# DCDmllm/AnyEdit

Measured on AMD Instinct MI355X. Metric: edited-images/sec @512x512, 50 DDIM steps, higher is better.
Workload: dtype bf16; 1 GPU; configs[1]: AnySD (SD-1.5 UNet in=8 + task embedding/expert adapters) 512x512 bf16, 50 DDIM steps, batch=4/GPU, 3-branch CFG (UNet batch 12); images_per_gpu=4, ddim_steps=50, cfg_branches=3, hip_graph=True, parallelism=dp1 (image-sharded, no data-path collective)

## Files before the change

anyedit_amd/_lib.py:

```python
import ctypes
import os

import torch

_HERE = os.path.dirname(os.path.abspath(__file__))
LIB_PATH = os.environ.get("AE_LIB_PATH") or os.path.join(_HERE, "libanyedit_hip.so")

c_void_p, c_int, c_long, c_float = ctypes.c_void_p, ctypes.c_int, ctypes.c_long, ctypes.c_float

SIGNATURES = {
    "ae_version": [],
    "ae_last_error": [],
    "ae_device_arch": [ctypes.c_char_p, c_int],
    "ae_device_info": [ctypes.POINTER(c_int), ctypes.POINTER(c_long), ctypes.POINTER(c_int)],
    "ae_gemm_bf16": [c_void_p, c_long, c_void_p, c_long, c_int, c_void_p, c_long, c_void_p, c_long, c_int, c_int, c_int,
                     c_void_p, c_void_p, c_long, c_void_p, c_long, c_int, c_int, c_int, c_void_p, c_void_p],
    "ae_conv3x3_workspace_floats": [c_int, c_int, c_int, c_int, c_int, c_int, c_int],
    "ae_conv3x3_bf16": [c_void_p, c_void_p, c_void_p, c_void_p, c_long, c_void_p, c_void_p, c_int, c_int, c_int, c_int, c_int,
                        c_int, c_int, c_int, c_void_p, c_void_p, c_int, c_void_p],
    "ae_conv3x3_up2_bf16": [c_void_p, c_void_p, c_void_p, c_void_p, c_int, c_int, c_int, c_int, c_int, c_void_p, c_void_p],
    "ae_gemm_plan": [c_int] * 8 + [ctypes.POINTER(c_int)],
    "ae_conv3x3_plan": [c_int] * 11 + [ctypes.POINTER(c_int)],
    "ae_conv3x3_up2_plan": [c_int] * 6 + [ctypes.POINTER(c_int)],
    "ae_groupnorm_rows_per_chunk": [c_int, c_int],
    "ae_groupnorm_workspace_floats": [c_int, c_int, c_int, c_int],
    "ae_groupnorm_nhwc_bf16": [c_void_p, c_void_p, c_int, c_void_p, c_void_p, c_void_p, c_int, c_int, c_int, c_int, c_float,
                               c_int, c_void_p, c_void_p, c_void_p, c_void_p, c_void_p, c_void_p],
    "ae_layernorm_bf16": [c_void_p, c_void_p, c_void_p, c_void_p, c_int, c_int, c_float, c_void_p],
    "ae_attn_fwd_bf16": [c_void_p, c_void_p, c_void_p, c_void_p, c_int, c_int, c_int, c_int, c_int,
                         c_long, c_long, c_long, c_long, c_long, c_long, c_long, c_long, c_long, c_long, c_long, c_long,
                         c_float, c_void_p, c_void_p, c_int, c_int, c_void_p, c_void_p, c_int,
                         c_void_p, c_void_p, c_int, c_long, c_long, c_long, c_long, c_long, c_long, c_void_p, c_void_p, c_void_p,
                         c_void_p],
    "ae_attn_bwd_bf16": [c_void_p] * 10 + [c_int] * 5 + [c_long] * 21 + [c_float, c_void_p, c_int, c_void_p, c_void_p],
    "ae_attn_bwd_workspace_floats": [c_int] * 5,
    "ae_groupnorm_bwd_workspace_floats": [c_int, c_int, c_int, c_int],
    "ae_groupnorm_bwd_nhwc_bf16": [c_void_p, c_void_p, c_int, c_void_p, c_void_p, c_void_p, c_void_p, c_void_p, c_int, c_int, c_int,
                                   c_int, c_float, c_int, c_void_p, c_void_p, c_void_p, c_int, c_void_p],
    "ae_layernorm_bwd_bf16": [c_void_p, c_void_p, c_void_p, c_void_p, c_void_p, c_int, c_int, c_float, c_int, c_void_p],
    "ae_layernorm_param_grad_f32": [c_void_p, c_void_p, c_void_p, c_void_p, c_void_p, c_int, c_int, c_void_p],
    "ae_add_bf16": [c_void_p, c_void_p, c_void_p, c_long, c_void_p],
    "ae_axpy_bf16": [c_void_p, c_void_p, c_float, c_void_p, c_long, c_void_p],
    "ae_geglu_fwd_bf16": [c_void_p, c_void_p, c_long, c_int, c_void_p],
    "ae_geglu_bwd_bf16": [c_void_p, c_void_p, c_void_p, c_long, c_int, c_void_p],
    "ae_sumpool2x2_bf16": [c_void_p, c_void_p, c_int, c_int, c_int, c_int, c_void_p],
    "ae_colsum_bf16_f32": [c_void_p, c_void_p, c_int, c_int, c_long, c_void_p],
    "ae_mse_grad_f32": [c_void_p, c_void_p, c_void_p, c_long, c_float, c_void_p],
    "ae_adamw_f32": [c_void_p, c_void_p, c_void_p, c_void_p, c_long, c_float, c_float, c_float, c_float, c_float, c_int, c_float,
                     c_void_p],
    "ae_rowsum_f32": [c_void_p, c_void_p, c_int, c_long, c_void_p],
    "ae_scatter_add_rows_f32": [c_void_p, c_void_p, c_void_p, c_int, c_int, c_int, c_void_p],
    "ae_attn_fp8_workspace_bytes": [c_int, c_int, c_int, c_int, c_int],
    "ae_attn_fwd_fp8": [c_void_p, c_void_p, c_void_p, c_void_p, c_int, c_int, c_int, c_int, c_int] + [c_long] * 12 +
                       [c_float, c_void_p, c_void_p, c_int, c_int, c_void_p, c_long, c_void_p],
    "ae_ln_gemm_supported": [c_int, c_int, c_int, c_int],
    "ae_ln_gemm_bf16": [c_void_p, c_long, c_void_p, c_long, c_void_p, c_long, c_int, c_int, c_int, c_void_p, c_void_p, c_long, c_void_p, c_void_p,
                        c_float, c_int, c_void_p, c_void_p],
    "ae_gemm_ln_plan": [c_int, c_int, c_int, c_int, c_int],
    "ae_ff_fused_supported": [c_int, c_int, c_int],
    "ae_ff_fused_bf16": [c_void_p, c_long, c_void_p, c_void_p, c_float, c_void_p, c_long, c_void_p, c_void_p, c_void_p, c_void_p, c_long,
                         c_void_p, c_long, c_void_p, c_void_p, c_long, c_void_p, c_void_p, c_long, c_int, c_int, c_int, c_void_p],
    "ae_gemm_ln_bf16": [c_void_p, c_long, c_void_p, c_long, c_void_p, c_long, c_int, c_int, c_int, c_void_p, c_void_p, c_long, c_int, c_void_p,
                        c_void_p, c_int, c_void_p, c_float, c_void_p],
    "ae_task_gate_bwd": [c_void_p, c_void_p, c_void_p, c_void_p, c_int, c_int, c_int, c_void_p, c_void_p],
    "ae_task_gate_wgrad": [c_void_p, c_void_p, c_void_p, c_void_p, c_void_p, c_int, c_int, c_int, c_int, c_void_p, c_void_p, c_void_p],
    "ae_expert_kv_fwd": [c_void_p, c_void_p, c_void_p, c_void_p, c_int, c_int, c_int, c_int, c_int, c_void_p],
    "ae_expert_kv_dgrad_slices": [c_int],
    "ae_expert_kv_dgrad": [c_void_p, c_void_p, c_void_p, c_void_p, c_int, c_int, c_int, c_int, c_int, c_void_p, c_void_p],
    "ae_expert_kv_wgrad": [c_void_p, c_void_p, c_void_p, c_void_p, c_int, c_int, c_int, c_int, c_int, c_void_p],
    "ae_transpose_last2": [c_void_p, c_void_p, c_int, c_int, c_int, c_int, c_int, c_int, c_void_p],
    "ae_concat_channels_bf16": [c_void_p, c_int, c_void_p, c_int, c_void_p, c_long, c_void_p],
    "ae_im2col3x3_c8_bf16": [c_void_p, c_void_p, c_int, c_int, c_int, c_void_p],
    "ae_split_channels_bf16": [c_void_p, c_int, c_int, c_void_p, c_void_p, c_long, c_int, c_int, c_void_p],
    "ae_timestep_embedding": [c_void_p, c_void_p, c_void_p, c_void_p, c_int, c_int, c_float, c_void_p],
    "ae_ddim_step_f32": [c_void_p, c_void_p, c_void_p, c_void_p, c_void_p, c_void_p, c_long, c_int, c_float, c_float, c_float,
                         c_float, c_float, c_float, c_float, c_float, c_void_p],
    "ae_ddim_encode_step_f32": [c_void_p, c_void_p, c_void_p, c_long, c_int, c_float, c_float, c_float, c_void_p],
    "ae_plms_combine_f32": [c_void_p, c_void_p, c_void_p, c_void_p, c_void_p, c_long, c_int, c_void_p],
    "ae_mask_blend_f32": [c_void_p, c_void_p, c_void_p, c_void_p, c_void_p, c_int, c_int, c_int, c_float, c_float, c_int, c_void_p],
    "ae_q_sample_f32": [c_void_p, c_void_p, c_void_p, c_void_p, c_void_p, c_int, c_long, c_void_p],
    "ae_silu_to_bf16": [c_void_p, c_int, c_void_p, c_long, c_void_p],
    "ae_add_bcast_bf16": [c_void_p, c_void_p, c_void_p, c_long, c_long, c_void_p],
    "ae_resample2x_rows_bf16": [c_void_p, c_void_p, c_int, c_int, c_int, c_int, c_int, c_void_p],
    "ae_scale_shift_rows_bf16": [c_void_p, c_void_p, c_long, c_void_p, c_int, c_long, c_int, c_int, c_void_p],
    "ae_window_partition_bf16": [c_void_p, c_void_p, c_int, c_int, c_int, c_int, c_int, c_int, c_void_p],
    "ae_layernorm_window_supported": [c_int],
    "ae_layernorm_window_bf16": [c_void_p, c_void_p, c_void_p, c_void_p, c_void_p, c_void_p, c_int, c_int, c_int, c_int, c_int, c_int, c_float,
                                 c_void_p],
    "ae_sam_relpos_terms": [c_void_p, c_long, c_long, c_long, c_void_p, c_void_p, c_void_p, c_void_p, c_int, c_int, c_int, c_int,
                            c_int, c_int, c_int, c_void_p],
    "ae_softmax_rows_f32_bf16": [c_void_p, c_long, c_void_p, c_long, c_int, c_int, c_float, c_void_p],
    "ae_gaussian_moments_f32": [c_void_p, c_void_p, c_void_p, c_void_p, c_void_p, c_void_p, c_int, c_long, c_void_p],
    "ae_ms_deform_attn_fwd_f32": [c_void_p] * 6 + [c_int] * 7 + [c_void_p],
    "ae_ms_deform_attn_bwd_f32": [c_void_p] * 9 + [c_int] * 7 + [c_void_p],
    "ae_linear_f32": [c_void_p, c_long, c_void_p, c_long, c_void_p, c_void_p, c_long, c_int, c_int, c_int, c_void_p],
    "ae_dpm_multistep_f32": [c_void_p] * 5 + [c_long, c_int, c_float, c_int, c_int, c_float, c_float, c_int, c_float, c_float, c_float,
                             c_float, c_void_p],
    "ae_layernorm_act_bf16": [c_void_p, c_void_p, c_void_p, c_void_p, c_long, c_int, c_float, c_int, c_void_p],
    "ae_sam_pe_encode_f32": [c_void_p, c_void_p, c_void_p, c_void_p, c_void_p, c_int, c_int, c_float, c_float, c_float, c_void_p],
    "ae_sam_mask_downscale_bf16": [c_void_p] * 10 + [c_int, c_int, c_int, c_float, c_void_p],
    "ae_sam_mask_product_f32": [c_void_p, c_void_p, c_void_p, c_int, c_int, c_int, c_int, c_int, c_void_p],
    "ae_sam_postprocess_masks": [c_void_p, c_void_p, c_void_p] + [c_int] * 8 + [c_float, c_int, c_void_p],
    "ae_nms_sorted_f32": [c_void_p, c_void_p, c_int, c_float, c_void_p],
    "ae_sam_preprocess_f32": [c_void_p, c_int, c_void_p, c_int, c_int, c_int, c_int, c_int, c_void_p, c_void_p, c_void_p],
    "ae_patchify_f32_bf16": [c_void_p, c_void_p, c_int, c_int, c_int, c_int, c_int, c_void_p],
    "ae_mse_f32": [c_void_p, c_void_p, c_void_p, c_void_p, c_long, c_void_p],
    "ae_lincomb4_f32": [c_void_p, c_void_p, c_float, c_void_p, c_float, c_void_p, c_float, c_void_p, c_float, c_long, c_void_p],
    "ae_dpm_adaptive_err_f32": [c_void_p, c_void_p, c_void_p, c_float, c_float, c_int, c_long, c_void_p, c_void_p],
    "ae_task_gate": [c_void_p, c_void_p, c_void_p, c_void_p, c_int, c_int, c_int, c_int, c_void_p, c_void_p, c_void_p, c_void_p],
    "ae_attn_causal_short_bf16": [c_void_p, c_void_p, c_void_p, c_void_p, c_int, c_int, c_int, c_int] + [c_long] * 12 + [c_float, c_void_p],
    "ae_clip_embed_bf16": [c_void_p, c_int, c_void_p, c_void_p, c_void_p, c_int, c_int, c_int, c_int, c_int, c_void_p],
    "ae_bias_act_f32_bf16": [c_void_p, c_long, c_void_p, c_void_p, c_long, c_long, c_int, c_int, c_void_p],
    "ae_clip_pool_eos_bf16": [c_void_p, c_int, c_void_p, c_void_p, c_int, c_int, c_int, c_long, c_void_p],
    "ae_clip_patch_rows_bf16": [c_void_p, c_int, c_void_p, c_int, c_int, c_int, c_int, c_int, c_int, c_float, c_void_p, c_void_p, c_void_p],
    "ae_clip_vision_embed_ln_bf16": [c_void_p, c_long, c_void_p, c_void_p, c_void_p, c_void_p, c_void_p, c_int, c_int, c_int, c_float, c_void_p],
    "ae_clip_vision_pool_ln_bf16": [c_void_p, c_long, c_void_p, c_void_p, c_void_p, c_int, c_int, c_float, c_void_p],
    "ae_dino_embed_bf16": [c_void_p, c_long, c_void_p, c_void_p, c_void_p, c_void_p, c_int, c_int, c_int, c_void_p],
    "ae_swiglu_f32_bf16": [c_void_p, c_long, c_void_p, c_void_p, c_long, c_long, c_int, c_void_p],
    "ae_swin_window_attn_bf16": [c_void_p, c_long, c_void_p, c_void_p, c_void_p, c_long, c_int, c_int, c_int, c_int, c_int, c_int, c_int, c_float, c_void_p],
    "ae_swin_merge_ln_bf16": [c_void_p, c_void_p, c_void_p, c_void_p, c_int, c_int, c_int, c_int, c_float, c_void_p],
    "ae_scale_residual_f32_bf16": [c_void_p, c_long, c_void_p, c_void_p, c_void_p, c_long, c_void_p, c_long, c_long, c_int, c_void_p],
    "ae_biattn_split_rows": [c_int],
    "ae_biattn_workspace_bytes": [c_int, c_int, c_int, c_int, c_int],
    "ae_biattn_bf16": [c_void_p, c_long] * 4 + [c_void_p, c_void_p] + [c_void_p, c_long] * 2 + [c_int] * 5 + [c_float, c_void_p, c_long, c_void_p],
    "ae_attn_masked_short_bf16": [c_void_p] * 5 + [c_int] * 4 + [c_long] * 12 + [c_float, c_void_p],
    "ae_contrastive_bf16": [c_void_p, c_long, c_void_p, c_void_p, c_void_p, c_long, c_void_p] + [c_int] * 5 + [c_void_p],
    "ae_topk_rows_max_n": [],
    "ae_topk_rows_f32": [c_void_p, c_long, c_void_p, c_int, c_int, c_int, c_void_p],
    "ae_gdino_proposals_f32": [c_void_p, ctypes.POINTER(c_int), ctypes.POINTER(c_int), c_int, c_void_p, c_void_p, c_int, c_int, c_void_p],
    "ae_gdino_query_sine": [c_void_p, c_void_p, c_void_p, c_void_p, c_long, c_int, c_int, c_int, c_void_p],
    "ae_gdino_box_refine_f32": [c_void_p, c_long, c_void_p, c_void_p, c_void_p, c_void_p, c_void_p, c_long, c_int, c_void_p],
    "ae_gdino_text_spans": [c_void_p, c_int, c_int, c_int, c_int] + [c_long] * 8 + [c_void_p, c_void_p, c_void_p, c_void_p],
    "ae_bert_embed_ln_bf16": [c_void_p, c_void_p, c_void_p] + [c_void_p] * 6 + [c_int] * 6 + [c_float, c_void_p],
    "ae_attn_span_short_bf16": [c_void_p] * 5 + [c_int] * 4 + [c_long] * 12 + [c_float, c_void_p],
    "ae_gdino_level_geometry": [c_void_p, c_int, c_int, c_int, ctypes.POINTER(c_int), ctypes.POINTER(c_int), c_int, c_float, c_float, c_void_p, c_void_p, c_void_p,
                                c_void_p, c_int, c_void_p],
    "ae_gdino_neck_groupnorm_workspace_floats": [c_int, c_int],
    "ae_gdino_neck_groupnorm": [c_void_p, c_long, c_void_p, c_void_p, c_float, c_void_p, c_long, c_long, c_int, c_int, c_void_p, c_void_p],
    "ae_gdino_ground": [c_void_p, c_void_p, c_float, c_float, c_void_p, c_void_p, c_void_p, c_void_p, c_void_p, c_int, c_int, c_int, c_void_p],
    "ae_hed_stem_bf16": [c_void_p, c_int, c_long, c_long, c_long, c_long, c_void_p, c_void_p, c_void_p, c_void_p, c_int, c_int, c_int, c_int, c_void_p],
    "ae_relu_bf16": [c_void_p, c_long, c_void_p],
    "ae_hed_tail_bf16": [c_void_p, c_void_p, c_void_p, c_void_p, c_void_p, c_int, c_int, c_int, c_int, c_void_p],
    "ae_hed_fuse": [c_void_p] * 7 + [c_int] * 4 + [c_void_p],
    "ae_dpt_reassemble_bf16": [c_void_p, c_long, c_void_p, c_void_p, c_int, c_int, c_int, c_int, c_int, c_void_p],
    "ae_dpt_resize_bf16": [c_void_p] * 4 + [c_int] * 6 + [c_void_p],
    "ae_dpt_relu_bf16": [c_void_p, c_void_p, c_long, c_void_p],
    "ae_dpt_tail_bf16": [c_void_p] * 4 + [c_int] * 4 + [c_void_p],
    "ae_depth_resize_minmax_f32": [c_void_p] * 3 + [c_int] * 5 + [c_void_p],
    "ae_depth_colorize_u8": [c_void_p] * 4 + [c_int] * 3 + [c_void_p],
    "ae_dwconv_rows_bf16": [c_void_p] * 5 + [c_int] * 5 + [c_void_p],
    "ae_patch2_rows_bf16": [c_void_p, c_void_p, c_int, c_int, c_int, c_int, c_void_p],
    "ae_layernorm_rows_nchw": [c_void_p, c_void_p, c_void_p, c_float, c_void_p, c_void_p, c_int, c_int, c_int, c_int, c_void_p],
    "ae_ppm_pool_rows_bf16": [c_void_p, c_void_p, c_int, c_int, c_int, c_int, c_void_p, c_int, c_void_p],
    "ae_resize_concat_rows_bf16": [c_void_p] * 8 + [c_int, c_void_p, c_long, c_void_p, c_long, c_int, c_int, c_int, c_void_p],
    "ae_seg_argmax_u8": [c_void_p, c_long, c_int, c_void_p, c_void_p, c_void_p] + [c_int] * 7 + [c_void_p],
    "ae_attn_mutual_bf16": [c_void_p] * 4 + [c_int] * 4 + [c_long] * 12 + [c_float, ctypes.POINTER(c_int), c_void_p, c_void_p, c_void_p, c_void_p],
    "ae_attn_token_map_bf16": [c_void_p] * 3 + [c_int] * 5 + [c_long] * 6 + [c_float, ctypes.POINTER(ctypes.c_ulonglong), c_int, c_void_p],
    "ae_masactrl_classes": [c_void_p, c_long, c_int, c_int, c_float, c_int, ctypes.POINTER(c_int), ctypes.POINTER(c_int), c_void_p, c_void_p, c_void_p],
}
_RESTYPES = {"ae_last_error": ctypes.c_char_p, "ae_groupnorm_workspace_floats": c_long, "ae_conv3x3_workspace_floats": c_long,
             "ae_groupnorm_bwd_workspace_floats": c_long, "ae_attn_fp8_workspace_bytes": c_long, "ae_attn_bwd_workspace_floats": c_long,
             "ae_biattn_workspace_bytes": c_long, "ae_gdino_neck_groupnorm_workspace_floats": c_long}


class AnyEditHipError(RuntimeError):
    pass


def _load():
    if not os.path.exists(LIB_PATH):
        raise ImportError(
            f"{LIB_PATH} is missing: the HIP extension is REQUIRED (no CPU/eager fallback exists). "
            "Build it with `python -c 'import __graft_entry__ as g; g.build()'` or `python anyedit_amd/build.py`.")
    lib = ctypes.CDLL(LIB_PATH)
    for name, argtypes in SIGNATURES.items():
        fn = getattr(lib, name)
        fn.argtypes = argtypes
        fn.restype = _RESTYPES.get(name, c_int)
    return lib


lib = _load()


def check(rc, what=""):
    if rc != 0:
        msg = lib.ae_last_error()
        raise AnyEditHipError(f"{what} failed (rc={rc}): {msg.decode() if msg else ''}")


def device_arch():
    buf = ctypes.create_string_buffer(128)
    check(lib.ae_device_arch(buf, 128), "ae_device_arch")
    return buf.value.decode()
```

anyedit_amd/csrc/gemm_conv.hip:

```cpp
#include "common.hpp"
#include <stdlib.h>
#include <string.h>
#include <type_traits>

namespace {

#ifndef AE_CONV_SPEC
#define AE_CONV_SPEC 1
#endif
#ifndef AE_XE_OCC
#define AE_XE_OCC 4
#endif
#ifndef AE_PP_LAB
#define AE_PP_LAB 0
#endif
#ifndef AE_PP_PRIO
#define AE_PP_PRIO 1
#endif
#ifndef AE_PP_DMA_FIRST
#define AE_PP_DMA_FIRST 0
#endif
constexpr int BK = 64;

enum { A_DENSE = 0, A_CONV3 = 1 };
enum { EPI_NONE = 0, EPI_GELU = 1, EPI_GEGLU = 2, EPI_SILU = 3, EPI_RELU = 4 };

struct GemmArgs {
    const bf16_t* A;
    const bf16_t* A2;
    const bf16_t* W;
    void* C;
    const float* bias;
    const bf16_t* res;
    const float* addvec;
    int M, N, K, Ksplit;
    long lda, lda2, ldw, ldc, ldr, ldav;
    int epi, out_f32, rows_per_batch;
    int H, Wd, Cin, CinPad, Ho, Wo, stride, ups;
    unsigned a_bytes, a2_bytes, w_bytes;
    int splitk;
    float* partial;
    float* colstats;
    int kmajor;
    int m_fast;
    int xe;
    float* rowstats;
    const float* ln_stats;
    const float* ln_colsum;
    int ln_parts;
    float ln_eps;
    int sub2;
};

__device__ __forceinline__ void lds_dma16(__amdgpu_buffer_rsrc_t rs, bf16_t* lds_dst, int voffset, int soffset = 0) {
#if defined(__HIP_DEVICE_COMPILE__)
    __builtin_amdgcn_raw_ptr_buffer_load_lds(rs, (__attribute__((address_space(3))) void*)lds_dst, 16, voffset, soffset, 0, 0);
#endif
}

#ifdef AE_GEMM_LAB
__device__ unsigned long long g_gemm_dbg[32];
#define GL_T(i) do { const unsigned long long t_ = __builtin_readcyclecounter(); if (lab_me) g_gemm_dbg[lab_base + (i)] += t_ - tlast; tlast = t_; } while (0)
#elif defined(AE_GEMM_TRACE)
constexpr int TR_K0 = 18, TR_T = 6;
__device__ unsigned long long g_pp_trace[8 * TR_T * 16];
#define GL_T(i) do { __builtin_amdgcn_sched_barrier(0); tr_t[(i)] = __builtin_readcyclecounter(); __builtin_amdgcn_sched_barrier(0); } while (0)
#else
#define GL_T(i)
#endif

constexpr int epilogue_passes(int FM, int bytes_per_frag_row, int lds_bytes) {
    for (int ps = 1; ps <= FM; ++ps)
        if (FM % ps == 0 && (FM / ps) * bytes_per_frag_row <= lds_bytes) return ps;
    return FM;
}

template <int BM, int BN, int AMODE, int WAVES_M = 2, int WAVES_N = 2, bool GLDS = false, int WAVES_K = 1, int STAGES = 2, bool CS = false, int LAB = 0, int WA = 0, int XE = 0>
__global__ __launch_bounds__(64 * WAVES_M * WAVES_N * WAVES_K, (XE == 2 && BM == 128 && BN == 128 && STAGES == 2) ? AE_XE_OCC : 0) void gemm_kernel(const GemmArgs p) {
    static_assert(XE == 0 || (AMODE == A_DENSE && WAVES_K == 1 && !CS && GLDS), "row statistics / LayerNorm fold: dense LDS-DMA instantiations, one K group, no column statistics");
    static_assert(XE != 1 || BN / WAVES_N == 64, "row statistics are emitted per 64-column slice = one wave tile's width");
    static_assert(STAGES == 2 || (GLDS && WAVES_K == 1), "the deep LDS ring exists only for the LDS-DMA loader");
    static_assert(!WA || (GLDS && STAGES == 2 && WAVES_K == 1), "operand-ahead is a variant of the two-stage LDS-DMA pipeline");
    static_assert(WA == 0 || WA == 1 || WA == 3 || WA == 4, "WA: 0 none, 1 weights two tiles ahead (three W stages), 3 ping-pong (two wave groups one barrier apart), 4 ping-pong over an activation slab per (channel chunk, ky)");
    static_assert(WA < 3 || 64 * WAVES_M * WAVES_N * WAVES_K == 512, "the ping-pong loops pair wave w with wave w + 4 (one SIMD's two waves)");
    static_assert(WA != 4 || (AMODE == A_CONV3 && GLDS && BM % 16 == 0), "the slab loop is a 3x3-convolution loop");
    static_assert(WAVES_K == 1, "one K group per block (the two-group form is removed: DESIGN.md, \"Built, measured, removed\")");
    constexpr int NT = 64 * WAVES_M * WAVES_N * WAVES_K;
    constexpr int WM = BM / WAVES_M, WN = BN / WAVES_N;
    constexpr int FM = WM / 16, FN = WN / 16;
    constexpr int A_CH = BM * 8 / NT, B_CH = BN * 8 / NT;
    static_assert((BM * 8) % NT == 0 && (BN * 8) % NT == 0, "tile / thread-count combination not supported");
    extern __shared__ __attribute__((aligned(16))) unsigned char smem_raw[];
    bf16_t* const smem = reinterpret_cast<bf16_t*>(smem_raw);
    bf16_t* sA = smem;
    bf16_t* sB = smem + (WA >= 3 ? 3 : STAGES) * BM * BK;

#ifndef AE_WAVE_SGPR
#define AE_WAVE_SGPR 1
#endif
    const int tid = threadIdx.x, lane = tid & 63, wave = AE_WAVE_SGPR ? __builtin_amdgcn_readfirstlane(tid >> 6) : tid >> 6;
#ifdef AE_GEMM_TRACE
    const bool tr_blk = blockIdx.x == gridDim.x / 2 && WA == 3;
    unsigned long long* const tr_lds = reinterpret_cast<unsigned long long*>(smem_raw + 152 * 1024);
    int tr_kt = -1;
    unsigned long long tr_t[16];
#pragma unroll
    for (int q = 0; q < 16; ++q) tr_t[q] = 0;
#endif
#ifdef AE_GEMM_LAB
    unsigned long long tlast = __builtin_readcyclecounter();
    const bool lab_me = blockIdx.x == gridDim.x / 2 && lane == 0 && (wave == 0 || wave == 4);
    const int lab_base = wave == 0 ? 0 : 16;
#endif
    const int wk = wave / (WAVES_M * WAVES_N), wmn = wave % (WAVES_M * WAVES_N);
    const int wm = wmn / WAVES_N, wn = wmn % WAVES_N;
    const int l15 = lane & 15, lg = lane >> 4;
    const int ntn = (p.N + BN - 1) / BN, ntm = (p.M + BM - 1) / BM;
    const int ntiles = ntm * ntn;
    const int split = blockIdx.x / ntiles;
    const int py = (AMODE == A_CONV3 && p.sub2) ? split >> 1 : 0, px = (AMODE == A_CONV3 && p.sub2) ? split & 1 : 0;
    const int tile = xcd_remap(blockIdx.x % ntiles, ntiles);
    const int m0 = (p.m_fast ? tile % ntm : tile / ntn) * BM, n0 = (p.m_fast ? tile / ntm : tile % ntn) * BN;

    long a_base[A_CH];
    int a_iy[A_CH], a_ix[A_CH];
#pragma unroll
    for (int i = 0; i < A_CH; ++i) {
        const int row = (tid + i * NT) >> 3;
        const int m = m0 + row;
        const int mc = min(m, p.M - 1);
        if (AMODE == A_DENSE) {
            a_base[i] = (long)mc;
            a_iy[i] = a_ix[i] = 0;
        } else {
            const int hw = p.Ho * p.Wo;
            const int b = mc / hw, rem = mc - b * hw;
            const int oy = rem / p.Wo, ox = rem - oy * p.Wo;
            a_base[i] = (long)b * p.H * p.Wd;
            a_iy[i] = (m < p.M) ? oy * p.stride - 1 : -100000;
            a_ix[i] = ox * p.stride - 1;
        }
    }
    long b_base[B_CH];
#pragma unroll
    for (int i = 0; i < B_CH; ++i) {
        const int row = (tid + i * NT) >> 3;
        b_base[i] = (long)min(n0 + row, p.N - 1) * p.ldw;
    }

    const __amdgpu_buffer_rsrc_t rsA = __builtin_amdgcn_make_buffer_rsrc(const_cast<bf16_t*>(p.A), 0, (int)p.a_bytes, 0x00020000);
    const __amdgpu_buffer_rsrc_t rsA2 = __builtin_amdgcn_make_buffer_rsrc(const_cast<bf16_t*>(p.A2 ? p.A2 : p.A), 0, (int)(p.A2 ? p.a2_bytes : 0u), 0x00020000);
    const __amdgpu_buffer_rsrc_t rsW = __builtin_amdgcn_make_buffer_rsrc(const_cast<bf16_t*>(p.W) + ((AMODE == A_CONV3 && p.sub2) ? (long)split * p.N * p.ldw : 0L), 0, (int)p.w_bytes, 0x00020000);
    constexpr int OOB = (int)0x80000000;
    int fa_off[A_CH], fa2_off[A_CH], fb_off[B_CH];
    unsigned fa_mask[A_CH];
#pragma unroll
    for (int i = 0; i < A_CH; ++i) {
        const int id = tid + i * NT, row = id >> 3;
        const int c = GLDS ? ((id & 7) ^ (row & 7)) : (id & 7);
        const int m = m0 + row;
        fa_mask[i] = 0u;
        if (AMODE == A_DENSE) {
            fa_off[i] = (m < p.M) ? (int)((long)m * p.lda * 2) + c * 16 : OOB;
            fa2_off[i] = (m < p.M) ? (int)((long)m * p.lda2 * 2) + c * 16 : OOB;
        } else {
            fa2_off[i] = OOB;
            const int hw = p.Ho * p.Wo;
            const int mc = min(m, p.M - 1);
            const int b = mc / hw, rem = mc - b * hw;
            const int oy = rem / p.Wo, ox = rem - oy * p.Wo;
            const int iy0 = oy * p.stride - 1, ix0 = ox * p.stride - 1;
            fa_off[i] = (int)(((long)(b * p.H + iy0) * p.Wd + ix0) * p.Cin + c * 8) * 2;
            const int Hv = p.ups ? 2 * p.H : p.H, Wv = p.ups ? 2 * p.Wd : p.Wd;
            if (m < p.M) {
#pragma unroll
                for (int t9 = 0; t9 < 9; ++t9) {
                    const int iy = iy0 + t9 / 3, ix = ix0 + t9 % 3;
                    if ((unsigned)iy < (unsigned)Hv && (unsigned)ix < (unsigned)Wv && (p.ups != 2 || ((iy | ix) & 1) == 0)) fa_mask[i] |= 1u << t9;
                }
            }

        }
    }
#pragma unroll
    for (int i = 0; i < B_CH; ++i) {
        const int id = tid + i * NT, row = id >> 3;
        const int c = GLDS ? ((id & 7) ^ (row & 7)) : (id & 7);
        fb_off[i] = (n0 + row < p.N) ? (int)((long)(n0 + row) * p.ldw * 2) + c * 16 : OOB;
    }
    const bool conv_fast = (AMODE == A_CONV3) && p.Cin == p.CinPad;

    u32x4 ra[A_CH], rb[B_CH];
    const u32x4 zero4 = {0u, 0u, 0u, 0u};
    const int KT_all = (p.K + BK - 1) / BK;
    const int kt_per = (KT_all + p.splitk - 1) / p.splitk;
    const int kt_begin = (AMODE == A_CONV3 && p.sub2) ? 0 : split * kt_per;
    const int KT = max(min(KT_all - kt_begin, kt_per), 0);
    const int klast = p.K - 8;
    const int conv_per = AMODE == A_CONV3 ? p.CinPad / BK : 1;
    const unsigned conv_per_magic = (AE_CONV_SPEC && conv_per > 1) ? 0xFFFFFFFFu / (unsigned)conv_per + 1u : 0u;
    const unsigned pp_magic = (WA == 3 && conv_per > 1) ? 0xFFFFFFFFu / (unsigned)conv_per + 1u : 0u;
    int ld_tap = (kt_begin * BK) / (AMODE == A_CONV3 ? p.CinPad : 1 << 30), ld_ci = (AMODE == A_CONV3) ? (kt_begin * BK) % p.CinPad : 0;
    if (AMODE == A_CONV3 && p.kmajor) { ld_tap = kt_begin % 9; ld_ci = (kt_begin / 9) * BK; }

    auto load_tile = [&](int kt) __attribute__((always_inline)) {
        const int k0 = (kt_begin + kt) * BK;
        const bool full_k = k0 + BK <= p.K;
        if (AMODE == A_DENSE && full_k && (k0 + BK <= p.Ksplit || k0 >= p.Ksplit)) {
            if (k0 < p.Ksplit) {
#pragma unroll
                for (int i = 0; i < A_CH; ++i) ra[i] = __builtin_amdgcn_raw_buffer_load_b128(rsA, fa_off[i] + k0 * 2, 0, 0);
            } else {
#pragma unroll
                for (int i = 0; i < A_CH; ++i) ra[i] = __builtin_amdgcn_raw_buffer_load_b128(rsA2, fa2_off[i] + (k0 - p.Ksplit) * 2, 0, 0);
            }
#pragma unroll
            for (int i = 0; i < B_CH; ++i) rb[i] = __builtin_amdgcn_raw_buffer_load_b128(rsW, fb_off[i] + k0 * 2, 0, 0);
            return;
        }
        if (conv_fast) {
            const int ky = ld_tap / 3, kx = ld_tap - ky * 3;
            const int tap_off = ((ky * p.Wd + kx) * p.Cin + ld_ci) * 2;
#pragma unroll
            for (int i = 0; i < A_CH; ++i) {
                int src = fa_off[i] + tap_off;
                if (p.ups) {
                    const int cc = GLDS ? (((tid + i * NT) & 7) ^ (((tid + i * NT) >> 3) & 7)) : ((tid + i * NT) & 7);
                    src = (int)((a_base[i] + (long)(max(a_iy[i] + ky, 0) >> 1) * p.Wd + (max(a_ix[i] + kx, 0) >> 1)) * p.Cin + cc * 8 + ld_ci) * 2;
                }
                const int off = ((fa_mask[i] >> ld_tap) & 1u) ? src : OOB;
                ra[i] = __builtin_amdgcn_raw_buffer_load_b128(rsA, off, 0, 0);
            }
            ld_ci += BK;
            if (ld_ci >= p.CinPad) { ld_ci = 0; ++ld_tap; }
#pragma unroll
            for (int i = 0; i < B_CH; ++i) rb[i] = __builtin_amdgcn_raw_buffer_load_b128(rsW, fb_off[i] + k0 * 2, 0, 0);
            return;
        }
        if (AMODE == A_DENSE) {
#pragma unroll
            for (int i = 0; i < A_CH; ++i) {
                const int c = (tid + i * NT) & 7;
                const int k = min(k0 + c * 8, klast);
                const bf16_t* src = (k >= p.Ksplit) ? p.A2 + a_base[i] * p.lda2 + (k - p.Ksplit) : p.A + a_base[i] * p.lda + k;
                ra[i] = *reinterpret_cast<const u32x4*>(src);
            }
        } else {
            const int ky = ld_tap / 3, kx = ld_tap - ky * 3;
            const int Hv = p.ups ? 2 * p.H : p.H, Wv = p.ups ? 2 * p.Wd : p.Wd;
#pragma unroll
            for (int i = 0; i < A_CH; ++i) {
                const int c = (tid + i * NT) & 7;
                const int iy = a_iy[i] + ky, ix = a_ix[i] + kx;
                const int ci = ld_ci + c * 8;
                const bool ok = (unsigned)iy < (unsigned)Hv && (unsigned)ix < (unsigned)Wv && ci < p.Cin && (p.ups != 2 || ((iy | ix) & 1) == 0);
                const int cy = min(max(iy, 0), Hv - 1), cx = min(max(ix, 0), Wv - 1);
                const int sy = p.ups ? (cy >> 1) : cy, sx = p.ups ? (cx >> 1) : cx;
                const u32x4 v = *reinterpret_cast<const u32x4*>(p.A + (a_base[i] + (long)sy * p.Wd + sx) * p.Cin + min(ci, p.Cin - 8));
                ra[i] = ok ? v : zero4;
            }
            ld_ci += BK;
            if (ld_ci >= p.CinPad) { ld_ci = 0; ++ld_tap; }
        }
#pragma unroll
        for (int i = 0; i < B_CH; ++i) {
            const int k = k0 + ((tid + i * NT) & 7) * 8;
            const u32x4 v = *reinterpret_cast<const u32x4*>(p.W + b_base[i] + min(k, klast));
            rb[i] = (k < p.K) ? v : zero4;
        }
    };

    auto store_tile = [&](int buf) __attribute__((always_inline)) {
#pragma unroll
        for (int i = 0; i < A_CH; ++i) {
            const int id = tid + i * NT, row = id >> 3, c = id & 7;
            *reinterpret_cast<u32x4*>(sA + buf * BM * BK + row * BK + ((c ^ (row & 7)) << 3)) = ra[i];
        }
#pragma unroll
        for (int i = 0; i < B_CH; ++i) {
            const int id = tid + i * NT, row = id >> 3, c = id & 7;
            *reinterpret_cast<u32x4*>(sB + buf * BN * BK + row * BK + ((c ^ (row & 7)) << 3)) = rb[i];
        }
    };

    f32x4 acc[FM][FN];
#pragma unroll
    for (int i = 0; i < FM; ++i)
#pragma unroll
        for (int j = 0; j < FN; ++j) acc[i][j] = (f32x4){0.f, 0.f, 0.f, 0.f};

    float ln_r[XE == 2 ? FM : 1], ln_t[XE == 2 ? FM : 1];
    constexpr int LNP = 5;
    constexpr bool SC_LDS = XE == 2 && WA == 3;
    static_assert(!SC_LDS || (BN % 4 == 0 && (3 * BM + 2 * BN) * BK * 2 + 2 * BN * 4 <= 160 * 1024), "s / c of the block must fit behind the ping-pong ring");
    float* const sc_lds = reinterpret_cast<float*>(smem_raw + (3 * BM + 2 * BN) * BK * 2);
    f32x2 raw[XE == 2 ? FM : 1][LNP];
    f32x4 szp[(XE == 2 && !SC_LDS) ? FN : 1], bzp[(XE == 2 && !SC_LDS) ? FN : 1], scv[2];
    if constexpr (XE == 2) {
#pragma unroll
        for (int i = 0; i < FM; ++i) {
            const int m = min(m0 + wm * WM + i * 16 + l15, p.M - 1);
            const f32x2* sp = reinterpret_cast<const f32x2*>(p.ln_stats) + (long)m * p.ln_parts;
#pragma unroll
            for (int u = 0; u < LNP; ++u) raw[i][u] = sp[min(lg + 4 * u, p.ln_parts - 1)];
        }
        if constexpr (SC_LDS) {
            const int n = min(n0 + 4 * min(tid, BN / 4 - 1), p.N - 4);
            scv[0] = *reinterpret_cast<const f32x4*>(p.ln_colsum + n);
            scv[1] = *reinterpret_cast<const f32x4*>(p.bias + n);
        } else {
#pragma unroll
            for (int j = 0; j < FN; ++j) {
                const int nc = p.epi == EPI_GEGLU ? min(n0 + wn * WN + (j & ~1) * 16 + lg * 4, p.N - 20) + (j & 1) * 16 : min(n0 + wn * WN + j * 16 + lg * 4, p.N - 4);
                szp[j] = *reinterpret_cast<const f32x4*>(p.ln_colsum + nc);
                bzp[j] = *reinterpret_cast<const f32x4*>(p.bias + nc);
            }
        }
    }
    auto xe_mid = [&]() __attribute__((always_inline)) {
        if constexpr (XE == 2) {
            const float inv_k = 1.0f / (float)p.K;
#pragma unroll
            for (int i = 0; i < FM; ++i) {
                float s = 0.f, q = 0.f;
#pragma unroll
                for (int u = 0; u < LNP; ++u) {
                    const bool in = lg + 4 * u < p.ln_parts;
                    s += in ? raw[i][u][0] : 0.f;
                    q += in ? raw[i][u][1] : 0.f;
                }
                s += __shfl_xor(s, 16, 64); q += __shfl_xor(q, 16, 64);
                s += __shfl_xor(s, 32, 64); q += __shfl_xor(q, 32, 64);
                const float mu = s * inv_k;
                const float r = rsqrtf(fmaxf(q * inv_k - mu * mu, 0.f) + p.ln_eps);
                ln_r[i] = r;
                ln_t[i] = -r * mu;
            }
            if constexpr (SC_LDS) {
                if (tid < BN / 4) {
                    const float hc = (p.epi == EPI_GEGLU && ((4 * tid) & 16) == 0) ? 0.5f : 1.0f;
                    reinterpret_cast<f32x4*>(sc_lds)[tid] = scv[0];
                    reinterpret_cast<f32x4*>(sc_lds + BN)[tid] = (f32x4){scv[1][0] * hc, scv[1][1] * hc, scv[1][2] * hc, scv[1][3] * hc};
                }
            }
        }
    };

    auto compute_tile = [&](int cur, int curB = -1) __attribute__((always_inline)) {
        if (LAB == 2) return;
        const bf16_t* cA = sA + cur * BM * BK + (wm * WM) * BK;
        const bf16_t* cB = sB + (curB < 0 ? cur : curB) * BN * BK + (wn * WN) * BK;
#pragma unroll
        for (int kk = 0; kk < 2; ++kk) {
            bf16x8_t af[FM], bfr[FN];
            const int ch = kk * 4 + lg;
#pragma unroll
            for (int i = 0; i < FM; ++i) {
                const int row = i * 16 + l15;
                if (LAB == 3) af[i] = as_bf16x8((u32x4){(uint32_t)(i + cur), 0x3f803f80u, (uint32_t)lane, 0u});
                else af[i] = as_bf16x8(*reinterpret_cast<const u32x4*>(cA + row * BK + ((ch ^ (row & 7)) << 3)));
            }
#pragma unroll
            for (int j = 0; j < FN; ++j) {
                const int row = j * 16 + l15;
                if (LAB == 3) bfr[j] = as_bf16x8((u32x4){(uint32_t)(j + kk), 0x3f803f80u, (uint32_t)lane, 0u});
                else bfr[j] = as_bf16x8(*reinterpret_cast<const u32x4*>(cB + row * BK + ((ch ^ (row & 7)) << 3)));
            }
#pragma unroll
            for (int i = 0; i < FM; ++i)
#pragma unroll
                for (int j = 0; j < FN; ++j)
                    acc[i][j] = __builtin_amdgcn_mfma_f32_16x16x32_bf16(bfr[j], af[i], acc[i][j], 0, 0, 0);
        }
    };

    if (!GLDS) {
        load_tile(0);
        store_tile(0);
        __syncthreads();
        for (int kt = 0; kt < KT; ++kt) {
            const int cur = kt & 1;
            if (kt + 1 < KT) load_tile(kt + 1);
            compute_tile(cur);
            if (kt + 1 < KT) store_tile(cur ^ 1);
            __syncthreads();
        }
    } else {
        int fa_cur[A_CH];
        auto dma_a = [&](int kt, int buf) __attribute__((always_inline)) {
            const int k0 = (kt_begin + kt) * BK;
            if (AMODE == A_DENSE) {
                const bool second = k0 >= p.Ksplit;
                if (AE_CONV_SPEC) {
                    if (!second) {
#pragma unroll
                        for (int i = 0; i < A_CH; ++i) lds_dma16(rsA, sA + buf * BM * BK + (wave + (NT / 64) * i) * 8 * BK, fa_off[i], k0 * 2);
                    } else {
#pragma unroll
                        for (int i = 0; i < A_CH; ++i) lds_dma16(rsA2, sA + buf * BM * BK + (wave + (NT / 64) * i) * 8 * BK, fa2_off[i], (k0 - p.Ksplit) * 2);
                    }
                } else {
#pragma unroll
                for (int i = 0; i < A_CH; ++i) {
                    bf16_t* dst = sA + buf * BM * BK + (wave + (NT / 64) * i) * 8 * BK;
                    if (!second) lds_dma16(rsA, dst, fa_off[i], k0 * 2);
                    else lds_dma16(rsA2, dst, fa2_off[i], (k0 - p.Ksplit) * 2);
                }
                }
            } else {
                int cur_tap = ld_tap, cur_ci = ld_ci;
                constexpr bool STATELESS = true;
                if (STATELESS) {
                    const int lin = kt_begin + kt;
                    if (p.kmajor) { cur_tap = lin % 9; cur_ci = (lin / 9) * BK; }
                    else if (AE_CONV_SPEC) {
                        cur_tap = conv_per == 1 ? lin : (int)__umulhi((unsigned)lin, conv_per_magic);
                        cur_ci = (lin - cur_tap * conv_per) * BK;
                    } else { const int per = p.CinPad / BK; cur_tap = lin / per; cur_ci = (lin - cur_tap * per) * BK; }
                }
                const int ky = p.sub2 ? py + (cur_tap >> 1) : cur_tap / 3, kx = p.sub2 ? px + (cur_tap & 1) : cur_tap - ky * 3;
                const int mbit = p.sub2 ? ky * 3 + kx : cur_tap;
                if (cur_ci == 0 || kt == 0 || p.kmajor) {
#pragma unroll
                    for (int i = 0; i < A_CH; ++i) {
                        int src = fa_off[i] + ((ky * p.Wd + kx) * p.Cin) * 2;
                        if (p.ups) {
                            const int cc = ((tid + i * NT) & 7) ^ (((tid + i * NT) >> 3) & 7);
                            src = (int)((a_base[i] + (long)(max(a_iy[i] + ky, 0) >> 1) * p.Wd + (max(a_ix[i] + kx, 0) >> 1)) * p.Cin + cc * 8) * 2;
                        }
                        fa_cur[i] = ((fa_mask[i] >> mbit) & 1u) ? src : OOB;
                    }
                }
                const int tap_off = cur_ci * 2;
                if (!(LAB == 4 && (kt % 9) >= 2)) {
#pragma unroll
                for (int i = 0; i < A_CH; ++i) {
                    bf16_t* dst = sA + buf * BM * BK + (wave + (NT / 64) * i) * 8 * BK;
                    lds_dma16(rsA, dst, fa_cur[i], tap_off);
                }
                }
                if (STATELESS) {
                } else if (p.kmajor) {
                    if (++ld_tap == 9) { ld_tap = 0; ld_ci += BK; }
                } else {
                    ld_ci += BK;
                    if (ld_ci >= p.CinPad) { ld_ci = 0; ++ld_tap; }
                }
            }
        };
        auto dma_w = [&](int kt, int buf) __attribute__((always_inline)) {
            const int k0 = (kt_begin + kt) * BK;
#pragma unroll
            for (int i = 0; i < B_CH; ++i) {
                bf16_t* dst = sB + buf * BN * BK + (wave + (NT / 64) * i) * 8 * BK;
                lds_dma16(rsW, dst, fb_off[i], k0 * 2);
            }
        };
        auto dma_tile = [&](int kt, int buf) __attribute__((always_inline)) { dma_a(kt, buf); dma_w(kt, buf); };
        if constexpr (WA == 4) {
            static_assert(BK * 2 == 128, "slab rows are 128 bytes");
            constexpr int SLAB_P = (BM + BM / 16 + 1 + 7) / 8;
            constexpr int S_CH = (SLAB_P + NT / 64 - 1) / (NT / 64);
            constexpr int A_ST = SLAB_P * 1024, W_ST = BN * BK * 2;
            const int lds0 = (int)(uintptr_t)((__attribute__((address_space(3))) char*)smem_raw);
            const int ldsW = lds0 + 2 * A_ST + wave * 1024;
            const int grp = wave >> 2;
            const int W1 = p.Wd + 1, nrow = BM / p.Wd;
            const int y0 = (m0 / p.Wd) % p.H;
            int sl_off[S_CH], sl_dst[S_CH];
            unsigned sl_ok[S_CH];
#pragma unroll
            for (int j = 0; j < S_CH; ++j) {
                int q = wave + (NT / 64) * j;
                if (q >= SLAB_P) q -= NT / 64;
                const int srow = 8 * q + (lane >> 3);
                const int jr = srow / W1, pos = srow - jr * W1;
                const int m = m0 + jr * p.Wd + pos - 1;
                int y = y0 + jr;
                y -= (y >= p.H) ? p.H : 0;
                unsigned ok = 0u;
                if (pos > 0 && jr < nrow && m < p.M) {
#pragma unroll
                    for (int ky = 0; ky < 3; ++ky)
                        if ((unsigned)(y + ky - 1) < (unsigned)p.H) ok |= 1u << ky;
                }
                sl_ok[j] = ok;
                sl_off[j] = m * p.Cin * 2 + (((lane & 7) ^ (lane >> 3)) << 4);
                sl_dst[j] = lds0 + q * 1024;
            }
            const int ky_step = p.Wd * p.Cin * 2;
            const int cbase = kt_begin / 9;
            auto pp_slab = [&](int c, int ky, int st) __attribute__((always_inline)) {
                int off[S_CH];
#pragma unroll
                for (int j = 0; j < S_CH; ++j) off[j] = ((sl_ok[j] >> ky) & 1u) ? sl_off[j] + (ky - 1) * ky_step : OOB;
#pragma unroll
                for (int j = 0; j < S_CH; ++j) asm volatile("" : "+v"(off[j]));
#pragma unroll
                for (int j = 0; j < S_CH; ++j) ae_dma16(rsA, sl_dst[j] + st * A_ST, off[j], (cbase + c) * (BK * 2));
            };
            auto pp_w = [&](int kt, int st) __attribute__((always_inline)) {
                const int k0 = (kt_begin + kt) * BK;
#pragma unroll
                for (int i = 0; i < B_CH; ++i) ae_dma16(rsW, ldsW + st * W_ST + i * (NT / 64) * 1024, fb_off[i], k0 * 2);
            };
            int a_rd[FM][3][2];
#pragma unroll
            for (int i = 0; i < FM; ++i) {
                const int r0 = wm * WM + i * 16;
                const int base = r0 + r0 / p.Wd + l15;
#pragma unroll
                for (int kx = 0; kx < 3; ++kx)
#pragma unroll
                    for (int kk = 0; kk < 2; ++kk) a_rd[i][kx][kk] = (base + kx) * 128 + (((kk * 4 + lg) ^ ((base + kx) & 7)) << 4);
            }
            int w_rd[2];
#pragma unroll
            for (int kk = 0; kk < 2; ++kk) w_rd[kk] = 2 * A_ST + (wn * WN + l15) * 128 + (((kk * 4 + lg) ^ (l15 & 7)) << 4);
            bf16x8_t af[FM], bfr[FN];
            auto pp_read = [&](int kk, int kx, int sa, int sw) __attribute__((always_inline)) {
#pragma unroll
                for (int i = 0; i < FM; ++i) af[i] = as_bf16x8(*reinterpret_cast<const u32x4*>(smem_raw + sa * A_ST + a_rd[i][kx][kk]));
#pragma unroll
                for (int j = 0; j < FN; ++j) bfr[j] = as_bf16x8(*reinterpret_cast<const u32x4*>(smem_raw + sw * W_ST + w_rd[kk] + j * 16 * 128));
            };
            auto pp_mfma = [&]() __attribute__((always_inline)) {
                __builtin_amdgcn_sched_barrier(0);
                if (AE_PP_PRIO) __builtin_amdgcn_s_setprio(1);
#pragma unroll
                for (int i = 0; i < FM; ++i)
#pragma unroll
                    for (int j = 0; j < FN; ++j) acc[i][j] = __builtin_amdgcn_mfma_f32_16x16x32_bf16(bfr[j], af[i], acc[i][j], 0, 0, 0);
                if (AE_PP_PRIO) __builtin_amdgcn_s_setprio(0);
                __builtin_amdgcn_sched_barrier(0);
                __builtin_amdgcn_s_barrier();
                __builtin_amdgcn_sched_barrier(0);
            };
            if (KT > 0) { pp_w(0, 0); pp_slab(0, 0, 0); }
            asm volatile("s_waitcnt vmcnt(0)" ::: "memory");
            __builtin_amdgcn_s_barrier();
            if (grp) __builtin_amdgcn_s_barrier();
            __builtin_amdgcn_sched_barrier(0);
            for (int kt0 = 0; kt0 < KT; kt0 += 18) {
                const int c0 = kt0 / 9;
#pragma unroll
                for (int u = 0; u < 18; ++u) {
                    const int kt = kt0 + u;
                    if (kt >= KT) break;
                    const int tap = u % 9, ky = tap / 3, kx = tap % 3;
                    const int sa = ((u / 9) + ky) & 1, sw = u & 1;
                    pp_read(0, kx, sa, sw);
                    if (kt + 1 < KT) pp_w(kt + 1, sw ^ 1);
                    asm volatile("s_waitcnt lgkmcnt(0)" ::: "memory");
                    __builtin_amdgcn_sched_barrier(0);
                    __builtin_amdgcn_s_barrier();
                    pp_mfma();
                    pp_read(1, kx, sa, sw);
                    const bool slab_next = kx == 0 && kt + 3 < KT;
                    if (slab_next) pp_slab(ky == 2 ? c0 + u / 9 + 1 : c0 + u / 9, ky == 2 ? 0 : ky + 1, sa ^ 1);
                    asm volatile("s_waitcnt lgkmcnt(0)" ::: "memory");
                    if (slab_next) asm volatile("s_waitcnt vmcnt(%0)" ::"n"(S_CH) : "memory");
                    else asm volatile("s_waitcnt vmcnt(0)" ::: "memory");
                    __builtin_amdgcn_sched_barrier(0);
                    __builtin_amdgcn_s_barrier();
                    pp_mfma();
                }
            }
            if (!grp) __builtin_amdgcn_s_barrier();
            __builtin_amdgcn_sched_barrier(0);
        } else if constexpr (WA == 3) {
            const int lds0 = (int)(uintptr_t)((__attribute__((address_space(3))) char*)smem_raw);
            constexpr int A_ST = BM * BK * 2, W_ST = BN * BK * 2;
            const int ldsA = lds0 + wave * 1024, ldsW = lds0 + 3 * A_ST + wave * 1024;
            const int grp = wave >> 2;
            auto pp_w = [&](int kt, int st) __attribute__((always_inline)) {
                const int k0 = (kt_begin + kt) * BK;
#pragma unroll
                for (int i = 0; i < B_CH; ++i) ae_dma16(rsW, ldsW + st * W_ST + i * (NT / 64) * 1024, fb_off[i], k0 * 2);
            };
            int cs_tap = 0, cs_kx = 0, cs_base = 0, cs_ci = 0;
            const int cs_cin2 = p.Cin * 2, cs_row2 = (p.Wd - 3) * p.Cin * 2;
            auto cs_set = [&](int kt) __attribute__((always_inline)) {
                const int lin = kt_begin + kt;
                if (p.kmajor) { cs_tap = lin % 9; cs_ci = (lin / 9) * BK; }
                else { cs_tap = conv_per == 1 ? lin : (int)__umulhi((unsigned)lin, pp_magic); cs_ci = (lin - cs_tap * conv_per) * BK; }
                int ky = cs_tap / 3;
                cs_kx = cs_tap - ky * 3;
                if (p.sub2) { ky = py + (cs_tap >> 1); cs_kx = px + (cs_tap & 1); cs_tap = ky * 3 + cs_kx; }
                cs_base = ((ky * p.Wd + cs_kx) * p.Cin) * 2;
            };
            auto cs_next = [&]() __attribute__((always_inline)) {
                bool tap_step = true;
                if (!p.kmajor) { cs_ci += BK; tap_step = cs_ci >= p.CinPad; cs_ci = tap_step ? 0 : cs_ci; }
                if (tap_step) {
                    if (p.sub2) {
                        if (cs_kx == px) { ++cs_tap; ++cs_kx; cs_base += cs_cin2; }
                        else { cs_tap += 2; cs_kx = px; cs_base += cs_row2 + 2 * cs_cin2; }
                    } else {
                    ++cs_tap; ++cs_kx; cs_base += cs_cin2;
                    if (cs_kx == 3) { cs_kx = 0; cs_base += cs_row2; }
                    if (cs_tap == 9) { cs_tap = 0; cs_base = 0; cs_ci += BK; }
                    }
                }
            };
            auto pp_a = [&](int kt, int st) __attribute__((always_inline)) {
                if constexpr (AMODE == A_DENSE) {
                    const int k0 = (kt_begin + kt) * BK;
                    if (k0 < p.Ksplit) {
#pragma unroll
                        for (int i = 0; i < A_CH; ++i) ae_dma16(rsA, ldsA + st * A_ST + i * (NT / 64) * 1024, fa_off[i], k0 * 2);
                    } else {
#pragma unroll
                        for (int i = 0; i < A_CH; ++i) ae_dma16(rsA2, ldsA + st * A_ST + i * (NT / 64) * 1024, fa2_off[i], (k0 - p.Ksplit) * 2);
                    }
                } else {
                    int off[A_CH];
#pragma unroll
                    for (int i = 0; i < A_CH; ++i) off[i] = ((fa_mask[i] >> cs_tap) & 1u) ? fa_off[i] + cs_base : OOB;
#pragma unroll
                    for (int i = 0; i < A_CH; ++i) asm volatile("" : "+v"(off[i]));
#pragma unroll
                    for (int i = 0; i < A_CH; ++i) ae_dma16(rsA, ldsA + st * A_ST + i * (NT / 64) * 1024, off[i], cs_ci * 2);
                    cs_next();
                }
            };
            bf16x8_t af[FM], bfr[FN];
            auto pp_read = [&](int kk, int sa, int sw) __attribute__((always_inline)) {
                const bf16_t* cA = sA + sa * BM * BK + (wm * WM) * BK;
                const bf16_t* cB = sB + sw * BN * BK + (wn * WN) * BK;
                const int ch = kk * 4 + lg;
#pragma unroll
                for (int i = 0; i < FM; ++i) {
                    const int row = i * 16 + l15;
                    if (AE_PP_LAB == 2 || AE_PP_LAB == 3) af[i] = as_bf16x8((u32x4){(uint32_t)(i + sa), 0x3f803f80u, (uint32_t)lane, 0u});
                    else af[i] = as_bf16x8(*reinterpret_cast<const u32x4*>(cA + row * BK + ((ch ^ (row & 7)) << 3)));
                }
#pragma unroll
                for (int j = 0; j < FN; ++j) {
                    const int row = j * 16 + l15;
                    if (AE_PP_LAB == 2 || AE_PP_LAB == 3) bfr[j] = as_bf16x8((u32x4){(uint32_t)(j + kk), 0x3f803f80u, (uint32_t)lane, 0u});
                    else bfr[j] = as_bf16x8(*reinterpret_cast<const u32x4*>(cB + row * BK + ((ch ^ (row & 7)) << 3)));
                }
            };
            auto pp_mfma = [&](int lab_m, int lab_b) __attribute__((always_inline)) {
                __builtin_amdgcn_sched_barrier(0);
                if (AE_PP_PRIO) __builtin_amdgcn_s_setprio(1);
                if (AE_PP_LAB != 2) {
#pragma unroll
                for (int i = 0; i < FM; ++i)
#pragma unroll
                    for (int j = 0; j < FN; ++j) acc[i][j] = __builtin_amdgcn_mfma_f32_16x16x32_bf16(bfr[j], af[i], acc[i][j], 0, 0, 0);
                }
                if (AE_PP_PRIO) __builtin_amdgcn_s_setprio(0);
                __builtin_amdgcn_sched_barrier(0);
                GL_T(lab_m);
                __builtin_amdgcn_s_barrier();
                __builtin_amdgcn_sched_barrier(0);
                GL_T(lab_b);
            };
            if constexpr (AMODE == A_CONV3) cs_set(0);
            pp_w(0, 0); pp_a(0, 0);
            if (KT > 1) { pp_a(1, 1); asm volatile("s_waitcnt vmcnt(%0)" ::"n"(A_CH) : "memory"); }
            else asm volatile("s_waitcnt vmcnt(0)" ::: "memory");
            xe_mid();
            __builtin_amdgcn_s_barrier();
            if (grp) __builtin_amdgcn_s_barrier();
            __builtin_amdgcn_sched_barrier(0);
            GL_T(0);
            for (int kt0 = 0; kt0 < KT; kt0 += 6) {
#pragma unroll
                for (int u = 0; u < 6; ++u) {
                    const int kt = kt0 + u;
                    if (kt >= KT) break;
                    const int sa = u % 3, sw = u & 1;
#ifdef AE_GEMM_TRACE
                    tr_kt = kt;
                    GL_T(0);
#endif
                    if (AE_PP_DMA_FIRST && AE_PP_LAB != 1 && kt + 1 < KT) pp_w(kt + 1, sw ^ 1);
                    pp_read(0, sa, sw);
                    if (!AE_PP_DMA_FIRST && AE_PP_LAB != 1 && kt + 1 < KT) pp_w(kt + 1, sw ^ 1);
                    asm volatile("s_waitcnt lgkmcnt(0)" ::: "memory");
                    __builtin_amdgcn_sched_barrier(0);
                    GL_T(1);
                    __builtin_amdgcn_s_barrier();
                    GL_T(2);
                    pp_mfma(3, 8);
                    if (AE_PP_DMA_FIRST && AE_PP_LAB != 1 && kt + 2 < KT) pp_a(kt + 2, (u + 2) % 3);
                    pp_read(1, sa, sw);
                    if (!AE_PP_DMA_FIRST && AE_PP_LAB != 1 && kt + 2 < KT) pp_a(kt + 2, (u + 2) % 3);
                    asm volatile("s_waitcnt lgkmcnt(0)" ::: "memory");
                    GL_T(9);
                    if (kt + 2 < KT) asm volatile("s_waitcnt vmcnt(%0)" ::"n"(A_CH) : "memory");
                    else asm volatile("s_waitcnt vmcnt(0)" ::: "memory");
                    __builtin_amdgcn_sched_barrier(0);
                    GL_T(10);
                    __builtin_amdgcn_s_barrier();
                    GL_T(11);
                    pp_mfma(12, 13);
#ifdef AE_GEMM_TRACE
                    if (tr_blk && kt >= TR_K0 && kt < TR_K0 + TR_T && lane == 0) {
#pragma unroll
                        for (int q = 0; q < 16; ++q) tr_lds[(wave * TR_T + (kt - TR_K0)) * 16 + q] = tr_t[q];
                    }
#endif
#ifdef AE_GEMM_LAB
                    if (lab_me) g_gemm_dbg[lab_base + 5] += 1;
#endif
                }
            }
            if (!grp) __builtin_amdgcn_s_barrier();
            __builtin_amdgcn_sched_barrier(0);
#ifdef AE_GEMM_TRACE
            tr_kt = -1;
            if (tr_blk) {
                asm volatile("s_waitcnt lgkmcnt(0)" ::: "memory");
                __builtin_amdgcn_s_barrier();
                for (int q = tid; q < 8 * TR_T * 16; q += NT) g_pp_trace[q] = tr_lds[q];
            }
#endif
        } else if constexpr (WA != 0) {
            constexpr int FAR = B_CH;
            dma_a(0, 0); dma_w(0, 0); if (KT > 1) dma_w(1, 1);
            if (KT > 1) asm volatile("s_waitcnt vmcnt(%0)" ::"n"(FAR) : "memory");
            else asm volatile("s_waitcnt vmcnt(0)" ::: "memory");
            xe_mid();
            __builtin_amdgcn_s_barrier();
            for (int kt0 = 0; kt0 < KT; kt0 += 6) {
#pragma unroll
                for (int u = 0; u < 6; ++u) {
                    const int kt = kt0 + u;
                    if (kt >= KT) break;
                    const int near_cur = u & 1, far_cur = u % 3, far_next = (u + 2) % 3;
                    if (kt + 1 < KT) dma_a(kt + 1, near_cur ^ 1);
                    if (kt + 2 < KT) dma_w(kt + 2, far_next);
                    compute_tile(near_cur, far_cur);
                    if (kt + 2 < KT) asm volatile("s_waitcnt vmcnt(%0)" ::"n"(FAR) : "memory");
                    else asm volatile("s_waitcnt vmcnt(0)" ::: "memory");
                    asm volatile("s_waitcnt lgkmcnt(0)" ::: "memory");
                    __builtin_amdgcn_s_barrier();
                    asm volatile("" ::: "memory");
                }
            }
        } else if constexpr (STAGES == 2) {
            dma_tile(0, 0);
            __syncthreads();
            GL_T(0);
            for (int kt = 0; kt < KT; ++kt) {
                const int cur = kt & 1;
                if (LAB != 1 && kt + 1 < KT) dma_tile(kt + 1, cur ^ 1);
                GL_T(1);
                compute_tile(cur);
                GL_T(2);
                __syncthreads();
                GL_T(3);
#ifdef AE_GEMM_LAB
                if (lab_me) g_gemm_dbg[lab_base + 5] += 1;
#endif
            }
        } else {
            constexpr int PIECES = A_CH + B_CH;
            constexpr int AHEAD = STAGES - 1;
#pragma unroll
            for (int t = 0; t < AHEAD; ++t)
                if (t < KT) dma_tile(t, t);
            xe_mid();
            int cur = 0, nxt = AHEAD % STAGES;
// ... 387 lines not shown
        }
        if (p.res) { o[0] += bf16lo(rr.x); o[1] += bf16hi(rr.x); o[2] += bf16lo(rr.y); o[3] += bf16hi(rr.y); }
        if (p.out_f32) *reinterpret_cast<f32x4*>(reinterpret_cast<float*>(p.C) + (long)m * p.ldc + n) = (f32x4){o[0], o[1], o[2], o[3]};
        else *reinterpret_cast<u32x2*>(reinterpret_cast<bf16_t*>(p.C) + (long)m * p.ldc + n) = (u32x2){pack_bf16x2(o[0], o[1]), pack_bf16x2(o[2], o[3])};
    }
}

__global__ __launch_bounds__(256) void colstats_kernel(const bf16_t* x, long ld, int M, int N, float* out) {
    __shared__ float red[8][2][256];
    const int cc = threadIdx.x & 31, rr = threadIdx.x >> 5;
    const int n = blockIdx.y * 256 + cc * 8;
    const int r0 = blockIdx.x * 32;
    float s[8], q[8];
#pragma unroll
    for (int e = 0; e < 8; ++e) s[e] = q[e] = 0.f;
    if (n < N) {
        u32x4 v[4];
#pragma unroll
        for (int j = 0; j < 4; ++j) v[j] = *reinterpret_cast<const u32x4*>(x + (long)min(r0 + rr + 8 * j, M - 1) * ld + n);
#pragma unroll
        for (int j = 0; j < 4; ++j) {
            const float keep = (r0 + rr + 8 * j < M) ? 1.f : 0.f;
            const uint32_t w[4] = {v[j].x, v[j].y, v[j].z, v[j].w};
#pragma unroll
            for (int e = 0; e < 4; ++e) {
                const float a = bf16lo(w[e]) * keep, c = bf16hi(w[e]) * keep;
                s[2 * e] += a; q[2 * e] += a * a;
                s[2 * e + 1] += c; q[2 * e + 1] += c * c;
            }
        }
    }
#pragma unroll
    for (int e = 0; e < 8; ++e) { red[rr][0][cc * 8 + e] = s[e]; red[rr][1][cc * 8 + e] = q[e]; }
    __syncthreads();
    const int col = threadIdx.x;
    if (blockIdx.y * 256 + col < N) {
        float a = 0.f, c = 0.f;
#pragma unroll
        for (int r = 0; r < 8; ++r) { a += red[r][0][col]; c += red[r][1][col]; }
        *reinterpret_cast<f32x2*>(out + ((long)blockIdx.x * N + blockIdx.y * 256 + col) * 2) = (f32x2){a, c};
    }
}

int pick_tile(int M, int N) {
    const int cand[3][2] = {{128, 128}, {128, 64}, {64, 64}};
    if (N % 160 == 0 && N % 128 != 0 && (long)((M + 127) / 128) * (N / 160) >= 256) return 3;
    for (int c = 0; c < 3; ++c) {
        const long tm = (M + cand[c][0] - 1) / cand[c][0], tn = (N + cand[c][1] - 1) / cand[c][1];
        const double waste = (double)(tn * cand[c][1]) / (double)N;
        if (tm * tn >= 256 && waste <= 1.10) return c;
    }
    return 2;
}

struct Plan { int tile, splitk; };
Plan make_plan(int M, int N, int K, bool can_split) {
    const int t = pick_tile(M, N);
    const int kt = (K + BK - 1) / BK;
    static const int force_s = getenv("AE_GEMM_SPLITK") ? atoi(getenv("AE_GEMM_SPLITK")) : 0;
    static const int t320_split = getenv("AE_CONV_T320_SPLITK") ? atoi(getenv("AE_CONV_T320_SPLITK")) : 3;
    if (t320_split && can_split && N % 320 == 0 && M % 192 == 0 && force_s <= 0) {
        const long t192 = (long)(M / 192) * (N / 320);
        if (t192 >= 32 && t192 <= (t320_split == 2 ? 64 : (t320_split == 3 && kt < 180 ? 64 : 128))) {
            int s = (int)(256 / t192);
            if (s > 8) s = 8;
            while (s > 1 && kt / s < 16) --s;
            if (s >= 2) return {4, s};
        }
    }
    if (!can_split || kt < 32 || t == 0 || t == 3) return {t, 1};
    const long t128 = (long)((M + 127) / 128) * ((N + 127) / 128);
    const double waste128 = (double)(((N + 127) / 128) * 128) / (double)N;
    if (waste128 <= 1.10 && t128 < 256) {
        int s = force_s > 0 ? force_s : (int)((480 + t128 - 1) / t128);
        static const int smax = getenv("AE_CONV_SPLIT_MAX") ? atoi(getenv("AE_CONV_SPLIT_MAX")) : 8;
        if (s > smax) s = smax;
        if (s > kt / 8) s = kt / 8;
        if (s >= 2) return {0, s};
    }
    return {t, 1};
}

template <typename Kern>
int launch_kernel(Kern kern, unsigned grid, int threads, size_t lds, hipStream_t stream, const GemmArgs& a, const char* what) {
    if (lds > 64 * 1024) {
        static const void* done[32];
        static int ndone = 0;
        const void* fn = reinterpret_cast<const void*>(kern);
        bool seen = false;
        for (int i = 0; i < ndone; ++i) seen |= done[i] == fn;
        if (!seen) {
            if (hipFuncSetAttribute(fn, hipFuncAttributeMaxDynamicSharedMemorySize, (int)lds) != hipSuccess) {
                ae_set_error("hipFuncSetAttribute(MaxDynamicSharedMemorySize=%zu) failed", lds);
                return AE_ERR_LAUNCH;
            }
            if (ndone < 32) done[ndone++] = fn;
        }
    }
    hipLaunchKernelGGL(kern, dim3(grid), dim3(threads), lds, stream, a);
    return ae_check_launch(what);
}

struct PlanReport {
    int BM, BN, AMODE, WAVES_M, WAVES_N, GLDS, WAVES_K, STAGES, CS, LAB, WA, XE;
    int grid, threads, lds, splitk;
    int reduce, colstats;
    int rowpanel;
};
#define AE_PLAN_INTS 19
static_assert(sizeof(PlanReport) == AE_PLAN_INTS * sizeof(int), "PlanReport is the int array of anyedit_hip.h");

void* const kQueryPtr = reinterpret_cast<void*>(uintptr_t(256));
float* const kQueryF32 = reinterpret_cast<float*>(uintptr_t(256));
int plan_out(int rc, const PlanReport& r, int* plan) {
    if (!rc) memcpy(plan, &r, sizeof r);
    return rc;
}

struct LaunchCtx { const GemmArgs& a; hipStream_t stream; const char* what; PlanReport* report; };

template <int BM, int BN, int AMODE, int WAVES_M = 2, int WAVES_N = 2, bool GLDS = false, int WAVES_K = 1, int STAGES = 2, bool CS = false, int LAB = 0, int WA = 0, int XE = 0>
int run_tile(const LaunchCtx& c, long grid, size_t lds) {
    constexpr int threads = 64 * WAVES_M * WAVES_N * WAVES_K;
    if (c.report) {
        *c.report = PlanReport{BM, BN, AMODE, WAVES_M, WAVES_N, GLDS, WAVES_K, STAGES, CS, LAB, WA, XE, (int)grid, threads, (int)lds, c.a.splitk, 0, 0, 0};
        return 0;
    }
    return launch_kernel(gemm_kernel<BM, BN, AMODE, WAVES_M, WAVES_N, GLDS, WAVES_K, STAGES, CS, LAB, WA, XE>, (unsigned)grid, threads, lds, c.stream, c.a, c.what);
}

template <int BM, int BN, int AMODE, int WAVES_M, int WAVES_N>
int run_plain(const LaunchCtx& c, bool glds, long grid) {
    const size_t lds = (size_t)2 * (BM + BN) * BK * sizeof(bf16_t);
    return glds ? run_tile<BM, BN, AMODE, WAVES_M, WAVES_N, true>(c, grid, lds) : run_tile<BM, BN, AMODE, WAVES_M, WAVES_N, false>(c, grid, lds);
}

template <int AMODE>
int launch(const GemmArgs& a_in, hipStream_t stream, PlanReport* report = nullptr, int split_tile = 0) {
    GemmArgs a = a_in;
    static const int mfast_env = getenv("AE_GEMM_MFAST") ? atoi(getenv("AE_GEMM_MFAST")) : -1;
    a.m_fast = mfast_env >= 0 ? mfast_env : (AMODE == A_CONV3 ? (9L * a.N >= 8L * a.M) : ((long)a.N >= 3L * a.M)) ? 1 : 0;
    const int cand[4][2] = {{128, 128}, {128, 64}, {64, 64}, {128, 160}};
    static const int t160 = getenv("AE_GEMM_T160") ? atoi(getenv("AE_GEMM_T160")) : 1;
    int pick = a.splitk > 1 ? 0 : pick_tile(a.M, a.N);
    static const int force_tile = getenv("AE_GEMM_TILE") ? atoi(getenv("AE_GEMM_TILE")) : -1;
    if (force_tile >= 0 && force_tile <= 2 && a.splitk <= 1) pick = force_tile;
    if (pick == 3 && (!t160 || AMODE == A_DENSE || a.epi == EPI_GEGLU || a.splitk > 1)) pick = 1;
    const int kt_block = ((a.K + BK - 1) / BK + a.splitk - 1) / a.splitk;
    const bool conv = AMODE == A_CONV3;
    const char* what = conv ? "ae_conv3x3_bf16" : "ae_gemm_bf16";
    const LaunchCtx lc{a, stream, what, report};
    static const int glds_env = getenv("AE_GEMM_GLDS") ? atoi(getenv("AE_GEMM_GLDS")) : 1;
    const bool glds = glds_env && (conv ? (a.Cin == a.CinPad) : (a.K % BK == 0 && (!a.A2 || a.Ksplit % BK == 0)));
    if (conv && a.kmajor && !glds) { ae_set_error("%s: the chunk-major K order exists only in the LDS-DMA loader (AE_GEMM_GLDS=0 is set)", what); return AE_ERR_UNSUPPORTED; }
    auto lds_of = [](int bm, int bn, int st) { return (size_t)st * (bm + bn) * BK * sizeof(bf16_t); };
    auto lds_wa = [](int bm, int bn) { return (size_t)(2 * bm + 3 * bn) * BK * sizeof(bf16_t); };
#ifdef AE_GEMM_TRACE
    auto lds_aa = [](int bm, int bn) { return (size_t)(3 * bm + 2 * bn) * BK * sizeof(bf16_t) + 8192; };
#else
    auto lds_aa = [](int bm, int bn) { return (size_t)(3 * bm + 2 * bn) * BK * sizeof(bf16_t); };
#endif
    int rc = 0;

    static const int t320 = getenv("AE_GEMM_T320") ? atoi(getenv("AE_GEMM_T320")) : 11;
    bool done = false;
    bool xe_done = false;
    const bool cs_epi_ok = a.colstats && a.epi != EPI_GEGLU && !a.out_f32 && a.splitk <= 1 && a.N % 8 == 0 && a.ldc % 8 == 0 &&
                           (!a.res || (a.ldr % 8 == 0 && (reinterpret_cast<uintptr_t>(a.res) & 15) == 0));
    bool cs_done = false;
#ifdef AE_GEMM_ABLATE
    static const int lab_abl = getenv("AE_GEMM_ABL") ? atoi(getenv("AE_GEMM_ABL")) : 0;
#endif
    const bool slab_ok = conv && a.kmajor && a.stride == 1 && !a.ups && a.Cin == a.CinPad && a.H == a.Ho && a.Wd == a.Wo && a.Wd % 16 == 0 && 192 % a.Wd == 0 &&
                         192 / a.Wd <= a.H + 1 &&
                         (a.splitk <= 1 || kt_block % 9 == 0);
    const size_t lds_slab = (size_t)2 * ((192 + 192 / 16 + 1 + 7) / 8) * 1024 + (size_t)2 * 320 * BK * sizeof(bf16_t);
    if (conv && a.splitk > 1 && glds && split_tile == 4) {
        const long t = (long)(a.M / 192) * (a.N / 320) * a.splitk;
        if constexpr (AMODE == A_CONV3) {
            if (slab_ok) rc = run_tile<192, 320, A_CONV3, 2, 4, true, 1, 2, false, 0, 4>(lc, t, lds_slab);
            else if (!a.ups) rc = run_tile<192, 320, A_CONV3, 2, 4, true, 1, 2, false, 0, 3>(lc, t, lds_aa(192, 320));
            else rc = run_tile<192, 320, A_CONV3, 2, 4, true>(lc, t, lds_of(192, 320, 2));
        }
        done = true;
    }
    if (!done && t320 && glds && a.splitk <= 1 && a.N % 320 == 0 && ((conv && (t320 & 1)) || (!conv && a.epi == EPI_GEGLU && a.K >= 640 && (t320 & 2)) || (!conv && a.epi == EPI_GEGLU && a.K < 640 && a.K >= 320 && (t320 & 4)) ||
                                                                     (!conv && a.epi != EPI_GEGLU && a.K >= 640 && (t320 & 8)))) {
        const long t = (long)((a.M + 191) / 192) * (a.N / 320);
        const double fill = (double)t / (double)(((t + 255) / 256) * 256) * ((double)a.M / (double)(((a.M + 191) / 192) * 192));
        static const int t320_xe = getenv("AE_GEMM_T320_XE") ? atoi(getenv("AE_GEMM_T320_XE")) : 1;
        const long t128x = (long)((a.M + 127) / 128) * ((a.N + 127) / 128);
        const bool xe_tail = t320_xe && !conv && a.xe == 2 && a.epi != EPI_GEGLU && fill >= 0.74 && fill < 0.85 &&
                             (double)t128x / (double)(((t128x + 511) / 512) * 512) <= 0.72;
        if (fill >= 0.85 || xe_tail) {
            if constexpr (AMODE == A_DENSE) {
                if (xe_tail || (a.epi == EPI_GEGLU && a.xe == 2)) { rc = run_tile<192, 320, A_DENSE, 4, 2, true, 1, 2, false, 0, 3, 2>(lc, t, lds_aa(192, 320) + 2 * 320 * sizeof(float)); xe_done = true; }
                else if (a.epi == EPI_GEGLU) rc = run_tile<192, 320, A_DENSE, 4, 2, true, 1, 2, false, 0, 3>(lc, t, lds_aa(192, 320));
                else rc = run_tile<192, 320, A_DENSE, 2, 4, true, 1, 2, false, 0, 3>(lc, t, lds_aa(192, 320));
            } else {
#ifdef AE_GEMM_ABLATE
                if (lab_abl == 1) rc = run_tile<192, 320, A_CONV3, 2, 4, true, 1, 2, false, 1>(lc, t, lds_of(192, 320, 2));
                else if (lab_abl == 2) rc = run_tile<192, 320, A_CONV3, 2, 4, true, 1, 2, false, 2>(lc, t, lds_of(192, 320, 2));
                else if (lab_abl == 3) rc = run_tile<192, 320, A_CONV3, 2, 4, true, 1, 2, false, 3>(lc, t, lds_of(192, 320, 2));
                else if (lab_abl == 4) rc = run_tile<192, 320, A_CONV3, 2, 4, true, 1, 2, false, 4>(lc, t, lds_of(192, 320, 2));
                else if (lab_abl == 20) rc = run_tile<192, 320, A_CONV3, 2, 4, false>(lc, t, lds_of(192, 320, 2));
                else
#endif
                if (!a.ups) {
                    if (slab_ok && cs_epi_ok) { rc = run_tile<192, 320, A_CONV3, 2, 4, true, 1, 2, true, 0, 4>(lc, t, lds_slab); cs_done = true; }
                    else if (slab_ok) rc = run_tile<192, 320, A_CONV3, 2, 4, true, 1, 2, false, 0, 4>(lc, t, lds_slab);
                    else if (cs_epi_ok) { rc = run_tile<192, 320, A_CONV3, 2, 4, true, 1, 2, true, 0, 3>(lc, t, lds_aa(192, 320)); cs_done = true; }
                    else rc = run_tile<192, 320, A_CONV3, 2, 4, true, 1, 2, false, 0, 3>(lc, t, lds_aa(192, 320));
                } else if (cs_epi_ok) {
                    rc = run_tile<192, 320, A_CONV3, 2, 4, true, 1, 2, true>(lc, t, lds_of(192, 320, 2));
                    cs_done = true;
                }
                else rc = run_tile<192, 320, A_CONV3, 2, 4, true>(lc, t, lds_of(192, 320, 2));
            }
            done = true;
        }
    }
    static const int deep_pref = getenv("AE_GEMM_DEEP") ? atoi(getenv("AE_GEMM_DEEP")) : 1;
    if constexpr (AMODE == A_DENSE) {
        if (!done && deep_pref && glds && a.splitk <= 1 && a.epi != EPI_GEGLU && a.N % 128 == 0 && a.K >= 1280) {
            const long t128 = (long)((a.M + 127) / 128) * (a.N / 128);
            const long t192 = (long)((a.M + 191) / 192) * (a.N / 128);
            if (t128 >= 128 && t128 <= 256) {
                if (a.xe == 1) rc = run_tile<128, 128, A_DENSE, 4, 2, true, 1, 3, false, 0, 0, 1>(lc, t128, lds_of(128, 128, 3));
                else if (a.xe) rc = run_tile<128, 128, A_DENSE, 4, 2, true, 1, 3, false, 0, 0, 2>(lc, t128, lds_of(128, 128, 3));
                else rc = run_tile<128, 128, A_DENSE, 4, 2, true, 1, 3>(lc, t128, lds_of(128, 128, 3));
                xe_done = a.xe != 0;
                done = true;
            } else if (t128 > 256 && t192 >= 128 && t192 <= 256 && a.K >= 2560) {
                rc = run_tile<192, 128, A_DENSE, 4, 2, true, 1, 3>(lc, t192, lds_of(192, 128, 3));
                done = true;
            }
        }
    }
    if (!done) {
        const int BM = cand[pick][0], BN = cand[pick][1];
        const unsigned grid = (unsigned)((long)((a.M + BM - 1) / BM) * ((a.N + BN - 1) / BN) * a.splitk);
        static const int deep64_max = getenv("AE_GEMM_DEEP64_MAX") ? atoi(getenv("AE_GEMM_DEEP64_MAX")) : 768;
        if (pick == 3) {
            if constexpr (AMODE == A_CONV3) rc = run_plain<128, 160, AMODE, 2, 2>(lc, glds, grid);
        }
#ifdef AE_GEMM_ABLATE
        else if (pick == 0 && glds && lab_abl == 1) rc = run_tile<128, 128, AMODE, 4, 2, true, 1, 2, false, 1>(lc, grid, lds_of(128, 128, 2));
        else if (pick == 0 && glds && lab_abl == 2) rc = run_tile<128, 128, AMODE, 4, 2, true, 1, 2, false, 2>(lc, grid, lds_of(128, 128, 2));
        else if (pick == 0 && glds && lab_abl == 3) rc = run_tile<128, 128, AMODE, 4, 2, true, 1, 2, false, 3>(lc, grid, lds_of(128, 128, 2));
        else if (pick == 0 && glds && lab_abl == 4) rc = run_tile<128, 128, AMODE, 4, 2, true, 1, 2, false, 4>(lc, grid, lds_of(128, 128, 2));
#endif
        else if (pick == 0 && cs_epi_ok && glds) {
            rc = run_tile<128, 128, AMODE, 4, 2, true, 1, 2, true, 0, 1>(lc, grid, lds_wa(128, 128));
            cs_done = true;
        } else if (pick == 0 && glds && (conv || kt_block >= 3)) {
            if constexpr (AMODE == A_DENSE) {
                if (a.xe == 1) rc = run_tile<128, 128, A_DENSE, 4, 2, true, 1, 2, false, 0, 1, 1>(lc, grid, lds_wa(128, 128));
                else if (a.xe) rc = run_tile<128, 128, A_DENSE, 4, 2, true, 1, 2, false, 0, 1, 2>(lc, grid, lds_wa(128, 128));
                xe_done = a.xe != 0;
            }
            if (!a.xe) rc = run_tile<128, 128, AMODE, 4, 2, true, 1, 2, false, 0, 1>(lc, grid, lds_wa(128, 128));
        }
        else if (pick == 0) {
            if constexpr (AMODE == A_DENSE) rc = run_plain<128, 128, AMODE, 4, 2>(lc, glds, grid);
            else rc = run_tile<128, 128, A_CONV3, 4, 2, false>(lc, grid, lds_of(128, 128, 2));
        } else if (pick == 1) {
            if constexpr (AMODE == A_DENSE) rc = run_plain<128, 64, AMODE, 4, 2>(lc, glds, grid);
            else rc = run_plain<128, 64, AMODE, 2, 2>(lc, glds, grid);
        } else if (deep_pref && glds && !conv && a.splitk <= 1 && grid <= (unsigned)deep64_max && a.K >= 1280) {
            if constexpr (AMODE == A_DENSE) rc = run_tile<64, 64, A_DENSE, 2, 2, true, 1, 3>(lc, grid, lds_of(64, 64, 3));
        } else rc = run_plain<64, 64, AMODE, 2, 2>(lc, glds, grid);
    }
    if (rc) return rc;
    if (a.xe && !xe_done) {
        ae_set_error("%s: no %s instantiation for M=%d N=%d K=%d epilogue %d (ae_gemm_ln_plan says which shapes are covered)", what,
                     a.xe == 1 ? "row-statistics" : "LayerNorm-fold", a.M, a.N, a.K, a.epi);
        return AE_ERR_UNSUPPORTED;
    }
    if (report) {
        report->reduce = a.splitk > 1;
        report->colstats = a.colstats && !cs_done;
        return 0;
    }
    if (a.splitk > 1) {
        long nb = ((long)a.M * a.N / 4 + 255) / 256;
        if (nb > 2048) nb = 2048;
        hipLaunchKernelGGL(splitk_reduce_kernel, dim3((unsigned)nb), dim3(256), 0, stream, a);
        rc = ae_check_launch("ae_conv3x3_bf16(split-K reduce)");
        if (rc) return rc;
    }
    if (a.colstats && !cs_done) return ae_launch_colstats(reinterpret_cast<const bf16_t*>(a.C), a.ldc, a.M, a.epi == EPI_GEGLU ? a.N / 2 : a.N, a.colstats, stream);
    return rc;
}

bool aligned16(const void* p) { return (reinterpret_cast<uintptr_t>(p) & 15) == 0; }

}

int ae_launch_colstats(const bf16_t* x, long ld, int M, int N, float* out, hipStream_t stream) {
    hipLaunchKernelGGL(colstats_kernel, dim3((unsigned)((M + 31) / 32), (unsigned)((N + 255) / 256)), dim3(256), 0, stream, x, ld, M, N, out);
    return ae_check_launch("column statistics");
}

namespace {
struct LnExtras {
    float* rowstats_out = nullptr;
// ... 15 lines not shown
    AE_REQUIRE(epilogue >= EPI_NONE && epilogue <= EPI_RELU, "ae_gemm_bf16: bad epilogue %d", epilogue);
    if (A2) {
        AE_REQUIRE(Ksplit > 0 && Ksplit < K && Ksplit % 8 == 0 && lda2 % 8 == 0 && aligned16(A2),
                   "ae_gemm_bf16: bad two-source split (Ksplit=%d, K=%d)", Ksplit, K);
    }
    if (epilogue == EPI_GEGLU) {
        AE_REQUIRE(N % 32 == 0 && !residual && !addvec && !out_f32, "ae_gemm_bf16: GEGLU needs N %% 32 == 0, bf16 out, no residual");
    }
    if (residual) AE_REQUIRE(ldr % 4 == 0 && (reinterpret_cast<uintptr_t>(residual) & 7) == 0, "ae_gemm_bf16: residual alignment");
    if (addvec) AE_REQUIRE(rows_per_batch > 0, "ae_gemm_bf16: rows_per_batch must be > 0 with addvec");
    a = GemmArgs{};
    a.A = (const bf16_t*)A; a.A2 = (const bf16_t*)A2; a.W = (const bf16_t*)W; a.C = C;
    a.bias = bias; a.res = (const bf16_t*)residual; a.addvec = addvec;
    a.M = M; a.N = N; a.K = K; a.Ksplit = A2 ? Ksplit : K;
    a.lda = lda; a.lda2 = lda2; a.ldw = ldw; a.ldc = ldc; a.ldr = ldr; a.ldav = addvec_ld > 0 ? addvec_ld : N;
    a.epi = epilogue; a.out_f32 = out_f32; a.rows_per_batch = rows_per_batch > 0 ? rows_per_batch : 1;
    a.splitk = 1; a.partial = nullptr; a.colstats = colstats;
    a.a_bytes = (unsigned)((((long)M - 1) * lda + (A2 ? Ksplit : K)) * 2);
    a.a2_bytes = A2 ? (unsigned)((((long)M - 1) * lda2 + (K - Ksplit)) * 2) : 0u;
    a.w_bytes = (unsigned)((((long)N - 1) * ldw + K) * 2);
    AE_REQUIRE(((long)M * lda * 2) < (1L << 31) && ((long)N * ldw * 2) < (1L << 31) && (!A2 || ((long)M * lda2 * 2) < (1L << 31)),
               "ae_gemm_bf16: operands must be smaller than 2 GiB");
    if (x.rowstats_out || x.ln_stats) {
        const int n_out = epilogue == EPI_GEGLU ? N / 2 : N;
        AE_REQUIRE(N % 64 == 0 && n_out % 8 == 0 && ldc % 8 == 0 && (!residual || (ldr % 8 == 0 && aligned16(residual))),
                   "ae_gemm_ln_bf16: N %% 64 == 0 and 16-byte aligned output / residual rows");
        if (x.rowstats_out) {
            AE_REQUIRE(epilogue != EPI_GEGLU && (reinterpret_cast<uintptr_t>(x.rowstats_out) & 7) == 0, "ae_gemm_ln_bf16: row statistics: no GEGLU, 8-byte aligned buffer");
            a.xe = 1; a.rowstats = x.rowstats_out;
        } else {
            AE_REQUIRE(x.ln_colsum && bias && x.ln_parts > 0 && x.ln_parts <= 20 && x.ln_eps >= 0.f, "ae_gemm_ln_bf16: LayerNorm fold needs s (ln_colsum), c (bias), 1..20 statistics slices per row (K <= 1280)");
            AE_REQUIRE(x.ln_parts * 64 == K, "ae_gemm_ln_bf16: the statistics must cover the row: ln_parts * 64 = %d, K = %d (the kernel divides the summed slices by K)", x.ln_parts * 64, K);
            AE_REQUIRE(aligned16(x.ln_colsum) && aligned16(bias) && (reinterpret_cast<uintptr_t>(x.ln_stats) & 7) == 0, "ae_gemm_ln_bf16: s / c must be 16-byte aligned, the statistics 8-byte aligned");
            a.xe = 2; a.ln_stats = x.ln_stats; a.ln_colsum = x.ln_colsum; a.ln_parts = x.ln_parts; a.ln_eps = x.ln_eps;
        }
    }
    return 0;
}

int gemm_entry(const void* A, long lda, const void* A2, long lda2, int Ksplit, const void* W, long ldw,
               void* C, long ldc, int M, int N, int K, const float* bias, const void* residual, long ldr,
               const float* addvec, long addvec_ld, int rows_per_batch, int epilogue, int out_f32, float* colstats, const LnExtras& x, void* stream) {
    GemmArgs a;
    int rc = gemm_args(a, A, lda, A2, lda2, Ksplit, W, ldw, C, ldc, M, N, K, bias, residual, ldr, addvec, addvec_ld, rows_per_batch, epilogue, out_f32, colstats, x);
    if (rc) return rc;
    if (a.xe) {
        PlanReport r;
        rc = launch<A_DENSE>(a, nullptr, &r);
        if (rc) return rc;
    }
    return launch<A_DENSE>(a, (hipStream_t)stream);
}
}

extern "C" int ae_gemm_bf16(const void* A, long lda, const void* A2, long lda2, int Ksplit, const void* W, long ldw,
                            void* C, long ldc, int M, int N, int K, const float* bias, const void* residual, long ldr,
                            const float* addvec, long addvec_ld, int rows_per_batch, int epilogue, int out_f32, float* colstats, void* stream) {
    return gemm_entry(A, lda, A2, lda2, Ksplit, W, ldw, C, ldc, M, N, K, bias, residual, ldr, addvec, addvec_ld, rows_per_batch, epilogue, out_f32, colstats, LnExtras{}, stream);
}

extern "C" int ae_gemm_ln_bf16(const void* A, long lda, const void* W, long ldw, void* C, long ldc, int M, int N, int K, const float* bias,
                               const void* residual, long ldr, int epilogue, float* rowstats_out, const float* ln_stats, int ln_parts,
                               const float* ln_colsum, float ln_eps, void* stream) {
    AE_REQUIRE((rowstats_out != nullptr) != (ln_stats != nullptr), "ae_gemm_ln_bf16: exactly one of rowstats_out (emit) and ln_stats (consume) must be given");
    AE_REQUIRE(A && W && C && M > 0 && N > 0 && K > 0, "ae_gemm_ln_bf16: null pointer or empty shape");
    {
        const int rc = ae_rowpanel_fold_launch(A, lda, W, ldw, C, ldc, M, N, K, bias, residual, ldr, epilogue, rowstats_out, ln_stats, ln_parts, ln_colsum, ln_eps, stream);
        if (rc != AE_ERR_UNSUPPORTED) return rc;
    }
    LnExtras x;
    x.rowstats_out = rowstats_out; x.ln_stats = ln_stats; x.ln_colsum = ln_colsum; x.ln_parts = ln_parts; x.ln_eps = ln_eps;
    return gemm_entry(A, lda, nullptr, 0, 0, W, ldw, C, ldc, M, N, K, bias, residual, ldr, nullptr, 0, 0, epilogue, 0, nullptr, x, stream);
}

extern "C" int ae_gemm_plan(int M, int N, int K, int epilogue, int Ksplit, int out_f32, int colstats, int ln_mode, int* plan) {
    AE_REQUIRE(plan && ln_mode >= 0 && ln_mode <= 2, "ae_gemm_plan: null plan or LN mode %d outside 0..2", ln_mode);
    AE_REQUIRE(M > 0 && N > 0 && K > 0 && K % 8 == 0 && epilogue >= EPI_NONE && epilogue <= EPI_RELU, "ae_gemm_plan: bad shape or epilogue");
    PlanReport r{};
    r.rowpanel = ln_mode ? ae_rowpanel_fold_covers(M, N, K, epilogue, ln_mode) : 0;
    if (r.rowpanel) return plan_out(0, r, plan);
    AE_REQUIRE(ln_mode != 1 || N <= 1280, "ae_gemm_plan: the consumer of row statistics sums up to 20 slices per row (N = %d)", N);
    void* const p = kQueryPtr;
    float* const f = kQueryF32;
    LnExtras x;
    if (ln_mode == 1) x.rowstats_out = f;
    if (ln_mode == 2) { x.ln_stats = f; x.ln_colsum = f; x.ln_parts = K / 64; }
    GemmArgs a;
    const int rc = gemm_args(a, p, K, Ksplit > 0 ? p : nullptr, K, Ksplit, p, K, p, epilogue == EPI_GEGLU ? N / 2 : N, M, N, K, ln_mode == 2 ? f : nullptr, nullptr, 0,
                             nullptr, 0, 0, epilogue, out_f32, colstats ? f : nullptr, x);
    return plan_out(rc ? rc : launch<A_DENSE>(a, nullptr, &r), r, plan);
}

extern "C" int ae_gemm_ln_plan(int M, int N, int K, int epilogue, int mode) {
    int plan[AE_PLAN_INTS];
    return (mode == 1 || mode == 2) && ae_gemm_plan(M, N, K, epilogue, 0, 0, 0, mode, plan) == 0 ? 1 : 0;
}

namespace {
int launch_sub2(GemmArgs a, hipStream_t stream, PlanReport* report = nullptr) {
    const LaunchCtx lc{a, stream, "ae_conv3x3_up2_bf16", report};
    a.m_fast = (9L * a.N >= 8L * a.M) ? 1 : 0;
    const bool cs = a.colstats != nullptr;
    int rc;
    const long t192 = (a.M % 192 == 0 && a.N % 320 == 0) ? (long)(a.M / 192) * (a.N / 320) * 4 : 0;
    if (t192 > 0 && (double)t192 / (double)(((t192 + 255) / 256) * 256) >= 0.85) {
        const size_t lds = (size_t)(3 * 192 + 2 * 320) * BK * sizeof(bf16_t);
        if (cs) rc = run_tile<192, 320, A_CONV3, 2, 4, true, 1, 2, true, 0, 3>(lc, t192, lds);
        else rc = run_tile<192, 320, A_CONV3, 2, 4, true, 1, 2, false, 0, 3>(lc, t192, lds);
    } else {
        const unsigned grid = (unsigned)((long)((a.M + 127) / 128) * ((a.N + 127) / 128) * 4);
        const size_t lds = (size_t)(2 * 128 + 3 * 128) * BK * sizeof(bf16_t);
        if (cs) rc = run_tile<128, 128, A_CONV3, 4, 2, true, 1, 2, true, 0, 1>(lc, grid, lds);
        else rc = run_tile<128, 128, A_CONV3, 4, 2, true, 1, 2, false, 0, 1>(lc, grid, lds);
    }
    return rc;
}
}

namespace {
int up2_args(GemmArgs& a, const void* x, const void* w4, const float* bias, void* y, int B, int H, int W, int Cin, int Cout, float* colstats) {
    AE_REQUIRE(x && w4 && y, "ae_conv3x3_up2_bf16: null pointer");
    AE_REQUIRE(B > 0 && H > 0 && W > 0, "ae_conv3x3_up2_bf16: bad shape B=%d H=%d W=%d", B, H, W);
    AE_REQUIRE(Cin % 64 == 0 && Cout % 8 == 0, "ae_conv3x3_up2_bf16: Cin %% 64 == 0 (whole K tiles per tap) and Cout %% 8 == 0 (row-contiguous stores), got %d -> %d", Cin, Cout);
    AE_REQUIRE(aligned16(x) && aligned16(w4) && aligned16(y), "ae_conv3x3_up2_bf16: pointers must be 16-byte aligned");
    if (colstats) AE_REQUIRE((H * W) % 32 == 0 && (reinterpret_cast<uintptr_t>(colstats) & 15) == 0, "ae_conv3x3_up2_bf16: column statistics are kept per 32-row slab of a sample and parity: H * W = %d must be a multiple of 32", H * W);
    AE_REQUIRE((long)B * H * W * Cin * 2 < (1L << 31) && (long)Cout * 4 * Cin * 2 < (1L << 31) && (long)B * 4 * H * W < (1L << 31), "ae_conv3x3_up2_bf16: operands must be smaller than 2 GiB");
    a = GemmArgs{};
    a.A = (const bf16_t*)x; a.A2 = nullptr; a.W = (const bf16_t*)w4; a.C = y;
    a.bias = bias; a.res = nullptr; a.addvec = nullptr;
    a.M = B * H * W; a.N = Cout; a.K = 4 * Cin; a.Ksplit = a.K;
    a.lda = 0; a.lda2 = 0; a.ldw = 4L * Cin; a.ldc = Cout; a.ldr = Cout; a.ldav = Cout;
    a.epi = EPI_NONE; a.out_f32 = 0; a.rows_per_batch = H * W;
    a.H = H; a.Wd = W; a.Cin = Cin; a.CinPad = Cin; a.Ho = H; a.Wo = W; a.stride = 1; a.ups = 0;
    a.a_bytes = (unsigned)((long)B * H * W * Cin * 2); a.a2_bytes = 0u; a.w_bytes = (unsigned)((long)Cout * 4 * Cin * 2);
    a.splitk = 1; a.partial = nullptr; a.colstats = colstats; a.kmajor = 0; a.sub2 = 1;
    return 0;
}
}

extern "C" int ae_conv3x3_up2_bf16(const void* x, const void* w4, const float* bias, void* y, int B, int H, int W, int Cin, int Cout, float* colstats, void* stream) {
    GemmArgs a;
    const int rc = up2_args(a, x, w4, bias, y, B, H, W, Cin, Cout, colstats);
    return rc ? rc : launch_sub2(a, (hipStream_t)stream);
}

extern "C" int ae_conv3x3_up2_plan(int B, int H, int W, int Cin, int Cout, int colstats, int* plan) {
    AE_REQUIRE(plan, "ae_conv3x3_up2_plan: null plan");
    GemmArgs a;
    PlanReport r{};
    const int rc = up2_args(a, kQueryPtr, kQueryPtr, nullptr, kQueryPtr, B, H, W, Cin, Cout, colstats ? kQueryF32 : nullptr);
    return plan_out(rc ? rc : launch_sub2(a, nullptr, &r), r, plan);
}

extern "C" long ae_conv3x3_workspace_floats(int B, int H, int W, int Cin, int Cout, int stride, int upsample2x) {
    const int Hv = upsample2x ? 2 * H : H, Wv = upsample2x ? 2 * W : W;
    const int Ho = (Hv + 2 - 3) / stride + 1, Wo = (Wv + 2 - 3) / stride + 1;
    const int CinPad = (Cin + BK - 1) / BK * BK;
    const long M = (long)B * Ho * Wo;
    const int s = make_plan((int)M, Cout, 9 * CinPad, true).splitk;
    return s > 1 ? (long)s * M * Cout : 0;
}

namespace {
int conv_args(GemmArgs& a, int& split_tile, const void* x, const void* w, const float* bias, const float* addvec, long addvec_ld,
              const void* residual, void* y, int B, int H, int W, int Cin, int Cout, int stride, int upsample2x,
              int out_f32, float* workspace, float* colstats, int k_order) {
    AE_REQUIRE(x && w && y, "ae_conv3x3_bf16: null pointer");
    AE_REQUIRE(k_order == 0 || k_order == 1, "ae_conv3x3_bf16: k_order must be 0 (tap, channel) or 1 (64-channel chunk, tap, channel)");
    AE_REQUIRE(k_order == 0 || (Cin % 64 == 0 && !upsample2x), "ae_conv3x3_bf16: the chunk-major K order needs Cin %% 64 == 0 and no upsampling (Cin=%d)", Cin);
    if (colstats) AE_REQUIRE(!out_f32 && Cout % 8 == 0 && (reinterpret_cast<uintptr_t>(colstats) & 15) == 0, "ae_conv3x3_bf16: column statistics need a bf16 output with Cout %% 8 == 0");
    AE_REQUIRE(B > 0 && H > 0 && W > 0, "ae_conv3x3_bf16: bad shape B=%d H=%d W=%d", B, H, W);
    AE_REQUIRE(Cin % 8 == 0, "ae_conv3x3_bf16: Cin=%d must be a multiple of 8", Cin);
    AE_REQUIRE(Cout % 4 == 0, "ae_conv3x3_bf16: Cout=%d must be a multiple of 4", Cout);
    AE_REQUIRE(stride == 1 || stride == 2, "ae_conv3x3_bf16: stride must be 1 or 2");
    AE_REQUIRE(upsample2x >= 0 && upsample2x <= 2, "ae_conv3x3_bf16: upsample2x must be 0, 1 (nearest) or 2 (zero-insert)");
    AE_REQUIRE(!(upsample2x && stride != 1), "ae_conv3x3_bf16: upsample2x requires stride 1");
    AE_REQUIRE(aligned16(x) && aligned16(w) && aligned16(y), "ae_conv3x3_bf16: pointers must be 16-byte aligned");
    const int Hv = upsample2x ? 2 * H : H, Wv = upsample2x ? 2 * W : W;
    const int Ho = (Hv + 2 - 3) / stride + 1, Wo = (Wv + 2 - 3) / stride + 1;
    a = GemmArgs{};
    a.A = (const bf16_t*)x; a.A2 = nullptr; a.W = (const bf16_t*)w; a.C = y;
    a.bias = bias; a.res = (const bf16_t*)residual; a.addvec = addvec;
    const int CinPad = (Cin + BK - 1) / BK * BK;
    a.M = B * Ho * Wo; a.N = Cout; a.K = 9 * CinPad; a.Ksplit = a.K;
    a.lda = 0; a.lda2 = 0; a.ldw = 9L * CinPad; a.ldc = Cout; a.ldr = Cout; a.ldav = addvec_ld > 0 ? addvec_ld : Cout;
    a.epi = EPI_NONE; a.out_f32 = out_f32; a.rows_per_batch = Ho * Wo;
    a.H = H; a.Wd = W; a.Cin = Cin; a.CinPad = CinPad; a.Ho = Ho; a.Wo = Wo; a.stride = stride; a.ups = upsample2x;
    a.a_bytes = (unsigned)((long)B * H * W * Cin * 2); a.a2_bytes = 0u; a.w_bytes = (unsigned)((long)Cout * 9 * CinPad * 2);
    AE_REQUIRE((long)B * H * W * Cin * 2 < (1L << 31) && (long)Cout * 9 * CinPad * 2 < (1L << 31), "ae_conv3x3_bf16: operands must be smaller than 2 GiB");
    const Plan plan = workspace ? make_plan(a.M, a.N, a.K, true) : Plan{0, 1};
    a.splitk = plan.splitk;
    split_tile = plan.tile;
    a.partial = workspace;
    a.colstats = colstats;
    a.kmajor = k_order;
    return 0;
}
}

extern "C" int ae_conv3x3_bf16(const void* x, const void* w, const float* bias, const float* addvec, long addvec_ld,
                               const void* residual, void* y, int B, int H, int W, int Cin, int Cout, int stride, int upsample2x,
                               int out_f32, float* workspace, float* colstats, int k_order, void* stream) {
    GemmArgs a;
    int split_tile;
    const int rc = conv_args(a, split_tile, x, w, bias, addvec, addvec_ld, residual, y, B, H, W, Cin, Cout, stride, upsample2x, out_f32, workspace, colstats, k_order);
    return rc ? rc : launch<A_CONV3>(a, (hipStream_t)stream, nullptr, split_tile);
}

extern "C" int ae_conv3x3_plan(int B, int H, int W, int Cin, int Cout, int stride, int upsample2x, int out_f32, int workspace, int colstats, int k_order, int* plan) {
    AE_REQUIRE(plan, "ae_conv3x3_plan: null plan");
    GemmArgs a;
    int split_tile;
    PlanReport r{};
    const int rc = conv_args(a, split_tile, kQueryPtr, kQueryPtr, nullptr, nullptr, 0, nullptr, kQueryPtr, B, H, W, Cin, Cout, stride, upsample2x, out_f32,
                             workspace ? kQueryF32 : nullptr, colstats ? kQueryF32 : nullptr, k_order);
    return plan_out(rc ? rc : launch<A_CONV3>(a, nullptr, &r, split_tile), r, plan);
}
```

anyedit_amd/ldm/modules/diffusionmodules/openaimodel.py:

```python
from abc import abstractmethod
import math

import torch
import torch.nn as nn

from anyedit_amd import ops
from anyedit_amd.ldm.util import exists
from anyedit_amd.ldm.modules.attention import SpatialTransformer
from anyedit_amd.ldm.modules.diffusionmodules.util import avg_pool_nd, conv_nd, linear, normalization, zero_module

BF16 = torch.bfloat16


class TimestepBlock(nn.Module):

    @abstractmethod
    def forward(self, x, emb):
        """Apply the module to `x` given `emb` timestep embeddings."""


class Feat:
    __slots__ = ("t", "B", "H", "W", "t2", "st", "st2")

    def __init__(self, t, B, H, W, t2=None, st=None, st2=None):
# ... 25 lines not shown
            if isinstance(layer, TimestepBlock):
                f = layer.rows(f, emb_silu)
            elif isinstance(layer, SpatialTransformer):
                x_st = f.st if f.t2 is None else None
                x = f.materialize()
                st = _stats_for(f.B, f.H, f.W, x.shape[1], x.device)
                f = Feat(layer.rows(x, f.B, f.H, f.W, context_rows=context_rows, kv_cache=kv_cache, colstats=x_st, out_colstats=st),
                         f.B, f.H, f.W, st=st)
            elif isinstance(layer, AttentionBlock):
                x_st = f.st if f.t2 is None else None
                f = Feat(layer.rows(f.materialize(), f.B, f.H * f.W, colstats=x_st), f.B, f.H, f.W)
            else:
                f = layer.rows(f)
        return f

    def forward(self, x, emb, context=None):
        for layer in self:
            if isinstance(layer, TimestepBlock):
                x = layer(x, emb)
            elif isinstance(layer, SpatialTransformer):
                x = layer(x, context)
            else:
                x = layer(x)
        return x


class Upsample(nn.Module):

    def __init__(self, channels, use_conv, dims=2, out_channels=None, padding=1):
        super().__init__()
        self.channels = channels
        self.out_channels = out_channels or channels
        self.use_conv = use_conv
        self.dims = dims
        if dims != 2:
            raise NotImplementedError("Upsample: only dims=2 (the 1-D / 3-D forms of openaimodel.py:108-112 have no caller in AnyEdit)")
        if use_conv:
            self.conv = conv_nd(dims, self.channels, self.out_channels, 3, padding=padding)

    def rows(self, f):
        if not self.use_conv:
            y, Ho, Wo = ops.resample2x_rows(f.materialize(), f.B, f.H, f.W)
            return Feat(y, f.B, Ho, Wo)
        Ho, Wo = self.conv.out_hw(f.H, f.W, upsample2x=True)
        st = _stats_for(f.B, Ho, Wo, self.out_channels, f.t.device)
        y, Ho, Wo = self.conv.rows(f.materialize(), f.B, f.H, f.W, upsample2x=True, colstats=st)
        return Feat(y, f.B, Ho, Wo, st=st)

    def forward(self, x):
        assert x.shape[1] == self.channels
        B, C, H, W = x.shape
        f = self.rows(Feat(ops.nchw_to_rows(x), B, H, W))
        return ops.rows_to_nchw(f.t, B, f.H, f.W, out_dtype=x.dtype)


class Downsample(nn.Module):

    def __init__(self, channels, use_conv, dims=2, out_channels=None, padding=1):
        super().__init__()
        self.channels = channels
        self.out_channels = out_channels or channels
        self.use_conv = use_conv
        self.dims = dims
        if dims != 2:
            raise NotImplementedError("Downsample: only dims=2 (the 1-D / 3-D forms of openaimodel.py:146 have no caller in AnyEdit)")
        if use_conv:
            self.op = conv_nd(dims, self.channels, self.out_channels, 3, stride=2, padding=padding)
        else:
            assert self.channels == self.out_channels
            self.op = avg_pool_nd(dims, kernel_size=2, stride=2)

    def rows(self, f):
        if not self.use_conv:
            y, Ho, Wo = self.op.rows(f.materialize(), f.B, f.H, f.W)
            return Feat(y, f.B, Ho, Wo)
        Ho, Wo = self.op.out_hw(f.H, f.W)
        st = _stats_for(f.B, Ho, Wo, self.out_channels, f.t.device)
        y, Ho, Wo = self.op.rows(f.materialize(), f.B, f.H, f.W, colstats=st)
        return Feat(y, f.B, Ho, Wo, st=st)

    def forward(self, x):
        assert x.shape[1] == self.channels
        B, C, H, W = x.shape
        f = self.rows(Feat(ops.nchw_to_rows(x), B, H, W))
        return ops.rows_to_nchw(f.t, B, f.H, f.W, out_dtype=x.dtype)


class ResBlock(TimestepBlock):

    def __init__(self, channels, emb_channels, dropout, out_channels=None, use_conv=False, use_scale_shift_norm=False,
                 dims=2, use_checkpoint=False, up=False, down=False):
        super().__init__()
        self.channels = channels
        self.emb_channels = emb_channels
        self.dropout = dropout
        self.out_channels = out_channels or channels
        self.use_conv = use_conv
        self.use_checkpoint = use_checkpoint
        self.use_scale_shift_norm = use_scale_shift_norm
        self.in_layers = nn.Sequential(normalization(channels), nn.SiLU(), conv_nd(dims, channels, self.out_channels, 3, padding=1))
        self.updown = up or down
        self.up, self.down = bool(up), bool(down) and not up
        if up:
            self.h_upd, self.x_upd = Upsample(channels, False, dims), Upsample(channels, False, dims)
        elif down:
            self.h_upd, self.x_upd = Downsample(channels, False, dims), Downsample(channels, False, dims)
        else:
            self.h_upd = self.x_upd = nn.Identity()
        self.emb_layers = nn.Sequential(nn.SiLU(), linear(emb_channels, 2 * self.out_channels if use_scale_shift_norm else self.out_channels))
        self.out_layers = nn.Sequential(normalization(self.out_channels), nn.SiLU(), nn.Dropout(p=dropout),
                                        zero_module(conv_nd(dims, self.out_channels, self.out_channels, 3, padding=1)))
        if self.out_channels == channels:
            self.skip_connection = nn.Identity()
        elif use_conv:
            self.skip_connection = conv_nd(dims, channels, self.out_channels, 3, padding=1)
        else:
            self.skip_connection = conv_nd(dims, channels, self.out_channels, 1)

    def rows(self, f, emb_silu):
        tape = ops._TAPE
        if self.use_checkpoint and tape is not None and tape.active:
            return Feat(tape.checkpoint(lambda: self._rows(f, emb_silu).t), f.B, f.H, f.W)
        return self._rows(f, emb_silu)

    def _rows(self, f, emb_silu):
        B, H, W = f.B, f.H, f.W
        if isinstance(emb_silu, EmbPack) and id(self) in emb_silu.offsets:
            off = emb_silu.offsets[id(self)]
            emb_out = emb_silu.all[:, off:off + self.emb_layers[1].out_features]
        else:
            silu = emb_silu.silu if isinstance(emb_silu, EmbPack) else emb_silu
            emb_out = self.emb_layers[1].rows(silu, out_f32=True)
        dev = f.t.device
        ssn = self.use_scale_shift_norm
        h = self.in_layers[0].rows(f.t, B, H * W, silu=True, x2=f.t2, colstats=f.st, colstats2=f.st2)
        whole = (lambda: f.t if f.t2 is None else ops.concat_channels(f.t, f.t2))
        Ho, Wo, xs = H, W, None
        if self.up:
            Ho, Wo = 2 * H, 2 * W
            xs, _, _ = ops.resample2x_rows(whole(), B, H, W)
        elif self.down:
            h, Ho, Wo = ops.resample2x_rows(h, B, H, W, down=True)
            xs, _, _ = ops.resample2x_rows(whole(), B, H, W, down=True)
        conv1, norm2 = self.in_layers[2], self.out_layers[0]
        st1 = _stats_for(B, Ho, Wo, self.out_channels, dev)
        if self.up:
            h, _, _ = conv1.rows(h, B, H, W, addvec=None if ssn else emb_out, upsample2x=True, colstats=st1)
        else:
            h, _, _ = conv1.rows(h, B, Ho, Wo, addvec=None if ssn else emb_out, colstats=st1)
        if ssn:
            h = ops.scale_shift_rows(norm2.rows(h, B, Ho * Wo, silu=False, colstats=st1), emb_out, B, Ho * Wo, silu=True)
        else:
            h = norm2.rows(h, B, Ho * Wo, silu=True, colstats=st1)
        if isinstance(self.skip_connection, nn.Identity):
            res = whole() if xs is None else xs
        elif self.skip_connection.kernel_size[0] == 1 and xs is None:
            res, _, _ = self.skip_connection.rows(f.t, B, H, W, a2=f.t2)
        else:
            res, _, _ = self.skip_connection.rows(whole() if xs is None else xs, B, Ho, Wo)
        st = _stats_for(B, Ho, Wo, self.out_channels, dev)
        y, _, _ = self.out_layers[3].rows(h, B, Ho, Wo, residual=res, colstats=st)
        return Feat(y, B, Ho, Wo, st=st)

    def forward(self, x, emb):
        B, C, H, W = x.shape
        f = self.rows(Feat(ops.nchw_to_rows(x), B, H, W), ops.silu_to_bf16(emb))
        return ops.rows_to_nchw(f.t, B, f.H, f.W, out_dtype=x.dtype)

    _forward = forward


class _QKVAttentionBase(nn.Module):

    def __init__(self, n_heads):
        super().__init__()
        self.n_heads = n_heads

    def _offsets(self, ch):
        raise NotImplementedError

    def rows(self, qkv, B, T):
        width = qkv.shape[1]
        assert width % (3 * self.n_heads) == 0
        ch = width // (3 * self.n_heads)
        (oq, ok, ov), hs = self._offsets(ch)
        st = (T * width, hs, width)
        return ops.attention(qkv[:, oq:], qkv[:, ok:], qkv[:, ov:], B, self.n_heads, T, T, ch, 1.0 / math.sqrt(ch), st, st, st).reshape(B * T, self.n_heads * ch)

    def forward(self, qkv):
        bs, width, length = qkv.shape
        y = self.rows(ops.nchw_to_rows(qkv.reshape(bs, width, length, 1)), bs, length)
        return ops.rows_to_nchw(y, bs, length, 1, out_dtype=qkv.dtype).reshape(bs, -1, length)


class QKVAttentionLegacy(_QKVAttentionBase):

    def _offsets(self, ch):
        return (0, ch, 2 * ch), 3 * ch


class QKVAttention(_QKVAttentionBase):

    def _offsets(self, ch):
        return (0, self.n_heads * ch, 2 * self.n_heads * ch), ch


class AttentionBlock(nn.Module):

    def __init__(self, channels, num_heads=1, num_head_channels=-1, use_checkpoint=False, use_new_attention_order=False):
        super().__init__()
        self.channels = channels
        if num_head_channels == -1:
            self.num_heads = num_heads
        else:
            assert channels % num_head_channels == 0, f"q,k,v channels {channels} is not divisible by num_head_channels {num_head_channels}"
            self.num_heads = channels // num_head_channels
        self.use_checkpoint = use_checkpoint
        self.norm = normalization(channels)
        self.qkv = conv_nd(1, channels, channels * 3, 1)
        self.attention = QKVAttention(self.num_heads) if use_new_attention_order else QKVAttentionLegacy(self.num_heads)
        self.proj_out = zero_module(conv_nd(1, channels, channels, 1))

    def rows(self, x, B, T, colstats=None):
        h = self.norm.rows(x, B, T, silu=False, colstats=colstats)
        return self.proj_out.rows(self.attention.rows(self.qkv.rows(h), B, T), residual=x)

    def forward(self, x):
        b, c = x.shape[:2]
        T = int(x.numel() // (b * c))
        y = self.rows(ops.nchw_to_rows(x.reshape(b, c, T, 1)), b, T)
        return ops.rows_to_nchw(y, b, T, 1, out_dtype=x.dtype).reshape(x.shape)

    _forward = forward


class UNetModel(nn.Module):

    def __init__(self, image_size, in_channels, model_channels, out_channels, num_res_blocks, attention_resolutions,
                 dropout=0, channel_mult=(1, 2, 4, 8), conv_resample=True, dims=2, num_classes=None, use_checkpoint=False,
                 use_fp16=False, num_heads=-1, num_head_channels=-1, num_heads_upsample=-1, use_scale_shift_norm=False,
                 resblock_updown=False, use_new_attention_order=False, use_spatial_transformer=False, transformer_depth=1,
                 context_dim=None, n_embed=None, legacy=True, disable_self_attentions=None, num_attention_blocks=None,
                 disable_middle_self_attn=False, use_linear_in_transformer=False):
        super().__init__()
        if use_spatial_transformer:
            assert context_dim is not None, "use_spatial_transformer needs context_dim (openaimodel.py:474-475)"
        if context_dim is not None:
            assert use_spatial_transformer, "a cross-attention context_dim needs use_spatial_transformer (openaimodel.py:477-478)"
            if not isinstance(context_dim, int):
                context_dim = list(context_dim)
        if dims != 2:
            raise NotImplementedError("dims != 2: the 1-D / 3-D UNets of openaimodel.py have no caller in AnyEdit")
        if num_classes is not None and not isinstance(num_classes, int) and num_classes != "continuous":
            raise ValueError(f"num_classes must be None, an int or 'continuous' (openaimodel.py:533-540), got {num_classes!r}")
        if num_heads_upsample == -1:
            num_heads_upsample = num_heads
        if num_heads == -1:
            assert num_head_channels != -1, "Either num_heads or num_head_channels has to be set"
        if num_head_channels == -1:
            assert num_heads != -1, "Either num_heads or num_head_channels has to be set"
        self.image_size = image_size
        self.in_channels = in_channels
        self.model_channels = model_channels
        self.out_channels = out_channels
        if isinstance(num_res_blocks, int):
            self.num_res_blocks = len(channel_mult) * [num_res_blocks]
        else:
            if len(num_res_blocks) != len(channel_mult):
                raise ValueError("provide num_res_blocks either as an int or as a per-level list")
            self.num_res_blocks = list(num_res_blocks)
        if disable_self_attentions is not None:
            assert len(disable_self_attentions) == len(channel_mult)
        if num_attention_blocks is not None:
            assert len(num_attention_blocks) == len(self.num_res_blocks)
        self.attention_resolutions = attention_resolutions
        self.dropout = dropout
        self.channel_mult = channel_mult
        self.conv_resample = conv_resample
        self.num_classes = num_classes
        self.use_checkpoint = use_checkpoint
        self.dtype = torch.float32
        self.num_heads = num_heads
        self.num_head_channels = num_head_channels
        self.num_heads_upsample = num_heads_upsample
        self.predict_codebook_ids = n_embed is not None

        def heads_for(ch, nh):
            if num_head_channels == -1:
                return nh, ch // nh
            return ch // num_head_channels, num_head_channels

        def make_st(ch, nh, level, is_middle=False):
            if not use_spatial_transformer:
                d_h = num_head_channels if (num_head_channels != -1 or legacy) else ch // num_heads
                return AttentionBlock(ch, use_checkpoint=use_checkpoint, num_heads=nh, num_head_channels=d_h, use_new_attention_order=use_new_attention_order)
            n_h, d_h = heads_for(ch, nh)
            if legacy:
                d_h = ch // n_h
            dsa = disable_middle_self_attn if is_middle else (disable_self_attentions[level] if exists(disable_self_attentions) else False)
            return SpatialTransformer(ch, n_h, d_h, depth=transformer_depth, context_dim=context_dim, disable_self_attn=dsa,
                                      use_linear=use_linear_in_transformer, use_checkpoint=use_checkpoint)

        time_embed_dim = model_channels * 4
        self.time_embed = nn.Sequential(linear(model_channels, time_embed_dim), nn.SiLU(), linear(time_embed_dim, time_embed_dim))
        if num_classes is not None:
            self.label_emb = nn.Embedding(num_classes, time_embed_dim) if isinstance(num_classes, int) else nn.Linear(1, time_embed_dim)
        self.input_blocks = nn.ModuleList([TimestepEmbedSequential(conv_nd(dims, in_channels, model_channels, 3, padding=1))])
        self._feature_size = model_channels
        input_block_chans = [model_channels]
        ch = model_channels
        ds = 1
        for level, mult in enumerate(channel_mult):
            for nr in range(self.num_res_blocks[level]):
                layers = [ResBlock(ch, time_embed_dim, dropout, out_channels=mult * model_channels, dims=dims,
                                   use_checkpoint=use_checkpoint, use_scale_shift_norm=use_scale_shift_norm)]
# ... 140 lines not shown
```

anyedit_amd/ops.py:

```python
import torch

import collections
import ctypes
import os
import threading

from ._lib import lib, check as _check

BF16 = torch.bfloat16
EPI_NONE, EPI_GELU, EPI_GEGLU, EPI_SILU, EPI_RELU = 0, 1, 2, 3, 4


def _s():
    return torch.cuda.current_stream().cuda_stream


def _p(t):
    return None if t is None else t.data_ptr()


_live = threading.local()


def _tmp(t):
    if t is not None:
        lst = getattr(_live, "t", None)
        if lst is None:
            lst = _live.t = []
        lst.append(t)
    return t


def check(rc, what=""):
    lst = getattr(_live, "t", None)
    if lst:
        lst.clear()
    _check(rc, what)


def weights_token(*tensors):
    return tuple((t.data_ptr(), _version_of(t)) for t in tensors if t is not None)


def _version_of(t):
    try:
        return t._version
    except RuntimeError:
        return -1


def cache_stale(mod, attr, *tensors):
    tok = weights_token(*tensors)
    if getattr(mod, attr, None) is None or mod.__dict__.get(attr + "_tok") != tok:
        mod.__dict__[attr + "_tok"] = tok
        return True
    return False


def _chk(t, dtype, name, dims=None):
    if not t.is_cuda:
        raise ValueError(f"{name}: expected a GPU tensor (anyedit_amd has no CPU path)")
    if t.dtype != dtype:
        raise TypeError(f"{name}: expected {dtype}, got {t.dtype}")
    if dims is not None and t.dim() != dims:
        raise ValueError(f"{name}: expected {dims} dims, got shape {tuple(t.shape)}")


def _dense(t, dtype, name, dims=None):
    _chk(t, dtype, name, dims)
    return t.contiguous()


def _target(t, dtype, shape, name):
    _chk(t, dtype, name)
    if tuple(t.shape) != tuple(shape) or not t.is_contiguous():
        raise ValueError(f"{name}: expected a contiguous {tuple(shape)} tensor, got shape {tuple(t.shape)} strides {t.stride()}")
    return t


def pack_linear(w):
    return w.detach().reshape(w.shape[0], -1).to(BF16).contiguous()


def pack_conv3x3(w, cin_pad=None, k_order=0):
    cout, cin = w.shape[0], w.shape[1]
    cin_pad = cin_pad or ((cin + 63) // 64 * 64)
    wp = torch.zeros(cout, 3, 3, cin_pad, dtype=BF16, device=w.device)
    wp[..., :cin] = w.detach().permute(0, 2, 3, 1).to(BF16)
    if k_order == 1:
        wp = wp.reshape(cout, 9, cin_pad // 64, 64).permute(0, 2, 1, 3)
    return wp.reshape(cout, 9 * cin_pad).contiguous()


def pack_conv3x3_taps8(w):
    cout, cin = w.shape[0], w.shape[1]
    assert cin == 8 and tuple(w.shape[2:]) == (3, 3)
    wp = torch.zeros(cout, 128, dtype=BF16, device=w.device)
    wp[:, :72] = w.detach().permute(0, 2, 3, 1).reshape(cout, 72).to(BF16)
    return wp.contiguous()


def pack_conv3x3_up2(w):
    cout, cin = w.shape[0], w.shape[1]
    assert tuple(w.shape[2:]) == (3, 3) and cin % 64 == 0
    return up2_weight_sums(w).reshape(4, cout, 4 * cin).to(BF16).contiguous()


def up2_weight_sums(w):
    cout, cin = w.shape[0], w.shape[1]
    w32 = w.detach().float()
    sets = {(0, 0): (0,), (0, 1): (1, 2), (1, 0): (0, 1), (1, 1): (2,)}
    out = torch.empty(4, cout, 4, cin, dtype=torch.float32, device=w.device)
    for py in range(2):
        for px in range(2):
            for i in range(2):
                for j in range(2):
                    acc = torch.zeros(cout, cin, dtype=torch.float32, device=w.device)
                    for ky in sets[(py, i)]:
                        for kx in sets[(px, j)]:
                            acc = acc + w32[:, :, ky, kx]
                    out[2 * py + px, :, 2 * i + j] = acc
    return out


_UP2_SUBPIXEL = os.environ.get("AE_UP2_SUBPIXEL", "1") != "0"


def up2_subpixel_ok(Cin, Cout, H, W, want_stats):
    return _UP2_SUBPIXEL and Cin % 64 == 0 and Cout % 8 == 0 and (not want_stats or (H * W) % 32 == 0) and not (_TAPE is not None and _TAPE.active)


def conv3x3_up2(x, w4, bias, B, H, W, out=None, colstats=None):
    _chk(x, BF16, "conv3x3_up2.x", 2)
    _chk(w4, BF16, "conv3x3_up2.w4", 3)
    Cin, Cout = x.shape[1], w4.shape[1]
    if x.shape[0] != B * H * W or not x.is_contiguous():
        raise ValueError(f"conv3x3_up2: x must be contiguous [B*H*W, Cin] = [{B * H * W}, Cin], got {tuple(x.shape)}")
    if tuple(w4.shape) != (4, Cout, 4 * Cin) or not w4.is_contiguous():
        raise ValueError(f"conv3x3_up2: packed weight must be a contiguous [4, Cout, {4 * Cin}] tensor, got {tuple(w4.shape)}")
    if out is None:
        out = torch.empty(B * 4 * H * W, Cout, dtype=BF16, device=x.device)
    if colstats is not None:
        _chk(colstats, torch.float32, "conv3x3_up2.colstats", 3)
        if tuple(colstats.shape) != (B * 4 * H * W // 32, Cout, 2) or not colstats.is_contiguous() or (H * W) % 32:
            raise ValueError(f"conv3x3_up2: colstats must be a contiguous [{B * 4 * H * W // 32}, {Cout}, 2] fp32 buffer (H * W % 32 == 0)")
    check(lib.ae_conv3x3_up2_bf16(_p(x), _p(w4), _p(bias), _p(out), B, H, W, Cin, Cout, _p(colstats), _s()), "ae_conv3x3_up2_bf16")
    return out, 2 * H, 2 * W


_STEM_IM2COL = os.environ.get("AE_STEM_IM2COL", "1") != "0"


def stem_im2col_ok(Cin, stride, upsample2x):
    return _STEM_IM2COL and Cin == 8 and stride == 1 and not upsample2x and not (_TAPE is not None and _TAPE.active)


def im2col3x3_c8(x, B, H, W):
    _chk(x, BF16, "im2col3x3_c8.x", 2)
    if tuple(x.shape) != (B * H * W, 8) or not x.is_contiguous():
        raise ValueError(f"im2col3x3_c8: x must be contiguous [{B * H * W}, 8], got {tuple(x.shape)}")
    y = torch.empty(B * H * W, 128, dtype=BF16, device=x.device)
    check(lib.ae_im2col3x3_c8_bf16(_p(x), _p(y), B, H, W, _s()), "ae_im2col3x3_c8_bf16")
    return y


_CONV_KMAJOR = int(os.environ.get("AE_CONV_KMAJOR", "2"))


Plan = collections.namedtuple("Plan", "BM BN AMODE WAVES_M WAVES_N GLDS WAVES_K STAGES CS LAB WA XE grid threads lds splitk reduce colstats rowpanel")
_PLANS = {}


def _plan(query, *args):
    key = (query,) + args
    if key not in _PLANS:
        buf = (ctypes.c_int * len(Plan._fields))()
        _PLANS[key] = Plan(*buf) if getattr(lib, query)(*args, buf) == 0 else None
    return _PLANS[key]


def gemm_plan(M, N, K, epilogue=EPI_NONE, Ksplit=0, out_f32=False, colstats=False, ln_mode=0):
    return _plan("ae_gemm_plan", M, N, K, epilogue, Ksplit, int(out_f32), int(colstats), ln_mode)


def conv_plan(B, H, W, Cin, Cout, stride=1, upsample2x=0, out_f32=False, colstats=False, k_order=0):
    return _plan("ae_conv3x3_plan", B, H, W, Cin, Cout, stride, int(upsample2x), int(out_f32), 1, int(colstats), int(k_order))


def up2_plan(B, H, W, Cin, Cout, colstats=False):
    return _plan("ae_conv3x3_up2_plan", B, H, W, Cin, Cout, int(colstats))


def plan_label(p):
    return f"{p.BM}x{p.BN}" + (",ring3" if p.STAGES == 3 else "") + (",splitK" if p.splitk > 1 else "")


def conv_k_order(M, Cin, Cout, stride=1, upsample2x=False):
    if _CONV_KMAJOR == 0 or upsample2x or Cin % 64 != 0 or (_TAPE is not None and _TAPE.active):
        return 0
    p = conv_plan(M, 1, 1, Cin, Cout, stride)
    if p is None or not p.GLDS:
        return 0
    if _CONV_KMAJOR == 3:
        return 1
    label = plan_label(p)
    if _CONV_KMAJOR == 4:
        return 1 if label in ("192x320", "128x128") else 0
    return 1 if (label == "192x320" or (_CONV_KMAJOR >= 2 and label == "192x320,splitK")) else 0


def pack_geglu(w, b):
    inner = w.shape[0] // 2
    assert inner % 16 == 0
    a, g = w[:inner], w[inner:]
    wp = torch.stack([a.reshape(inner // 16, 16, -1), g.reshape(inner // 16, 16, -1)], dim=1).reshape(2 * inner, -1)
    bp = torch.stack([b[:inner].reshape(-1, 16), b[inner:].reshape(-1, 16)], dim=1).reshape(-1)
    return wp.detach().to(BF16).contiguous(), bp.detach().float().contiguous()


def pack_ff2_fused(w2):
    C, H = w2.shape
    assert C == 320 and H % 32 == 0
    dev = w2.device
    i = torch.arange(C, device=dev)
    i5 = i & 31
    col = 32 * (i >> 5) + 8 * ((i5 & 15) >> 2) + 4 * (i5 >> 4) + (i5 & 3)
    pos = torch.arange(4, device=dev)
    e = torch.arange(8, device=dev)
    gp = (pos[None, :] - 2 * ((i[:, None] & 15) >> 2)) & 3
    u = 16 * (e >> 2)[None, None, :] + 4 * gp[:, :, None] + (e & 3)[None, None, :]
    wf = w2.detach().float()[col]
    img = wf.reshape(C, H // 32, 32).permute(1, 0, 2)
    idx = u.reshape(1, C, 32).expand(H // 32, C, 32)
    return torch.gather(img, 2, idx).to(BF16).contiguous()


def ff_fused_ok(M, C, H):
    return not (_TAPE is not None and _TAPE.active) and bool(lib.ae_ff_fused_supported(M, C, H))


def ff_fused(x, gamma, beta, eps, w1, b1, w2img, b2, residual=None, out=None, w3=None, b3=None, residual3=None, colstats=None):
    _chk(x, BF16, "ff_fused.x", 2)
    _chk(w1, BF16, "ff_fused.w1", 2)
    _chk(w2img, BF16, "ff_fused.w2img", 3)
    _chk(gamma, torch.float32, "ff_fused.gamma", 1)
    _chk(beta, torch.float32, "ff_fused.beta", 1)
    _chk(b1, torch.float32, "ff_fused.b1", 1)
    M, C = x.shape
    H = w1.shape[0] // 2
    if w1.shape[1] != C or tuple(w2img.shape) != (H // 32, C, 32) or not w2img.is_contiguous() or x.stride(1) != 1 or w1.stride(1) != 1:
        raise ValueError(f"ff_fused: x {tuple(x.shape)}, w1 {tuple(w1.shape)}, w2img {tuple(w2img.shape)} do not fit together")
    if b1.numel() != 2 * H or gamma.numel() != C or beta.numel() != C:
        raise ValueError("ff_fused: b1 / gamma / beta sizes")
    if b2 is not None:
        _chk(b2, torch.float32, "ff_fused.b2", 1)
    if residual is not None:
        _chk(residual, BF16, "ff_fused.residual", 2)
    if w3 is not None:
        _chk(w3, BF16, "ff_fused.w3", 2)
        if tuple(w3.shape) != (C, C) or w3.stride(1) != 1:
            raise ValueError("ff_fused: w3 must be [C, C] with unit inner stride")
        if b3 is not None:
            _chk(b3, torch.float32, "ff_fused.b3", 1)
        if residual3 is not None:
            _chk(residual3, BF16, "ff_fused.residual3", 2)
        if colstats is not None:
            _chk(colstats, torch.float32, "ff_fused.colstats", 3)
            if tuple(colstats.shape) != ((M + 31) // 32, C, 2) or not colstats.is_contiguous():
                raise ValueError(f"ff_fused: colstats must be a contiguous [{(M + 31) // 32}, {C}, 2] fp32 buffer")
    elif b3 is not None or residual3 is not None or colstats is not None:
        raise ValueError("ff_fused: b3 / residual3 / colstats go with w3")
    if out is None:
        out = torch.empty(M, C, dtype=BF16, device=x.device)
    _chk(out, BF16, "ff_fused.out", 2)
    check(lib.ae_ff_fused_bf16(_p(x), x.stride(0), _p(gamma), _p(beta), float(eps), _p(w1), w1.stride(0), _p(b1), _p(w2img), _p(b2), _p(residual),
                               residual.stride(0) if residual is not None else 0, _p(w3), w3.stride(0) if w3 is not None else 0, _p(b3), _p(residual3),
                               residual3.stride(0) if residual3 is not None else 0, _p(colstats), _p(out), out.stride(0), M, C, H, _s()), "ae_ff_fused_bf16")
    return out


def colstats_buffer(M, N, device):
    return torch.empty((M + 31) // 32, N, 2, dtype=torch.float32, device=device)


_GN_COLSTATS = os.environ.get("AE_GN_COLSTATS", "1") != "0"


def want_colstats(HW):
    return _GN_COLSTATS and HW > 256 and HW % 32 == 0 and not (_TAPE is not None and _TAPE.active)


def gemm(a, w, bias=None, residual=None, addvec=None, rows_per_batch=0, epilogue=EPI_NONE, out_f32=False, a2=None, out=None, colstats=None,
         rowstats=None):
    if rowstats is not None:
        if _TAPE is not None and _TAPE.active:
            raise ValueError("gemm: row statistics are not recorded on the training tape (ln_fold_plan is False while it records)")
        if addvec is not None or a2 is not None or out_f32 or colstats is not None or epilogue != EPI_NONE:
            raise ValueError("gemm: rowstats goes with a plain bf16 GEMM (+bias, +residual) only")
        return _gemm_ln(a, w, bias, residual, EPI_NONE, out, rowstats, None, None, 0.0)
    if _TAPE is not None and _TAPE.active:
        return _TAPE.gemm(a, w, bias=bias, residual=residual, addvec=addvec, rows_per_batch=rows_per_batch, epilogue=epilogue, out_f32=out_f32, a2=a2, out=out)
    _chk(a, BF16, "gemm.a", 2)
    _chk(w, BF16, "gemm.w", 2)
    M, K1 = a.shape
    N, K = w.shape
    if a.stride(1) != 1 or w.stride(1) != 1:
        raise ValueError("gemm: a and w must have unit inner stride")
    K2 = 0
    if a2 is not None:
        _chk(a2, BF16, "gemm.a2", 2)
        K2 = a2.shape[1]
        if a2.shape[0] != M or a2.stride(1) != 1:
            raise ValueError("gemm: a2 shape mismatch")
    if K1 + K2 != K:
        raise ValueError(f"gemm: K mismatch: a has {K1}+{K2} columns, w has {K}")
    n_out = N // 2 if epilogue == EPI_GEGLU else N
    if out is None:
        out = torch.empty(M, n_out, dtype=torch.float32 if out_f32 else BF16, device=a.device)
    if bias is not None:
        _chk(bias, torch.float32, "gemm.bias", 1)
    if residual is not None:
        _chk(residual, BF16, "gemm.residual", 2)
    if addvec is not None:
        _chk(addvec, torch.float32, "gemm.addvec", 2)
    if colstats is not None:
        _chk(colstats, torch.float32, "gemm.colstats", 3)
        if tuple(colstats.shape) != ((M + 31) // 32, n_out, 2) or not colstats.is_contiguous():
            raise ValueError(f"gemm: colstats must be a contiguous [{(M + 31) // 32}, {n_out}, 2] fp32 buffer")
    if a2 is None and addvec is None and not out_f32 and _rowpanel_ok(a, w, out, residual, M, N, K, epilogue):
        return _ln_gemm_launch(a, w, bias, residual, None, None, 0.0, epilogue, out, M, N, K, colstats)
    check(lib.ae_gemm_bf16(_p(a), a.stride(0), _p(a2), a2.stride(0) if a2 is not None else 0, K1, _p(w), w.stride(0),
                           _p(out), out.stride(0), M, N, K, _p(bias), _p(residual),
                           residual.stride(0) if residual is not None else 0, _p(addvec),
                           addvec.stride(0) if addvec is not None else 0, rows_per_batch, epilogue,
                           1 if out_f32 else 0, _p(colstats), _s()), "ae_gemm_bf16")
    return out


_LN_FOLD = os.environ.get("AE_LN_FOLD", "1") != "0"


def ln_fold_plan(M, N, K, epilogue, mode):
    if not _LN_FOLD or (_TAPE is not None and _TAPE.active):
        return False
    p = gemm_plan(M, N, K, epilogue, ln_mode=mode)
    return p is not None and (_ROWPANEL or not p.rowpanel)


def rowstats_buffer(M, N, device):
    return torch.empty(M, N // 64, 2, dtype=torch.float32, device=device)


def pack_ln_fold(w, bias, gamma, beta, geglu=False):
    wf = w.detach().float().reshape(w.shape[0], -1).contiguous()
    g, be = gamma.detach().float(), beta.detach().float()
    c = linear_f32(be[None, :].contiguous(), wf, bias)[0]
    wp = wf * g[None, :]
    if geglu:
        wq, c = pack_geglu(wp, c)
    else:
        wq = wp.to(BF16).contiguous()
    s = linear_f32(torch.ones(1, wq.shape[1], dtype=torch.float32, device=wq.device), wq.float())[0]
    return wq, s.contiguous(), c.contiguous()


def _gemm_ln(a, w, bias, residual, epilogue, out, rowstats_out, ln_stats, ln_colsum, eps):
    _chk(a, BF16, "gemm_ln.a", 2)
    _chk(w, BF16, "gemm_ln.w", 2)
    M, K = a.shape
    N = w.shape[0]
    if w.shape[1] != K or a.stride(1) != 1 or w.stride(1) != 1:
        raise ValueError(f"gemm_ln: a is [{M}, {K}], w is {tuple(w.shape)}; both need unit inner stride")
    n_out = N // 2 if epilogue == EPI_GEGLU else N
    if out is None:
        out = torch.empty(M, n_out, dtype=BF16, device=a.device)
    _chk(out, BF16, "gemm_ln.out", 2)
    if bias is not None:
        _chk(bias, torch.float32, "gemm_ln.bias", 1)
    if residual is not None:
        _chk(residual, BF16, "gemm_ln.residual", 2)
    nparts = 0
    if rowstats_out is not None:
        if rowstats_out.dtype != torch.float32 or tuple(rowstats_out.shape) != (M, N // 64, 2) or not rowstats_out.is_contiguous():
            raise ValueError(f"gemm: rowstats must be a contiguous fp32 [{M}, {N // 64}, 2] buffer (rowstats_buffer)")
    else:
        if ln_stats.dtype != torch.float32 or ln_stats.dim() != 3 or ln_stats.shape[0] != M or ln_stats.shape[2] != 2 or not ln_stats.is_contiguous() \
                or ln_stats.shape[1] * 64 != K:
            raise ValueError(f"gemm_ln: statistics must be the producer's contiguous fp32 [{M}, {K // 64}, 2] buffer, got {tuple(ln_stats.shape)}")
        _chk(ln_colsum, torch.float32, "gemm_ln.s", 1)
        if bias is None or bias.numel() != N or ln_colsum.numel() != N:
            raise ValueError("gemm_ln: s and c must be fp32 [N]")
        nparts = ln_stats.shape[1]
    return _gemm_ln_launch(a, w, bias, residual, epilogue, out, M, N, K, rowstats_out, ln_stats, nparts, ln_colsum, float(eps))


def _gemm_ln_launch(a, w, bias, residual, epilogue, out, M, N, K, rowstats_out, ln_stats, nparts, ln_colsum, eps):
    check(lib.ae_gemm_ln_bf16(_p(a), a.stride(0), _p(w), w.stride(0), _p(out), out.stride(0), M, N, K, _p(bias), _p(residual),
                              residual.stride(0) if residual is not None else 0, epilogue, _p(rowstats_out), _p(ln_stats), nparts,
                              _p(ln_colsum), eps, _s()), "ae_gemm_ln_bf16")
    return out


def gemm_ln(x, rowstats, wq, s, c, eps, residual=None, epilogue=EPI_NONE, out=None):
    return _gemm_ln(x, wq, c, residual, epilogue, out, None, rowstats, s, eps)


_ROWPANEL = os.environ.get("AE_GEMM_ROWPANEL", "1") != "0"


def _rowpanel_ok(a, w, out, residual, M, N, K, epilogue):
    if not _ROWPANEL or not lib.ae_ln_gemm_supported(M, N, K, epilogue):
        return False
    ts = [a, w, out] + ([residual] if residual is not None else [])
    ld_max = max(t.stride(0) for t in ts if t is not w)
    return all(t.data_ptr() % 16 == 0 and t.stride(0) % 8 == 0 and t.stride(1) == 1 for t in ts) and N * w.stride(0) * 2 < 2 ** 31 \
        and (M + 192) * ld_max * 2 < 2 ** 31


def _ln_gemm_launch(a, w, bias, residual, gamma, beta, eps, epilogue, out, M, N, K, colstats=None):
    check(lib.ae_ln_gemm_bf16(_p(a), a.stride(0), _p(w), w.stride(0), _p(out), out.stride(0), M, N, K, _p(bias), _p(residual),
                              residual.stride(0) if residual is not None else 0, _p(gamma), _p(beta), float(eps), epilogue,
                              _p(colstats), _s()),
          "ae_ln_gemm_bf16")
    return out


def ln_gemm(x, gamma, beta, eps, w, bias=None, residual=None, epilogue=EPI_NONE, out=None, colstats=None):
    if not (_TAPE is not None and _TAPE.active):
        _chk(x, BF16, "ln_gemm.x", 2)
        _chk(w, BF16, "ln_gemm.w", 2)
        M, K = x.shape
        N = w.shape[0]
        if w.shape[1] == K and x.stride(1) == 1 and w.stride(1) == 1:
            n_out = N // 2 if epilogue == EPI_GEGLU else N
            o = out if out is not None else torch.empty(M, n_out, dtype=BF16, device=x.device)
            if _rowpanel_ok(x, w, o, residual, M, N, K, epilogue):
                _chk(gamma, torch.float32, "ln_gemm.gamma", 1)
                _chk(beta, torch.float32, "ln_gemm.beta", 1)
                if bias is not None:
                    _chk(bias, torch.float32, "ln_gemm.bias", 1)
                if residual is not None:
                    _chk(residual, BF16, "ln_gemm.residual", 2)
                return _ln_gemm_fused(x, w, bias, residual, gamma, beta, eps, epilogue, o, M, N, K, colstats)
    return gemm(layernorm(x, gamma, beta, eps), w, bias, residual=residual, epilogue=epilogue, out=out, colstats=colstats)


def conv3x3(x, w, bias, B, H, W, addvec=None, residual=None, stride=1, upsample2x=False, out_f32=False, out=None, colstats=None, k_order=0):
    if _TAPE is not None and _TAPE.active:
        if k_order:
            raise ValueError("conv3x3: the tape records convolutions on tap-major packed weights (k_order=0)")
        return _TAPE.conv3x3(x, w, bias, B, H, W, addvec=addvec, residual=residual, stride=stride, upsample2x=upsample2x, out_f32=out_f32, out=out)
    _chk(x, BF16, "conv3x3.x", 2)
    _chk(w, BF16, "conv3x3.w", 2)
    Cin = x.shape[1]
    Cout = w.shape[0]
    if x.shape[0] != B * H * W or not x.is_contiguous():
        raise ValueError(f"conv3x3: x must be contiguous [B*H*W, Cin] = [{B * H * W}, Cin], got {tuple(x.shape)}")
    if w.shape[1] != 9 * ((Cin + 63) // 64 * 64):
        raise ValueError(f"conv3x3: packed weight has K={w.shape[1]}, expected {9 * ((Cin + 63) // 64 * 64)}")
    Hv, Wv = (2 * H, 2 * W) if upsample2x else (H, W)
    Ho, Wo = (Hv - 1) // stride + 1, (Wv - 1) // stride + 1
    if out is None:
        out = torch.empty(B * Ho * Wo, Cout, dtype=torch.float32 if out_f32 else BF16, device=x.device)
    if residual is not None:
        _chk(residual, BF16, "conv3x3.residual", 2)
        if residual.shape != (B * Ho * Wo, Cout) or not residual.is_contiguous():
            raise ValueError("conv3x3: residual shape mismatch")
    nws = lib.ae_conv3x3_workspace_floats(B, H, W, Cin, Cout, stride, int(upsample2x))
    ws = torch.empty(nws, dtype=torch.float32, device=x.device) if nws > 0 else None
    if colstats is not None:
        _chk(colstats, torch.float32, "conv3x3.colstats", 3)
        if tuple(colstats.shape) != ((B * Ho * Wo + 31) // 32, Cout, 2) or not colstats.is_contiguous():
            raise ValueError(f"conv3x3: colstats must be a contiguous [{(B * Ho * Wo + 31) // 32}, {Cout}, 2] fp32 buffer")
    check(lib.ae_conv3x3_bf16(_p(x), _p(w), _p(bias), _p(addvec), addvec.stride(0) if addvec is not None else 0, _p(residual),
                              _p(out), B, H, W, Cin, Cout, stride, int(upsample2x), 1 if out_f32 else 0, _p(ws), _p(colstats), int(k_order), _s()),
          "ae_conv3x3_bf16")
    return out, Ho, Wo


_GN_COUNTERS = {}


_GN_TAIL = os.environ.get("AE_GN_TAIL") == "1"


def _gn_counters(device, B):
    if not _GN_TAIL:
        return None
    key = (device, torch.cuda.current_stream(device).cuda_stream)
    c = _GN_COUNTERS.get(key)
    if c is None or c.numel() < B:
        c = _GN_COUNTERS[key] = torch.zeros(max(B, 256), dtype=torch.int32, device=device)
    return c


def groupnorm(x, gamma, beta, B, HW, eps, silu=False, groups=32, x2=None, out=None, stat_out=None, colstats=None, colstats2=None):
    if _TAPE is not None and _TAPE.active:
        return _TAPE.groupnorm(x, gamma, beta, B, HW, eps, silu=silu, groups=groups, x2=x2, out=out)
    _chk(x, BF16, "groupnorm.x", 2)
    C1 = x.shape[1]
    C = C1 + (x2.shape[1] if x2 is not None else 0)
    if not x.is_contiguous() or (x2 is not None and not x2.is_contiguous()):
        raise ValueError("groupnorm: inputs must be contiguous")
    if out is None:
        out = torch.empty(B * HW, C, dtype=BF16, device=x.device)
    if colstats is not None and (x2 is None) != (colstats2 is None):
        colstats = colstats2 = None
    if colstats is not None:
        for t, c, n in ((colstats, C1, "colstats"), (colstats2, C - C1, "colstats2")):
            if t is not None and (t.dtype != torch.float32 or tuple(t.shape) != (B * HW // 32, c, 2) or not t.is_contiguous() or HW % 32):
                raise ValueError(f"groupnorm: {n} must be a contiguous fp32 [{B * HW // 32}, {c}, 2] buffer (HW % 32 == 0), got {tuple(t.shape)}")
    nws = int(lib.ae_groupnorm_workspace_floats(B, HW, C, groups))
    ws = torch.empty(nws, dtype=torch.float32, device=x.device)
    check(lib.ae_groupnorm_nhwc_bf16(_p(x), _p(x2), C1, _p(gamma), _p(beta), _p(out), B, HW, C, groups, eps,
                                     1 if silu else 0, _p(ws), _p(_gn_counters(x.device, B)), _p(stat_out), _p(colstats), _p(colstats2), _s()),
          "ae_groupnorm_nhwc_bf16")
    return out


def layernorm(x, gamma, beta, eps=1e-5, out=None):
    if _TAPE is not None and _TAPE.active:
        return _TAPE.layernorm(x, gamma, beta, eps=eps, out=out)
    _chk(x, BF16, "layernorm.x", 2)
    if not x.is_contiguous():
        raise ValueError("layernorm: x must be contiguous")
    M, C = x.shape
    if out is None:
        out = torch.empty_like(x)
    check(lib.ae_layernorm_bf16(_p(x), _p(gamma), _p(beta), _p(out), M, C, eps, _s()), "ae_layernorm_bf16")
    return out


def attention(q, k, v, B, H, Nq, Nk, D, scale, q_strides, k_strides, v_strides, out=None, rel_h=None, rel_w=None,
              kH=0, kW=0, key_mask=None, out_scale=None, accumulate=False, seg2=None, lse=None, lse2=None, o_strides=None):
    if _TAPE is not None and _TAPE.active:
        return _TAPE.attention(q, k, v, B, H, Nq, Nk, D, scale, q_strides, k_strides, v_strides, out=out, key_mask=key_mask,
                               out_scale=out_scale, accumulate=accumulate, seg2=seg2, rel_h=rel_h)
    if out is None:
        out = torch.empty(B, Nq, H * D, dtype=BF16, device=q.device)
    if o_strides is None:
        o_strides = (Nq * H * D, D, H * D)
    if seg2 is not None:
        k2, v2, Nk2, k2_strides, v2_strides, scale2 = seg2
        seg_args = (_p(k2), _p(v2), Nk2, *k2_strides, *v2_strides, _p(scale2))
    else:
        seg_args = (None, None, 0, 0, 0, 0, 0, 0, 0, None)
    check(lib.ae_attn_fwd_bf16(_p(q), _p(k), _p(v), _p(out), B, H, Nq, Nk, D, *q_strides, *k_strides, *v_strides, *o_strides,
                               scale, _p(rel_h), _p(rel_w), kH, kW, _p(key_mask), _p(out_scale), 1 if accumulate else 0,
                               *seg_args, _p(lse), _p(lse2), _s()), "ae_attn_fwd_bf16")
    return out


_FP8_WS = {}


def attention_fp8(q, k, v, B, H, Nq, Nk, D, scale, q_strides, k_strides, v_strides, out=None, rel_h=None, rel_w=None, kH=0, kW=0):
    for t, n in ((q, "q"), (k, "k"), (v, "v")):
        _chk(t, BF16, "attention_fp8." + n)
    if out is None:
        out = torch.empty(B, Nq, H * D, dtype=BF16, device=q.device)
    need = lib.ae_attn_fp8_workspace_bytes(B, H, Nq, Nk, D)
    if need <= 0:
        raise ValueError(f"attention_fp8: unsupported sizes B={B} H={H} Nq={Nq} Nk={Nk} D={D}")
    key = (q.device, torch.cuda.current_stream(q.device).cuda_stream)
    ws = _FP8_WS.get(key)
    if ws is None or ws.numel() < need:
        ws = _FP8_WS[key] = torch.empty(need, dtype=torch.uint8, device=q.device)
    if rel_h is not None:
        _chk(rel_h, torch.float32, "attention_fp8.rel_h")
        _chk(rel_w, torch.float32, "attention_fp8.rel_w")
    check(lib.ae_attn_fwd_fp8(_p(q), _p(k), _p(v), _p(out), B, H, Nq, Nk, D, *q_strides, *k_strides, *v_strides, Nq * H * D, D, H * D,
                              float(scale), _p(rel_h), _p(rel_w), kH, kW, _p(ws), ws.numel(), _s()), "ae_attn_fwd_fp8")
    return out


def attention_bwd(q, k, v, dout, lse, B, H, Nq, Nk, D, scale, q_strides, k_strides, v_strides, dq, dk, dv, dq_strides,
                  dk_strides, dv_strides, out_scale=None, accumulate_dq=False, out=None, split_dkv=True, o_strides=None, delta=None):
    if delta is None:
        delta = torch.empty(B, H, Nq, dtype=torch.float32, device=q.device)
    if o_strides is None:
        o_strides = (Nq * H * D, D, H * D)
    zero3 = (0, 0, 0)
    ws = None
    if dk is not None and split_dkv:
        nws = lib.ae_attn_bwd_workspace_floats(B, H, Nq, Nk, D)
        if nws > 0:
            ws = torch.empty(nws, dtype=torch.float32, device=q.device)
    check(lib.ae_attn_bwd_bf16(_p(q), _p(k), _p(v), _p(dout), _p(out), _p(lse), _p(delta), _p(dq), _p(dk), _p(dv), B, H, Nq, Nk, D,
                               *q_strides, *k_strides, *v_strides, *o_strides, *dq_strides, *(dk_strides if dk is not None else zero3),
                               *(dv_strides if dv is not None else zero3), scale, _p(out_scale), 1 if accumulate_dq else 0, _p(ws), _s()),
          "ae_attn_bwd_bf16")
    return delta


def attention_bhnd(q, k, v, scale=None, key_mask=None):
    _chk(q, BF16, "attention.q", 3)
    BH, Nq, D = q.shape
    Nk = k.shape[1]
    q, k, v = q.contiguous(), k.contiguous(), v.contiguous()
    out = torch.empty(BH, Nq, D, dtype=BF16, device=q.device)
    scale = scale if scale is not None else D ** -0.5
    check(lib.ae_attn_fwd_bf16(_p(q), _p(k), _p(v), _p(out), BH, 1, Nq, Nk, D, Nq * D, 0, D, Nk * D, 0, D, Nk * D, 0, D,
                               Nq * D, 0, D, scale, None, None, 0, 0, _p(key_mask), None, 0, None, None, 0, 0, 0, 0, 0, 0, 0, None, None, None, _s()),
          "ae_attn_fwd_bf16")
    return out


ACT_QUICK_GELU, ACT_GELU = 0, 1


def _attention_short(name, fn, q, k, v, extra, B, H, N, D, scale, q_strides, k_strides, v_strides, out, max_n=None, dims=None):
    for t, n in ((q, "q"), (k, "k"), (v, "v")):
        _chk(t, BF16, f"{name}.{n}")
    if max_n is not None and not 1 <= N <= max_n:
        raise ValueError(f"{name}: sequence length {N}; {fn.__name__} takes between 1 and {max_n}")
    if dims is not None and D not in dims:
        raise ValueError(f"{name}: head_dim {D} is not built (supported: {', '.join(map(str, dims))})")
    ptrs = [_p(q), _p(k), _p(v)]
    if extra is not None:
        t, dtype, label, shape = extra
        _chk(t, dtype, f"{name}.{label}", 3)
        if tuple(t.shape) != shape or not t.is_contiguous():
            raise ValueError(f"{name}: {label} must be a contiguous {list(shape)} tensor, got {tuple(t.shape)}")
        ptrs.append(_p(t))
    if out is None:
        out = torch.empty(B, N, H * D, dtype=BF16, device=q.device)
    _chk(out, BF16, f"{name}.out")
    if out.numel() != B * N * H * D or not out.is_contiguous():
        raise ValueError(f"{name}: out must be a contiguous [{B}, {N}, {H * D}] buffer")
    check(fn(*ptrs, _p(out), B, H, N, D, *q_strides, *k_strides, *v_strides, N * H * D, D, H * D, float(scale), _s()), fn.__name__)
# ... 1717 lines not shown


def rowsum_f32(x):
    x = x.contiguous()
    out = torch.empty(x.shape[0], dtype=torch.float32, device=x.device)
    check(lib.ae_rowsum_f32(_p(x), _p(out), x.shape[0], x.shape[1], _s()), "ae_rowsum_f32")
    return out


def scatter_add_rows(src, code, dst):
    code = code.to(torch.int32).contiguous()
    check(lib.ae_scatter_add_rows_f32(_p(_tmp(src.contiguous())), _p(code), _p(dst), src.shape[0], src.shape[1], dst.shape[0], _s()),
          "ae_scatter_add_rows_f32")
    return dst


def task_gate_bwd(probs, top1, dgate, Wg):
    B, E = probs.shape
    dte = torch.empty(B, Wg.shape[1], dtype=torch.float32, device=probs.device)
    check(lib.ae_task_gate_bwd(_p(_tmp(probs.contiguous())), _p(_tmp(top1.contiguous())), _p(_tmp(dgate.float().contiguous())), _p(_tmp(Wg.float().contiguous())),
                               B, Wg.shape[1], E, _p(dte), _s()), "ae_task_gate_bwd")
    return dte


def task_gate_wgrad(probs, top1, dgate, task_emb, edit_code):
    B, E = probs.shape
    n_tasks, Dt = task_emb.shape
    probs32, top1c, dg32 = probs.float().contiguous(), top1.contiguous(), dgate.float().contiguous()
    te32, code = task_emb.float().contiguous(), edit_code.long().contiguous()
    dW = torch.empty(E, Dt, dtype=torch.float32, device=probs.device)
    db = torch.empty(E, dtype=torch.float32, device=probs.device)
    check(lib.ae_task_gate_wgrad(_p(probs32), _p(top1c), _p(dg32), _p(te32), _p(code), B, n_tasks, Dt, E, _p(dW), _p(db), _s()),
          "ae_task_gate_wgrad")
    return dW, db


_EXPERT_KV_WS = {}


def _experts_i32(experts):
    return experts.to(torch.int32).contiguous()


def expert_kv(x, W, experts, tokens):
    E, N, Dc = W.shape
    B = x.shape[0] // tokens
    assert x.dtype == BF16 and x.is_contiguous() and W.dtype == torch.float32 and W.is_contiguous() and x.shape == (B * tokens, Dc)
    ex = _tmp(_experts_i32(experts))
    y = torch.empty(B * tokens, N, dtype=BF16, device=x.device)
    check(lib.ae_expert_kv_fwd(_p(x), _p(W), _p(ex), _p(y), B, tokens, N, Dc, E, _s()), "ae_expert_kv_fwd")
    return y


def expert_kv_dgrad(dy, W, experts, tokens):
    E, N, Dc = W.shape
    B = dy.shape[0] // tokens
    assert dy.dtype == BF16 and dy.is_contiguous() and dy.shape == (B * tokens, N)
    S = lib.ae_expert_kv_dgrad_slices(N)
    key = (dy.device, torch.cuda.current_stream(dy.device).cuda_stream)
    need = S * B * tokens * Dc
    ws = _EXPERT_KV_WS.get(key)
    if ws is None or ws.numel() < need:
        ws = _EXPERT_KV_WS[key] = torch.empty(need, dtype=torch.float32, device=dy.device)
    ex = _tmp(_experts_i32(experts))
    dx = torch.empty(B * tokens, Dc, dtype=BF16, device=dy.device)
    check(lib.ae_expert_kv_dgrad(_p(dy), _p(W), _p(ex), _p(dx), B, tokens, N, Dc, E, _p(ws), _s()), "ae_expert_kv_dgrad")
    return dx


def expert_kv_wgrad(dy, x, experts, tokens, n_experts, out=None):
    B = dy.shape[0] // tokens
    N, Dc = dy.shape[1], x.shape[1]
    assert dy.dtype == BF16 and x.dtype == BF16 and dy.is_contiguous() and x.is_contiguous()
    if out is None:
        out = torch.empty(n_experts, N, Dc, dtype=torch.float32, device=dy.device)
    assert out.dtype == torch.float32 and out.is_contiguous() and out.numel() == n_experts * N * Dc
    ex = _tmp(_experts_i32(experts))
    check(lib.ae_expert_kv_wgrad(_p(dy), _p(x), _p(ex), _p(out), B, tokens, N, Dc, n_experts, _s()), "ae_expert_kv_wgrad")
    return out


class OpProfiler:

    def __init__(self):
        self.records = []

    def __enter__(self):
        global _PROF
        _PROF = self
        return self

    def __exit__(self, *a):
        global _PROF
        _PROF = None
        torch.cuda.synchronize()

    def summary(self, by_shape=False):
        agg = {}
        for label, flops, nbytes, e0, e1, nlaunch in self.records:
            if not by_shape:
                label = label.split("|")[0]
            ms = e0.elapsed_time(e1)
            a = agg.setdefault(label, {"calls": 0, "launches": 0, "ms": 0.0, "flops": 0.0, "bytes": 0.0})
            a["calls"] += 1
            a["launches"] += nlaunch
            a["ms"] += ms
            a["flops"] += flops
            a["bytes"] += nbytes
        for a in agg.values():
            a["avg_us"] = 1e3 * a["ms"] / a["calls"]
            a["tflops"] = a["flops"] / (a["ms"] * 1e-3) / 1e12 if a["ms"] > 0 else 0.0
            a["gbps"] = a["bytes"] / (a["ms"] * 1e-3) / 1e9 if a["ms"] > 0 else 0.0
        return agg


_PROF = None


def _wrap_profiled(fn, label_fn):
    def wrapped(*args, **kwargs):
        if _PROF is None:
            return fn(*args, **kwargs)
        e0, e1 = torch.cuda.Event(enable_timing=True), torch.cuda.Event(enable_timing=True)
        e0.record()
        out = fn(*args, **kwargs)
        e1.record()
        lab = label_fn(out, *args, **kwargs)
        if lab is not None:
            _PROF.records.append((lab[0], lab[1], lab[2], e0, e1, lab[3] if len(lab) > 3 else 1))
        return out
    wrapped.__doc__ = fn.__doc__
    return wrapped


def _gemm_label(_r, a, w, bias=None, residual=None, addvec=None, rows_per_batch=0, epilogue=EPI_NONE, out_f32=False, a2=None, **_):
    if _.get("rowstats") is not None:
        return None
    M, (N, K) = a.shape[0], w.shape
    nb = 2 * (M * K + N * K) + _r.numel() * _r.element_size() + (2 * M * N if residual is not None else 0)
    if a2 is None and addvec is None and not out_f32 and _rowpanel_ok(a, w, _r, residual, M, N, K, epilogue):
        return f"gemm_rowpanel_kernel<K=320{',geglu' if epilogue == EPI_GEGLU else ''}>|M={M} N={N}", 2.0 * M * N * K, nb
    p = gemm_plan(M, N, K, epilogue, a.shape[1] if a2 is not None else 0, out_f32, _.get("colstats") is not None)
    return f"gemm_kernel<{plan_label(p)},dense>|M={M} N={N} K={K}", 2.0 * M * N * K, float(nb), 1 + p.colstats


def _conv_label(_r, x, w, bias, B, H, W, addvec=None, residual=None, stride=1, upsample2x=False, out_f32=False, **_):
    y = _r[0]
    M, Cout, Cin = y.shape[0], w.shape[0], x.shape[1]
    nb = 2 * (x.numel() + 9 * Cin * Cout) + y.numel() * y.element_size() + (2 * y.numel() if residual is not None else 0)
    p = conv_plan(B, H, W, Cin, Cout, stride, upsample2x, out_f32, _.get("colstats") is not None, _.get("k_order", 0))
    return f"gemm_kernel<{plan_label(p)},conv3x3>|M={M} Cin={Cin} Cout={Cout} s{stride}{'u' if upsample2x else ''}", 2.0 * M * Cout * 9 * Cin, float(nb), 1 + p.reduce + p.colstats


def _attn_label(_r, q, k, v, B, H, Nq, Nk, D, *a, **kw):
    fast = D in (40, 80, 160) and kw.get("key_mask") is None and os.environ.get("AE_ATTN_FAST", "1") != "0" and \
        (D != 160 or os.environ.get("AE_ATTN_FAST160", "1") != "0") and \
        (kw.get("rel_h") is None or (D == 80 and ((kw.get("kW") == 64 and Nk % 64 == 0) or (kw.get("kH", 99) <= 16 and kw.get("kW", 99) <= 16))))
    seg2 = kw.get("seg2")
    skv = fast and kw.get("rel_h") is None and Nk <= 128 and (seg2 is None or seg2[2] <= 64) and os.environ.get("AE_ATTN_SKV", "1") != "0"
    name = ("attn_fast_kernel" if fast else "attn_kernel")
    return f"{name}<D={D}{',shortKV' if skv else ''}>|Nq={Nq} Nk={Nk}", 4.0 * B * H * Nq * Nk * D, 2.0 * B * H * D * (2 * Nq + 2 * Nk)


def _attn8_label(_r, q, k, v, B, H, Nq, Nk, D, *a, **kw):
    return f"fp8_attn_kernel<D={D}>+prepare|Nq={Nq} Nk={Nk}", 4.0 * B * H * Nq * Nk * D, 2.0 * B * H * D * (2 * Nq + 2 * Nk)


def _gn_label(_r, x, gamma, beta, B, HW, eps, silu=False, groups=32, x2=None, **_):
    nl = 2 if _.get("colstats") is not None and ((x2 is None) == (_.get("colstats2") is None)) else (1 if HW <= 256 and os.environ.get("AE_GN_SLAB", "1") != "0" else (2 if _GN_TAIL else 3))
    return f"groupnorm(stats+apply)|rows={_r.shape[0]} C={_r.shape[1]}", 0.0, 2.0 * _r.numel() * 2, nl


def _ln_label(_r, x, *a, **_):
    return f"layernorm_kernel|M={_r.shape[0]} C={_r.shape[1]}", 0.0, 2.0 * _r.numel() * 2


def _ln_gemm_label(_r, x, w, bias, residual, gamma, beta, eps, epilogue, o, M, N, K, colstats=None):
    nb = 2 * (M * K + N * K) + _r.numel() * 2 + (2 * M * N if residual is not None else 0)
    return f"gemm_rowpanel_kernel<K=320,LN{',geglu' if epilogue == EPI_GEGLU else ''}>|M={M} N={N}", 2.0 * M * N * K, nb


def _gemm_ln_label(_r, a, w, bias, residual, epilogue, out, M, N, K, rowstats_out, ln_stats, nparts, ln_colsum, eps):
    nb = 2 * (M * K + N * K) + _r.numel() * 2 + (2 * M * N if residual is not None else 0)
    tag = "rowstats" if rowstats_out is not None else "LNfold"
    p = gemm_plan(M, N, K, epilogue, ln_mode=1 if rowstats_out is not None else 2)
    if p.rowpanel:
        return f"gemm_rowpanel_kernel<K=320,{tag}{',geglu' if epilogue == EPI_GEGLU else ''}>|M={M} N={N}", 2.0 * M * N * K, nb
    return f"gemm_kernel<{plan_label(p)},dense,{tag}>|M={M} N={N} K={K}", 2.0 * M * N * K, float(nb)


def _up2_label(_r, x, w4, bias, B, H, W, **_):
    y = _r[0]
    Cout, Cin = w4.shape[1], x.shape[1]
    tl = plan_label(up2_plan(B, H, W, Cin, Cout, _.get("colstats") is not None))
    nb = 2 * (x.numel() + 16 * Cin * Cout) + 2 * y.numel()
    return f"gemm_kernel<{tl},conv3x3,up2x2>|M={y.shape[0]} Cin={Cin} Cout={Cout}", 2.0 * y.shape[0] * Cout * 4 * Cin, float(nb)


conv3x3_up2 = _wrap_profiled(conv3x3_up2, _up2_label)
ff_fused = _wrap_profiled(ff_fused, lambda _r, x, gamma, beta, eps, w1, b1, w2img, b2, residual=None, out=None, w3=None, b3=None, residual3=None, colstats=None: (
    f"ff_fused_kernel<C=320{',proj_out' if w3 is not None else ''}>|M={x.shape[0]} H={w1.shape[0] // 2}",
    2.0 * x.shape[0] * x.shape[1] * (3 * (w1.shape[0] // 2) + (x.shape[1] if w3 is not None else 0)),
    float(2 * (x.numel() * (2 + (residual is not None and residual is not x) + (residual3 is not None)) + w1.numel() + w2img.numel() + (w3.numel() if w3 is not None else 0))),
    2 if colstats is not None else 1))
_ln_gemm_fused = _wrap_profiled(_ln_gemm_launch, _ln_gemm_label)
_gemm_ln_launch = _wrap_profiled(_gemm_ln_launch, _gemm_ln_label)
gemm = _wrap_profiled(gemm, _gemm_label)
attention_fp8 = _wrap_profiled(attention_fp8, _attn8_label)
conv3x3 = _wrap_profiled(conv3x3, _conv_label)
attention = _wrap_profiled(attention, _attn_label)
groupnorm = _wrap_profiled(groupnorm, _gn_label)
layernorm = _wrap_profiled(layernorm, _ln_label)
expert_kv = _wrap_profiled(expert_kv, lambda _r, x, W, experts, tokens: (
    f"expert_kv_fwd_kernel|rows={x.shape[0]} N={W.shape[1]} Dc={W.shape[2]}", 2.0 * x.shape[0] * W.shape[1] * W.shape[2], 4.0 * (x.shape[0] // tokens) * W.shape[1] * W.shape[2]))
expert_kv_dgrad = _wrap_profiled(expert_kv_dgrad, lambda _r, dy, W, experts, tokens: (
    f"expert_kv_dgrad_kernel|rows={dy.shape[0]} N={W.shape[1]} Dc={W.shape[2]}", 2.0 * dy.shape[0] * W.shape[1] * W.shape[2], 4.0 * (dy.shape[0] // tokens) * W.shape[1] * W.shape[2]))
expert_kv_wgrad = _wrap_profiled(expert_kv_wgrad, lambda _r, dy, x, experts, tokens, n_experts, out=None: (
    f"expert_kv_wgrad_kernel|rows={dy.shape[0]} N={dy.shape[1]} Dc={x.shape[1]} E={n_experts}", 2.0 * dy.shape[0] * dy.shape[1] * x.shape[1], 4.0 * n_experts * dy.shape[1] * x.shape[1]))
hed_stem = _wrap_profiled(hed_stem, lambda _r, x, norm, w, bias, out=None: (
    f"hed_stem_kernel<{'u8' if x.dtype == torch.uint8 else 'f32'}>|M={_r[0].shape[0]} C1={_r[0].shape[1]}", 2.0 * 27 * _r[0].numel(),
    float(x.numel() * x.element_size() + 2 * _r[0].numel())))
relu_ = _wrap_profiled(relu_, lambda _r, x: (f"relu_bf16_kernel|n={x.numel()}", 0.0, 4.0 * x.numel()))
hed_tail = _wrap_profiled(hed_tail, lambda _r, y, wp, bp, B, H, W, pool=True, proj=None, pooled=None: (
    f"hed_tail_kernel<{'pool' if pool else 'last'}>|M={y.shape[0]} C={y.shape[1]}", 2.0 * y.numel(),
    float(2 * y.numel() + 4 * _r[0].numel() + (2 * _r[1].numel() if pool else 0))))
hed_fuse = _wrap_profiled(hed_fuse, lambda _r, sides, invert=True, out=None, logits=None, want_logits=False: (
    f"hed_fuse_kernel|B={sides[0].shape[0]} {sides[0].shape[-2]}x{sides[0].shape[-1]}", 0.0,
    float(4 * sum(s.numel() for s in sides) + sides[0].numel() * (1 + 4 * (want_logits or logits is not None)))))
dpt_reassemble = _wrap_profiled(dpt_reassemble, lambda _r, prod, bias, B, gh, gw, k, out=None: (
    f"dpt_reassemble_kernel<k={k}>|M={_r.shape[0]} oc={_r.shape[1]}", 0.0, 6.0 * _r.numel()))
dpt_resize = _wrap_profiled(dpt_resize, lambda _r, x, B, h, w, H, W, addend=None, out=None, relu_out=None, want_relu=False: (
    f"dpt_resize_kernel<{'add' if addend is not None else 'plain'}{'+relu' if want_relu or relu_out is not None else ''}>|{h}x{w}->{H}x{W} C={x.shape[1]}", 0.0,
    float(2 * x.numel() + 2 * B * H * W * x.shape[1] * (1 + (addend is not None) + (want_relu or relu_out is not None)))))
dpt_relu = _wrap_profiled(dpt_relu, lambda _r, x, out=None: (f"dpt_relu_kernel|n={x.numel()}", 0.0, 4.0 * x.numel()))
dpt_tail = _wrap_profiled(dpt_tail, lambda _r, y, wp, bp, B, H, W, out=None: (
    f"dpt_tail_kernel|M={y.shape[0]} C={y.shape[1]}", 2.0 * y.numel(), float(2 * y.numel() + 4 * y.shape[0])))
depth_resize_minmax = _wrap_profiled(depth_resize_minmax, lambda _r, depth, H, W, out=None, minmax=None: (
    f"depth_resize_minmax_kernel|B={depth.shape[0]} {depth.shape[1]}x{depth.shape[2]}->{H}x{W}", 0.0, float(4 * depth.numel() + 4 * _r[0].numel()), 2))
depth_colorize = _wrap_profiled(depth_colorize, lambda _r, depth, minmax, table, out=None: (
    f"depth_colorize_kernel|B={depth.shape[0]} {depth.shape[1]}x{depth.shape[2]}", 0.0, 7.0 * depth.numel()))
dwconv = _wrap_profiled(dwconv, lambda _r, x, w, bias, B, H, W, residual=None, out=None: (
    f"dwconv_rows_kernel<k={int(w.shape[0] ** 0.5 + 0.5)}{',res' if residual is not None else ''}>|B={B} {H}x{W} C={x.shape[1]}", 2.0 * w.shape[0] * x.numel(),
    float(2 * x.numel() * (2 + (residual is not None and residual is not x)) + 4 * w.numel())))
patch2_rows = _wrap_profiled(patch2_rows, lambda _r, x, B, H, W, out=None: (
    f"patch2_rows_kernel|B={B} {H}x{W} C={x.shape[1]}", 0.0, 4.0 * _r[0].numel()))
layernorm_rows_nchw = _wrap_profiled(layernorm_rows_nchw, lambda _r, x, gamma, beta, eps, B, H, W, out=None, rows=None, want_rows=False: (
    f"layernorm_rows_nchw_kernel{'<+rows>' if want_rows or rows is not None else ''}|B={B} {H}x{W} C={x.shape[1]}", 0.0,
    float(x.numel() * (2 + 4 + 2 * (want_rows or rows is not None)))))
ppm_pool = _wrap_profiled(ppm_pool, lambda _r, x, B, H, W, scales, out=None: (
    f"ppm_pool_kernel<{len(tuple(scales))} scales>|B={B} {H}x{W} C={x.shape[1]}", 0.0, float(2 * x.numel() * len(tuple(scales)) + 2 * _r.numel())))
resize_concat = _wrap_profiled(resize_concat, lambda _r, sources, dst, B, H, W, addend=None: (
    f"resize_concat_kernel<{len(sources)} sources{',add' if addend is not None else ''}>|->{H}x{W} ld={dst.shape[1]}", 0.0,
    float(sum(2 * s[0].numel() + 2 * B * H * W * s[0].shape[-1] for s in sources) + (2 * addend.numel() if addend is not None else 0))))
seg_argmax = _wrap_profiled(seg_argmax, lambda _r, logits, ncls, B, h, w, mid, out_size=None, palette=None, labels=None, colours=None: (
    f"seg_argmax_kernel<{'identity' if out_size is None or tuple(out_size) == tuple(mid) else 'two stages'}{',palette' if palette is not None else ''}>|{h}x{w}->{mid[0]}x{mid[1]} "
    f"ncls={ncls}", 0.0, float(4 * B * h * w * ncls + B * (out_size or mid)[0] * (out_size or mid)[1] * (4 if palette is not None else 1))))
```

include/anyedit_hip.h:

```cpp
#ifndef ANYEDIT_HIP_H
#define ANYEDIT_HIP_H

#ifdef __cplusplus
extern "C" {
#endif

#define AE_OK 0
#define AE_ERR_ARG (-1)
#define AE_ERR_LAUNCH (-2)
#define AE_ERR_UNSUPPORTED (-3)

#define AE_EPI_NONE 0
#define AE_EPI_GELU 1
#define AE_EPI_GEGLU 2
#define AE_EPI_SILU 3
#define AE_EPI_RELU 4

int ae_version(void);
const char* ae_last_error(void);
int ae_device_arch(char* buf, int n);
int ae_device_info(int* cus, long* hbm_bytes, int* clock_khz);

int ae_gemm_bf16(const void* A, long lda, const void* A2, long lda2, int Ksplit, const void* W, long ldw, void* C, long ldc,
                 int M, int N, int K, const float* bias, const void* residual, long ldr, const float* addvec, long addvec_ld,
                 int rows_per_batch, int epilogue, int out_f32, float* colstats, void* stream);

int ae_ln_gemm_supported(int M, int N, int K, int epilogue);
int ae_ln_gemm_bf16(const void* A, long lda, const void* W, long ldw, void* C, long ldc, int M, int N, int K, const float* bias,
                    const void* residual, long ldr, const float* ln_gamma, const float* ln_beta, float ln_eps, int epilogue,
                    float* colstats , void* stream);

int ae_gemm_ln_plan(int M, int N, int K, int epilogue, int mode);
int ae_gemm_ln_bf16(const void* A, long lda, const void* W, long ldw, void* C, long ldc, int M, int N, int K, const float* bias,
                    const void* residual, long ldr, int epilogue, float* rowstats_out, const float* ln_stats, int ln_parts,
                    const float* ln_colsum, float ln_eps, void* stream);

int ae_ff_fused_supported(int M, int C, int H);
int ae_ff_fused_bf16(const void* X, long ldx, const float* ln_gamma, const float* ln_beta, float ln_eps, const void* W1, long ldw1, const float* b1,
                     const void* W2img, const float* b2, const void* residual, long ldr, const void* W3, long ldw3, const float* b3,
                     const void* residual3, long ldr3, float* colstats, void* Y, long ldy, int M, int C, int H, void* stream);

long ae_conv3x3_workspace_floats(int B, int H, int W, int Cin, int Cout, int stride, int upsample2x);
int ae_conv3x3_bf16(const void* x, const void* w, const float* bias, const float* addvec, long addvec_ld, const void* residual,
                    void* y, int B, int H, int W, int Cin, int Cout, int stride, int upsample2x, int out_f32, float* workspace,
                    float* colstats , int k_order, void* stream);

int ae_conv3x3_up2_bf16(const void* x, const void* w4, const float* bias, void* y, int B, int H, int W, int Cin, int Cout,
                        float* colstats, void* stream);

#define AE_PLAN_INTS 19
int ae_gemm_plan(int M, int N, int K, int epilogue, int Ksplit, int out_f32, int colstats, int ln_mode, int* plan);
int ae_conv3x3_plan(int B, int H, int W, int Cin, int Cout, int stride, int upsample2x, int out_f32, int workspace, int colstats, int k_order,
                    int* plan);
int ae_conv3x3_up2_plan(int B, int H, int W, int Cin, int Cout, int colstats, int* plan);

int ae_groupnorm_rows_per_chunk(int HW, int C);
long ae_groupnorm_workspace_floats(int B, int HW, int C, int groups);
int ae_groupnorm_nhwc_bf16(const void* x, const void* x2, int C1, const float* gamma, const float* beta, void* y, int B, int HW,
                           int C, int groups, float eps, int act, float* workspace, int* counters, float* stat_out,
                           const float* colstats, const float* colstats2, void* stream);

int ae_layernorm_bf16(const void* x, const float* gamma, const float* beta, void* y, int M, int C, float eps, void* stream);

int ae_attn_fwd_bf16(const void* q, const void* k, const void* v, void* out, int B, int H, int Nq, int Nk, int D,
                     long q_sb, long q_sh, long q_sn, long k_sb, long k_sh, long k_sn, long v_sb, long v_sh, long v_sn,
                     long o_sb, long o_sh, long o_sn, float scale, const float* rel_h, const float* rel_w, int kH, int kW,
                     const unsigned char* key_mask, const float* out_scale, int accumulate, const void* k2, const void* v2,
                     int Nk2, long k2_sb, long k2_sh, long k2_sn, long v2_sb, long v2_sh, long v2_sn, const float* scale2,
                     float* lse, float* lse2, void* stream);
long ae_attn_fp8_workspace_bytes(int B, int H, int Nq, int Nk, int D);
int ae_attn_fwd_fp8(const void* q, const void* k, const void* v, void* out, int B, int H, int Nq, int Nk, int D, long q_sb, long q_sh,
                    long q_sn, long k_sb, long k_sh, long k_sn, long v_sb, long v_sh, long v_sn, long o_sb, long o_sh, long o_sn,
                    float scale, const float* rel_h, const float* rel_w, int kH, int kW, void* workspace, long workspace_bytes,
                    void* stream);
long ae_attn_bwd_workspace_floats(int B, int H, int Nq, int Nk, int D);
int ae_attn_bwd_bf16(const void* q, const void* k, const void* v, const void* dout, const void* out, const float* lse, float* delta, void* dq,
                     void* dk, void* dv, int B, int H, int Nq, int Nk, int D, long q_sb, long q_sh, long q_sn, long k_sb,
                     long k_sh, long k_sn, long v_sb, long v_sh, long v_sn, long o_sb, long o_sh, long o_sn, long dq_sb,
                     long dq_sh, long dq_sn, long dk_sb, long dk_sh, long dk_sn, long dv_sb, long dv_sh, long dv_sn,
                     float scale, const float* out_scale, int accumulate_dq, float* workspace, void* stream);
long ae_groupnorm_bwd_workspace_floats(int B, int HW, int C, int groups);
int ae_groupnorm_bwd_nhwc_bf16(const void* x, const void* x2, int C1, const float* gamma, const float* beta, const void* dy,
                               void* dx, void* dx2, int B, int HW, int C, int groups, float eps, int act, float* workspace,
                               int* counters, const float* stat_in, int accumulate, void* stream);
int ae_layernorm_bwd_bf16(const void* x, const float* gamma, const void* dy, void* dx, float* row_stat, int M, int C, float eps,
                          int accumulate, void* stream);
int ae_layernorm_param_grad_f32(const void* x, const void* dy, const float* row_stat, float* dgamma, float* dbeta, int M, int C,
                                void* stream);
int ae_add_bf16(const void* a, const void* b, void* y, long n, void* stream);
int ae_axpy_bf16(const void* a, const void* b, float alpha, void* y, long n, void* stream);
int ae_geglu_fwd_bf16(const void* h, void* y, long M, int F, void* stream);
int ae_geglu_bwd_bf16(const void* h, const void* dy, void* dh, long M, int F, void* stream);
int ae_sumpool2x2_bf16(const void* x, void* y, int B, int H, int W, int C, void* stream);
int ae_colsum_bf16_f32(const void* x, float* out, int M, int N, long ld, void* stream);
int ae_mse_grad_f32(const float* pred, const float* target, float* out, long n, float loss_scale, void* stream);
int ae_adamw_f32(float* param, const float* grad, float* exp_avg, float* exp_avg_sq, long n, float lr, float beta1, float beta2,
                 float eps, float weight_decay, int step, float grad_scale, void* stream);
int ae_rowsum_f32(const float* x, float* out, int rows, long n, void* stream);
int ae_scatter_add_rows_f32(const float* src, const int* code, float* dst, int B, int D, int n_rows, void* stream);
int ae_task_gate_bwd(const float* probs, const int* top1, const float* dgate, const float* Wg, int B, int Dt, int E, float* dte,
                     void* stream);
int ae_task_gate_wgrad(const float* probs, const int* top1, const float* dgate, const float* task_emb, const long* edit_code, int B,
                       int n_tasks, int Dt, int E, float* dWg, float* dbg, void* stream);

int ae_expert_kv_fwd(const void* x, const float* W, const int* experts, void* y, int B, int T, int N, int Dc, int E, void* stream);
int ae_expert_kv_dgrad_slices(int N);
int ae_expert_kv_dgrad(const void* dy, const float* W, const int* experts, void* dx, int B, int T, int N, int Dc, int E, float* partial,
                       void* stream);
int ae_expert_kv_wgrad(const void* dy, const void* x, const int* experts, float* dW, int B, int T, int N, int Dc, int E, void* stream);

int ae_transpose_last2(const void* in, void* out, int B, int X, int Y, int Xpad, int in_bf16, int out_bf16, void* stream);
int ae_concat_channels_bf16(const void* a, int Ca, const void* b, int Cb, void* y, long rows, void* stream);
int ae_im2col3x3_c8_bf16(const void* x, void* y, int B, int H, int W, void* stream);
int ae_split_channels_bf16(const void* y, int Ca, int Cb, void* a, void* b, long rows, int accumulate_a, int accumulate_b, void* stream);
int ae_timestep_embedding(const long* t_i64, const float* t_f32, void* out_bf16, float* out_f32, int B, int dim, float max_period,
                          void* stream);
int ae_ddim_step_f32(const float* x, const float* eps, const float* noise, float* x_prev, float* pred_x0, float* e_out, long n,
                     int branches, float s0, float s1, float sqrt_one_minus_at, float sqrt_at, float sqrt_a_prev, float dir_coef,
                     float sigma_t, float temperature, void* stream);
int ae_plms_combine_f32(const float* e_t, const float* old1, const float* old2, const float* old3, float* out, long n, int order,
                        void* stream);
int ae_ddim_encode_step_f32(const float* x, const float* eps, float* x_next, long n, int branches, float scale, float cx, float ce,
                            void* stream);
int ae_mask_blend_f32(const float* img, const float* x0, const float* noise, const float* mask, float* out, int B, int C, int HW,
                      float sqrt_ac, float sqrt_one_minus_ac, int ip2p_order, void* stream);
int ae_q_sample_f32(const float* x0, const float* noise, const float* sqrt_ac, const float* sqrt_one_minus_ac, float* out, int B,
                    long per_sample, void* stream);
int ae_silu_to_bf16(const void* x, int in_bf16, void* y, long n, void* stream);
int ae_add_bcast_bf16(const void* x, const void* p, void* y, long n, long period, void* stream);
int ae_resample2x_rows_bf16(const void* x, void* y, int B, int H, int W, int C, int mode, void* stream);
int ae_scale_shift_rows_bf16(const void* x, const float* emb, long ld_emb, void* y, int B, long HW, int C, int silu, void* stream);
int ae_window_partition_bf16(const void* image, void* windows, int B, int H, int W, int C, int ws, int reverse, void* stream);
int ae_layernorm_window_supported(int C);
int ae_layernorm_window_bf16(const void* x, const void* shortcut, const float* gamma, const float* beta, void* y, void* xsum,
                             int B, int H, int W, int C, int ws, int mode, float eps, void* stream);
int ae_sam_relpos_terms(const void* q, long q_sb, long q_sh, long q_sn, const float* Rh, const float* Rw, float* rel_h,
                        float* rel_w, int B, int heads, int qH, int qW, int kH, int kW, int D, void* stream);
int ae_patchify_f32_bf16(const float* x, void* y, int B, int Cin, int H, int W, int P, void* stream);
int ae_mse_f32(const float* a, const float* b, float* out, float* partial, long n, void* stream);
int ae_task_gate(const float* task_emb, const long* edit_code, const float* Wg, const float* bg, int B, int n_tasks, int Dt,
                 int E, float* probs, int* top1, float* top1_prob, void* stream);

int ae_softmax_rows_f32_bf16(const float* S, long lds, void* P, long ldp, int rows, int cols, float scale, void* stream);
int ae_gaussian_moments_f32(const float* moments, const float* noise, float* z, float* mean, float* logvar, float* std_out, int B,
                            long per_half, void* stream);

int ae_ms_deform_attn_fwd_f32(const float* value, const long* spatial_shapes, const long* level_start_index, const float* sampling_loc,
                              const float* attn_weight, float* out, int bs, int S, int heads, int d, int Q, int L, int P, void* stream);
int ae_ms_deform_attn_bwd_f32(const float* value, const long* spatial_shapes, const long* level_start_index, const float* sampling_loc,
                              const float* attn_weight, const float* grad_out, float* grad_value, float* grad_sampling_loc,
                              float* grad_attn_weight, int bs, int S, int heads, int d, int Q, int L, int P, void* stream);
int ae_linear_f32(const float* A, long lda, const float* W, long ldw, const float* bias, float* C, long ldc, int M, int N, int K,
                  void* stream);

int ae_dpm_multistep_f32(const float* x, const float* model_out, const float* m_prev, float* m_cur, float* x_next, long n, int branches,
                         float scale, int v_param, int predict_x0, float sigma_s, float alpha_s, int update, float a, float b, float c,
                         float inv_r0, void* stream);

int ae_lincomb4_f32(float* out, const float* x0, float c0, const float* x1, float c1, const float* x2, float c2, const float* x3, float c3,
                    long n, void* stream);
int ae_dpm_adaptive_err_f32(const float* x_lower, const float* x_higher, const float* x_prev, float atol, float rtol, int B,
                            long n_per_sample, float* out, void* stream);

int ae_layernorm_act_bf16(const void* x, const float* gamma, const float* beta, void* y, long M, int C, float eps, int act, void* stream);
int ae_sam_pe_encode_f32(const float* coords, const int* labels, const float* gauss, const float* table, float* out, int N, int F,
                         float offset, float inv_w, float inv_h, void* stream);
int ae_sam_mask_downscale_bf16(const float* masks, const float* w1, const float* b1, const float* g1, const float* e1, const float* w2,
                               const float* b2, const float* g2, const float* e2, void* out, int B, int h, int w, float eps, void* stream);
int ae_sam_mask_product_f32(const void* up, const float* hyper, float* out, int B, int h, int w, int M, int C, void* stream);
int ae_sam_postprocess_masks(const float* low, float* out_f32, void* out_u8, int N, int Hl, int Wl, int S, int ih, int iw, int oh, int ow,
                             float threshold, int merge, void* stream);
int ae_nms_sorted_f32(const float* boxes, void* keep, int N, float iou_threshold, void* stream);
int ae_sam_preprocess_f32(const void* x, int x_is_u8, float* y, int B, int C, int h, int w, int S, const float* mean, const float* stdv,
                          void* stream);

int ae_attn_causal_short_bf16(const void* q, const void* k, const void* v, void* out, int B, int H, int N, int D,
                              long q_sb, long q_sh, long q_sn, long k_sb, long k_sh, long k_sn, long v_sb, long v_sh, long v_sn,
                              long o_sb, long o_sh, long o_sn, float scale, void* stream);
int ae_clip_embed_bf16(const void* ids, int ids_are_i64, const void* token_table, const void* position_table, void* out, int B, int N,
                       int C, int vocab, int positions, void* stream);
int ae_bias_act_f32_bf16(const float* u, long ldu, const float* bias, void* y, long ldy, long M, int N, int act, void* stream);
int ae_clip_pool_eos_bf16(const void* ids, int ids_are_i64, const void* z, void* out, int B, int N, int C, long eos_token_id, void* stream);

int ae_clip_patch_rows_bf16(const void* x, int x_dtype, void* rows, int B, int Cin, int H, int W, int P, int Kpad, float rescale,
                            const float* mean, const float* stdv, void* stream);
int ae_clip_vision_embed_ln_bf16(const float* patch, long ldp, const float* class_embedding, const float* pos, const float* gamma,
                                 const float* beta, void* out, int B, int G, int C, float eps, void* stream);
int ae_clip_vision_pool_ln_bf16(const void* x, long row_stride, const float* gamma, const float* beta, void* out, int B, int C, float eps,
                                void* stream);

int ae_dino_embed_bf16(const float* patch, long ldp, const float* patch_bias, const float* cls_token, const float* pos, void* out, int B, int G,
                       int C, void* stream);
int ae_swiglu_f32_bf16(const float* u, long ldu, const float* bias, void* y, long ldy, long M, int Hd, void* stream);

int ae_swin_window_attn_bf16(const void* qkv, long ldq, const float* qkv_bias, const float* bias, void* out, long ldo, int B, int H, int W, int C,
                             int nH, int ws, int shift, float scale, void* stream);
int ae_swin_merge_ln_bf16(const void* x, const float* gamma, const float* beta, void* y, int B, int H, int W, int C, float eps, void* stream);

int ae_scale_residual_f32_bf16(const float* u, long ldu, const float* bias, const float* gamma, const void* res, long ldr, void* out, long ldo, long M,
                               int N, void* stream);
int ae_biattn_split_rows(int Nv);
long ae_biattn_workspace_bytes(int B, int heads, int Nv, int Nt, int D);
int ae_biattn_bf16(const void* q, long ldq, const void* k, long ldk, const void* val_v, long ldvv, const void* val_l, long ldvl, const void* mask_v,
                   const void* mask_l, void* out_v, long ldov, void* out_l, long ldol, int B, int heads, int Nv, int Nt, int D, float scale,
                   void* workspace, long workspace_bytes, void* stream);
int ae_attn_masked_short_bf16(const void* q, const void* k, const void* v, const void* mask, void* out, int B, int H, int N, int D, long q_sb, long q_sh,
                              long q_sn, long k_sb, long k_sh, long k_sn, long v_sb, long v_sh, long v_sn, long o_sb, long o_sh, long o_sn, float scale,
// ... 66 lines not shown
```

Measured before the change: 6.712 edited-images/sec.

## Fold ResBlock 1x1 skip conv into the output 3x3 conv GEMM K dimension

Appends the 1x1 skip-connection weights to the packed 3x3 conv weights and extends K with the skip input channels, so the conv GEMM loads skip activations (optionally from two concatenated sources) after the nine taps. This replaces the separate skip GEMM plus the residual read and write with a single kernel for ResBlocks whose channel count changes. Biases are summed on the host side once and cached. It adds loader branches to the conv kernel and applies only to stride-1, tap-major, 64-aligned inference paths.

```diff
diff --git a/anyedit_amd/_lib.py b/anyedit_amd/_lib.py
--- a/anyedit_amd/_lib.py
+++ b/anyedit_amd/_lib.py
@@ -22,6 +22,11 @@
     "ae_gemm_plan": [c_int] * 8 + [ctypes.POINTER(c_int)],
     "ae_conv3x3_plan": [c_int] * 11 + [ctypes.POINTER(c_int)],
     "ae_conv3x3_up2_plan": [c_int] * 6 + [ctypes.POINTER(c_int)],
+    "ae_conv3x3_skip_workspace_floats": [c_int] * 6,
+    "ae_conv3x3_skip_bf16": [c_void_p, c_void_p, c_void_p, c_void_p, c_long, c_void_p, c_long, c_int, c_int, c_void_p, c_int, c_int, c_int, c_int, c_int,
+                             c_void_p, c_void_p, c_void_p],
+    "ae_conv3x3_skip_plan": [c_int] * 9 + [ctypes.POINTER(c_int)],
+    "ae_conv3x3_skip_fold": [c_int] * 8,
     "ae_groupnorm_rows_per_chunk": [c_int, c_int],
     "ae_groupnorm_workspace_floats": [c_int, c_int, c_int, c_int],
     "ae_groupnorm_nhwc_bf16": [c_void_p, c_void_p, c_int, c_void_p, c_void_p, c_void_p, c_int, c_int, c_int, c_int, c_float,
@@ -158,7 +163,7 @@
     "ae_attn_token_map_bf16": [c_void_p] * 3 + [c_int] * 5 + [c_long] * 6 + [c_float, ctypes.POINTER(ctypes.c_ulonglong), c_int, c_void_p],
     "ae_masactrl_classes": [c_void_p, c_long, c_int, c_int, c_float, c_int, ctypes.POINTER(c_int), ctypes.POINTER(c_int), c_void_p, c_void_p, c_void_p],
 }
-_RESTYPES = {"ae_last_error": ctypes.c_char_p, "ae_groupnorm_workspace_floats": c_long, "ae_conv3x3_workspace_floats": c_long,
+_RESTYPES = {"ae_last_error": ctypes.c_char_p, "ae_groupnorm_workspace_floats": c_long, "ae_conv3x3_workspace_floats": c_long, "ae_conv3x3_skip_workspace_floats": c_long,
              "ae_groupnorm_bwd_workspace_floats": c_long, "ae_attn_fp8_workspace_bytes": c_long, "ae_attn_bwd_workspace_floats": c_long,
              "ae_biattn_workspace_bytes": c_long, "ae_gdino_neck_groupnorm_workspace_floats": c_long}
 
diff --git a/anyedit_amd/csrc/gemm_conv.hip b/anyedit_amd/csrc/gemm_conv.hip
--- a/anyedit_amd/csrc/gemm_conv.hip
+++ b/anyedit_amd/csrc/gemm_conv.hip
@@ -19,6 +19,9 @@
 #endif
 #ifndef AE_PP_DMA_FIRST
 #define AE_PP_DMA_FIRST 0
+#endif
+#ifndef AE_SKIP_FOLD_DEFAULT
+#define AE_SKIP_FOLD_DEFAULT 1
 #endif
 constexpr int BK = 64;
 
@@ -50,6 +53,11 @@
     int ln_parts;
     float ln_eps;
     int sub2;
+    const bf16_t* X;
+    const bf16_t* X2;
+    long ldx, ldx2;
+    int Cs, Cs1;
+    unsigned x_bytes, x2_bytes;
 };
 
 __device__ __forceinline__ void lds_dma16(__amdgpu_buffer_rsrc_t rs, bf16_t* lds_dst, int voffset, int soffset = 0) {
@@ -152,6 +160,15 @@
     const __amdgpu_buffer_rsrc_t rsA2 = __builtin_amdgcn_make_buffer_rsrc(const_cast<bf16_t*>(p.A2 ? p.A2 : p.A), 0, (int)(p.A2 ? p.a2_bytes : 0u), 0x00020000);
     const __amdgpu_buffer_rsrc_t rsW = __builtin_amdgcn_make_buffer_rsrc(const_cast<bf16_t*>(p.W) + ((AMODE == A_CONV3 && p.sub2) ? (long)split * p.N * p.ldw : 0L), 0, (int)p.w_bytes, 0x00020000);
     constexpr int OOB = (int)0x80000000;
+    const bool fold = AMODE == A_CONV3 && p.Cs > 0;
+    const __amdgpu_buffer_rsrc_t rsX = __builtin_amdgcn_make_buffer_rsrc(const_cast<bf16_t*>(fold ? p.X : p.A), 0, (int)(fold ? p.x_bytes : 0u), 0x00020000);
+    const __amdgpu_buffer_rsrc_t rsX2 = __builtin_amdgcn_make_buffer_rsrc(const_cast<bf16_t*>(fold && p.X2 ? p.X2 : p.A), 0, (int)(fold && p.X2 ? p.x2_bytes : 0u), 0x00020000);
+    const int skip_lin0 = fold ? 9 * (p.CinPad / BK) : 0x7fffffff;
+    auto skip_off = [&](int i, int ld2) __attribute__((always_inline)) -> int {
+        const int id = tid + i * NT, row = id >> 3;
+        const int m = m0 + row;
+        return m < p.M ? m * ld2 + (((id & 7) ^ (row & 7)) << 4) : OOB;
+    };
     int fa_off[A_CH], fa2_off[A_CH], fb_off[B_CH];
     unsigned fa_mask[A_CH];
 #pragma unroll
@@ -410,6 +427,15 @@
             } else {
                 int cur_tap = ld_tap, cur_ci = ld_ci;
                 constexpr bool STATELESS = true;
+                if (kt_begin + kt >= skip_lin0) {
+                    const int ks = (kt_begin + kt - skip_lin0) * BK;
+                    const bool second = ks >= p.Cs1;
+                    const int ld2 = (int)(second ? p.ldx2 : p.ldx) * 2, so = (second ? ks - p.Cs1 : ks) * 2;
+                    const __amdgpu_buffer_rsrc_t rs = second ? rsX2 : rsX;
+#pragma unroll
+                    for (int i = 0; i < A_CH; ++i) lds_dma16(rs, sA + buf * BM * BK + (wave + (NT / 64) * i) * 8 * BK, skip_off(i, ld2), so);
+                    return;
+                }
                 if (STATELESS) {
                     const int lin = kt_begin + kt;
                     if (p.kmajor) { cur_tap = lin % 9; cur_ci = (lin / 9) * BK; }
@@ -583,6 +609,7 @@
             auto cs_set = [&](int kt) __attribute__((always_inline)) {
                 const int lin = kt_begin + kt;
                 if (p.kmajor) { cs_tap = lin % 9; cs_ci = (lin / 9) * BK; }
+                else if (lin >= skip_lin0) { cs_tap = 9; cs_ci = (lin - skip_lin0) * BK; }
                 else { cs_tap = conv_per == 1 ? lin : (int)__umulhi((unsigned)lin, pp_magic); cs_ci = (lin - cs_tap * conv_per) * BK; }
                 int ky = cs_tap / 3;
                 cs_kx = cs_tap - ky * 3;
@@ -599,7 +626,7 @@
                     } else {
                     ++cs_tap; ++cs_kx; cs_base += cs_cin2;
                     if (cs_kx == 3) { cs_kx = 0; cs_base += cs_row2; }
-                    if (cs_tap == 9) { cs_tap = 0; cs_base = 0; cs_ci += BK; }
+                    if (cs_tap == 9 && p.kmajor) { cs_tap = 0; cs_base = 0; cs_ci += BK; }
                     }
                 }
             };
@@ -613,6 +640,18 @@
 #pragma unroll
                         for (int i = 0; i < A_CH; ++i) ae_dma16(rsA2, ldsA + st * A_ST + i * (NT / 64) * 1024, fa2_off[i], (k0 - p.Ksplit) * 2);
                     }
+                } else if (cs_tap >= 9 && !p.kmajor) {
+                    const bool second = cs_ci >= p.Cs1;
+                    const int ld2 = (int)(second ? p.ldx2 : p.ldx) * 2, so = (second ? cs_ci - p.Cs1 : cs_ci) * 2;
+                    const __amdgpu_buffer_rsrc_t rs = second ? rsX2 : rsX;
+                    int off[A_CH];
+#pragma unroll
+                    for (int i = 0; i < A_CH; ++i) off[i] = skip_off(i, ld2);
+#pragma unroll
+                    for (int i = 0; i < A_CH; ++i) asm volatile("" : "+v"(off[i]));
+#pragma unroll
+                    for (int i = 0; i < A_CH; ++i) ae_dma16(rs, ldsA + st * A_ST + i * (NT / 64) * 1024, off[i], so);
+                    cs_ci += BK;
                 } else {
                     int off[A_CH];
 #pragma unroll
@@ -1306,6 +1345,10 @@
     const LaunchCtx lc{a, stream, what, report};
     static const int glds_env = getenv("AE_GEMM_GLDS") ? atoi(getenv("AE_GEMM_GLDS")) : 1;
     const bool glds = glds_env && (conv ? (a.Cin == a.CinPad) : (a.K % BK == 0 && (!a.A2 || a.Ksplit % BK == 0)));
+    if (conv && a.Cs > 0 && (!glds || a.kmajor || a.stride != 1 || a.ups || a.sub2)) {
+        ae_set_error("%s: the skip fold runs in the tap-major LDS-DMA loaders of stride-1 convs without resampling (Cin %% 64 == 0, k_order 0)", what);
+        return AE_ERR_UNSUPPORTED;
+    }
     if (conv && a.kmajor && !glds) { ae_set_error("%s: the chunk-major K order exists only in the LDS-DMA loader (AE_GEMM_GLDS=0 is set)", what); return AE_ERR_UNSUPPORTED; }
     auto lds_of = [](int bm, int bn, int st) { return (size_t)st * (bm + bn) * BK * sizeof(bf16_t); };
     auto lds_wa = [](int bm, int bn) { return (size_t)(2 * bm + 3 * bn) * BK * sizeof(bf16_t); };
@@ -1627,19 +1670,35 @@
     return plan_out(rc ? rc : launch_sub2(a, nullptr, &r), r, plan);
 }
 
-extern "C" long ae_conv3x3_workspace_floats(int B, int H, int W, int Cin, int Cout, int stride, int upsample2x) {
+namespace {
+long conv_workspace_floats(int B, int H, int W, int Cin, int Cout, int stride, int upsample2x, int Cs) {
     const int Hv = upsample2x ? 2 * H : H, Wv = upsample2x ? 2 * W : W;
     const int Ho = (Hv + 2 - 3) / stride + 1, Wo = (Wv + 2 - 3) / stride + 1;
     const int CinPad = (Cin + BK - 1) / BK * BK;
     const long M = (long)B * Ho * Wo;
-    const int s = make_plan((int)M, Cout, 9 * CinPad, true).splitk;
+    const int s = make_plan((int)M, Cout, 9 * CinPad + Cs, true).splitk;
     return s > 1 ? (long)s * M * Cout : 0;
 }
+}
+
+extern "C" long ae_conv3x3_workspace_floats(int B, int H, int W, int Cin, int Cout, int stride, int upsample2x) {
+    return conv_workspace_floats(B, H, W, Cin, Cout, stride, upsample2x, 0);
+}
+
+extern "C" long ae_conv3x3_skip_workspace_floats(int B, int H, int W, int Cin, int Cout, int Cs) {
+    return conv_workspace_floats(B, H, W, Cin, Cout, 1, 0, Cs);
+}
 
 namespace {
+struct SkipOperand {
+    const void* x = nullptr;
+    const void* x2 = nullptr;
+    long ldx = 0, ldx2 = 0;
+    int Cs = 0, Cs1 = 0;
+};
 int conv_args(GemmArgs& a, int& split_tile, const void* x, const void* w, const float* bias, const float* addvec, long addvec_ld,
               const void* residual, void* y, int B, int H, int W, int Cin, int Cout, int stride, int upsample2x,
-              int out_f32, float* workspace, float* colstats, int k_order) {
+              int out_f32, float* workspace, float* colstats, int k_order, const SkipOperand& sk = SkipOperand{}) {
     AE_REQUIRE(x && w && y, "ae_conv3x3_bf16: null pointer");
     AE_REQUIRE(k_order == 0 || k_order == 1, "ae_conv3x3_bf16: k_order must be 0 (tap, channel) or 1 (64-channel chunk, tap, channel)");
     AE_REQUIRE(k_order == 0 || (Cin % 64 == 0 && !upsample2x), "ae_conv3x3_bf16: the chunk-major K order needs Cin %% 64 == 0 and no upsampling (Cin=%d)", Cin);
@@ -1657,11 +1716,25 @@
     a.A = (const bf16_t*)x; a.A2 = nullptr; a.W = (const bf16_t*)w; a.C = y;
     a.bias = bias; a.res = (const bf16_t*)residual; a.addvec = addvec;
     const int CinPad = (Cin + BK - 1) / BK * BK;
-    a.M = B * Ho * Wo; a.N = Cout; a.K = 9 * CinPad; a.Ksplit = a.K;
-    a.lda = 0; a.lda2 = 0; a.ldw = 9L * CinPad; a.ldc = Cout; a.ldr = Cout; a.ldav = addvec_ld > 0 ? addvec_ld : Cout;
+    if (sk.Cs > 0) {
+        AE_REQUIRE(stride == 1 && !upsample2x && k_order == 0 && Cin % 64 == 0, "ae_conv3x3_skip_bf16: the skip fold needs stride 1, no upsampling, the tap-major K order and Cin %% 64 == 0 (Cin=%d)", Cin);
+        AE_REQUIRE(sk.x && aligned16(sk.x) && sk.Cs % 64 == 0 && sk.ldx % 8 == 0, "ae_conv3x3_skip_bf16: the skip input needs 16-byte aligned rows and Cs %% 64 == 0 (Cs=%d)", sk.Cs);
+        if (sk.x2) AE_REQUIRE(aligned16(sk.x2) && sk.ldx2 % 8 == 0 && sk.Cs1 > 0 && sk.Cs1 < sk.Cs && sk.Cs1 % 64 == 0 && sk.ldx2 >= sk.Cs - sk.Cs1,
+                              "ae_conv3x3_skip_bf16: bad two-source split (Cs1=%d, Cs=%d): a multiple of 64 inside (0, Cs)", sk.Cs1, sk.Cs);
+        const int c1 = sk.x2 ? sk.Cs1 : sk.Cs;
+        AE_REQUIRE(sk.ldx >= c1, "ae_conv3x3_skip_bf16: the skip input's row stride %ld is shorter than its %d channels", sk.ldx, c1);
+        AE_REQUIRE((long)B * H * W * sk.ldx * 2 < (1L << 31) && (long)B * H * W * sk.ldx2 * 2 < (1L << 31) && (long)Cout * (9L * CinPad + sk.Cs) * 2 < (1L << 31),
+                   "ae_conv3x3_skip_bf16: operands must be smaller than 2 GiB");
+        a.X = (const bf16_t*)sk.x; a.X2 = (const bf16_t*)sk.x2; a.ldx = sk.ldx; a.ldx2 = sk.ldx2; a.Cs = sk.Cs; a.Cs1 = c1;
+        const long Mx = (long)B * H * W;
+        a.x_bytes = (unsigned)(((Mx - 1) * sk.ldx + c1) * 2);
+        a.x2_bytes = sk.x2 ? (unsigned)(((Mx - 1) * sk.ldx2 + (sk.Cs - c1)) * 2) : 0u;
+    }
+    a.M = B * Ho * Wo; a.N = Cout; a.K = 9 * CinPad + sk.Cs; a.Ksplit = a.K;
+    a.lda = 0; a.lda2 = 0; a.ldw = 9L * CinPad + sk.Cs; a.ldc = Cout; a.ldr = Cout; a.ldav = addvec_ld > 0 ? addvec_ld : Cout;
     a.epi = EPI_NONE; a.out_f32 = out_f32; a.rows_per_batch = Ho * Wo;
     a.H = H; a.Wd = W; a.Cin = Cin; a.CinPad = CinPad; a.Ho = Ho; a.Wo = Wo; a.stride = stride; a.ups = upsample2x;
-    a.a_bytes = (unsigned)((long)B * H * W * Cin * 2); a.a2_bytes = 0u; a.w_bytes = (unsigned)((long)Cout * 9 * CinPad * 2);
+    a.a_bytes = (unsigned)((long)B * H * W * Cin * 2); a.a2_bytes = 0u; a.w_bytes = (unsigned)((long)Cout * (9L * CinPad + sk.Cs) * 2);
     AE_REQUIRE((long)B * H * W * Cin * 2 < (1L << 31) && (long)Cout * 9 * CinPad * 2 < (1L << 31), "ae_conv3x3_bf16: operands must be smaller than 2 GiB");
     const Plan plan = workspace ? make_plan(a.M, a.N, a.K, true) : Plan{0, 1};
     a.splitk = plan.splitk;
@@ -1691,3 +1764,33 @@
                              workspace ? kQueryF32 : nullptr, colstats ? kQueryF32 : nullptr, k_order);
     return plan_out(rc ? rc : launch<A_CONV3>(a, nullptr, &r, split_tile), r, plan);
 }
+
+extern "C" int ae_conv3x3_skip_bf16(const void* x, const void* w, const float* bias, const void* xs, long ldxs, const void* xs2, long ldxs2, int Cs, int Cs1,
+                                    void* y, int B, int H, int W, int Cin, int Cout, float* workspace, float* colstats, void* stream) {
+    AE_REQUIRE(Cs > 0, "ae_conv3x3_skip_bf16: Cs=%d must be positive", Cs);
+    SkipOperand sk;
+    sk.x = xs; sk.x2 = xs2; sk.ldx = ldxs; sk.ldx2 = xs2 ? ldxs2 : 0; sk.Cs = Cs; sk.Cs1 = Cs1;
+    GemmArgs a;
+    int split_tile;
+    const int rc = conv_args(a, split_tile, x, w, bias, nullptr, 0, nullptr, y, B, H, W, Cin, Cout, 1, 0, 0, workspace, colstats, 0, sk);
+    return rc ? rc : launch<A_CONV3>(a, (hipStream_t)stream, nullptr, split_tile);
+}
+
+extern "C" int ae_conv3x3_skip_plan(int B, int H, int W, int Cin, int Cout, int Cs, int Cs1, int workspace, int colstats, int* plan) {
+    AE_REQUIRE(plan && Cs > 0, "ae_conv3x3_skip_plan: null plan or Cs=%d", Cs);
+    SkipOperand sk;
+    sk.x = kQueryPtr; sk.x2 = Cs1 > 0 && Cs1 < Cs ? kQueryPtr : nullptr; sk.ldx = sk.x2 ? Cs1 : Cs; sk.ldx2 = sk.x2 ? Cs - Cs1 : 0; sk.Cs = Cs; sk.Cs1 = Cs1;
+    GemmArgs a;
+    int split_tile;
+    PlanReport r{};
+    const int rc = conv_args(a, split_tile, kQueryPtr, kQueryPtr, nullptr, nullptr, 0, nullptr, kQueryPtr, B, H, W, Cin, Cout, 1, 0, 0,
+                             workspace ? kQueryF32 : nullptr, colstats ? kQueryF32 : nullptr, 0, sk);
+    return plan_out(rc ? rc : launch<A_CONV3>(a, nullptr, &r, split_tile), r, plan);
+}
+
+extern "C" int ae_conv3x3_skip_fold(int B, int H, int W, int Cin, int Cout, int Cs, int Cs1, int colstats) {
+    static const int knob = getenv("AE_SKIP_FOLD") ? atoi(getenv("AE_SKIP_FOLD")) : AE_SKIP_FOLD_DEFAULT;
+    if (!knob || Cs <= 0 || Cs % 64 || Cin % 64 || (Cs1 > 0 && Cs1 < Cs && Cs1 % 64)) return 0;
+    int plan[AE_PLAN_INTS];
+    return ae_conv3x3_skip_plan(B, H, W, Cin, Cout, Cs, Cs1, 1, colstats, plan) == 0 ? 1 : 0;
+}
diff --git a/anyedit_amd/ldm/modules/diffusionmodules/openaimodel.py b/anyedit_amd/ldm/modules/diffusionmodules/openaimodel.py
--- a/anyedit_amd/ldm/modules/diffusionmodules/openaimodel.py
+++ b/anyedit_amd/ldm/modules/diffusionmodules/openaimodel.py
@@ -201,15 +201,26 @@
             h = ops.scale_shift_rows(norm2.rows(h, B, Ho * Wo, silu=False, colstats=st1), emb_out, B, Ho * Wo, silu=True)
         else:
             h = norm2.rows(h, B, Ho * Wo, silu=True, colstats=st1)
+        st = _stats_for(B, Ho, Wo, self.out_channels, dev)
         if isinstance(self.skip_connection, nn.Identity):
             res = whole() if xs is None else xs
         elif self.skip_connection.kernel_size[0] == 1 and xs is None:
+            Cs1 = f.t.shape[1] if f.t2 is not None else 0
+            if ops.conv_skip_fold(B, H, W, self.out_channels, self.out_channels, self.channels, Cs1, st is not None):
+                w, b = self._skip_fold_pack()
+                y, _, _ = ops.conv3x3_skip(h, w, b, f.t, B, H, W, xs2=f.t2, colstats=st)
+                return Feat(y, B, Ho, Wo, st=st)
             res, _, _ = self.skip_connection.rows(f.t, B, H, W, a2=f.t2)
         else:
             res, _, _ = self.skip_connection.rows(whole() if xs is None else xs, B, Ho, Wo)
-        st = _stats_for(B, Ho, Wo, self.out_channels, dev)
         y, _, _ = self.out_layers[3].rows(h, B, Ho, Wo, residual=res, colstats=st)
         return Feat(y, B, Ho, Wo, st=st)
+
+    def _skip_fold_pack(self):
+        c2, sk = self.out_layers[3], self.skip_connection
+        if ops.cache_stale(self, "_skip_pk", c2.weight, c2.bias, sk.weight, sk.bias):
+            self._skip_pk = (ops.pack_conv3x3_skip(c2.weight, sk.weight), ops.skip_bias(c2.bias, sk.bias, self.out_channels, c2.weight.device))
+        return self._skip_pk
 
     def forward(self, x, emb):
         B, C, H, W = x.shape
diff --git a/anyedit_amd/ops.py b/anyedit_amd/ops.py
--- a/anyedit_amd/ops.py
+++ b/anyedit_amd/ops.py
@@ -90,6 +90,22 @@
     if k_order == 1:
         wp = wp.reshape(cout, 9, cin_pad // 64, 64).permute(0, 2, 1, 3)
     return wp.reshape(cout, 9 * cin_pad).contiguous()
+
+
+def pack_conv3x3_skip(w3x3, w1x1):
+    cout, cin = w3x3.shape[0], w3x3.shape[1]
+    ws = w1x1.detach().reshape(w1x1.shape[0], -1)
+    if cin % 64 or ws.shape[1] % 64 or ws.shape[0] != cout:
+        raise ValueError(f"pack_conv3x3_skip: Cin={cin} and Cs={ws.shape[1]} must be multiples of 64, both weights [Cout={cout}, ...]")
+    return torch.cat([pack_conv3x3(w3x3), ws.to(BF16)], dim=1).contiguous()
+
+
+def skip_bias(b2, b_skip, cout, device):
+    b = torch.zeros(cout, dtype=torch.float32, device=device)
+    for t in (b2, b_skip):
+        if t is not None:
+            b = b + t.detach().float().to(device)
+    return b.contiguous()
 
 
 def pack_conv3x3_taps8(w):
@@ -183,7 +199,11 @@
     return _plan("ae_gemm_plan", M, N, K, epilogue, Ksplit, int(out_f32), int(colstats), ln_mode)
 
 
-def conv_plan(B, H, W, Cin, Cout, stride=1, upsample2x=0, out_f32=False, colstats=False, k_order=0):
+def conv_plan(B, H, W, Cin, Cout, stride=1, upsample2x=0, out_f32=False, colstats=False, k_order=0, skip=0, skip_split=0):
+    if skip:
+        if stride != 1 or upsample2x or out_f32 or k_order:
+            return None
+        return _plan("ae_conv3x3_skip_plan", B, H, W, Cin, Cout, int(skip), int(skip_split), 1, int(colstats))
     return _plan("ae_conv3x3_plan", B, H, W, Cin, Cout, stride, int(upsample2x), int(out_f32), 1, int(colstats), int(k_order))
 
 
@@ -207,6 +227,18 @@
     if _CONV_KMAJOR == 4:
         return 1 if label in ("192x320", "128x128") else 0
     return 1 if (label == "192x320" or (_CONV_KMAJOR >= 2 and label == "192x320,splitK")) else 0
+
+
+_SKIP_FOLD = {}
+
+
+def conv_skip_fold(B, H, W, Cin, Cout, Cs, Cs1=0, colstats=False):
+    if _TAPE is not None and _TAPE.active:
+        return False
+    key = (B, H, W, Cin, Cout, Cs, Cs1, bool(colstats))
+    if key not in _SKIP_FOLD:
+        _SKIP_FOLD[key] = bool(lib.ae_conv3x3_skip_fold(B, H, W, Cin, Cout, Cs, Cs1, int(bool(colstats))))
+    return _SKIP_FOLD[key]
 
 
 def pack_geglu(w, b):
@@ -476,6 +508,37 @@
                               _p(out), B, H, W, Cin, Cout, stride, int(upsample2x), 1 if out_f32 else 0, _p(ws), _p(colstats), int(k_order), _s()),
           "ae_conv3x3_bf16")
     return out, Ho, Wo
+
+
+def conv3x3_skip(x, w, bias, xs, B, H, W, xs2=None, out=None, colstats=None):
+    if _TAPE is not None and _TAPE.active:
+        raise ValueError("conv3x3_skip: forward / inference only (the training tape keeps the separate skip GEMM)")
+    _chk(x, BF16, "conv3x3_skip.x", 2)
+    _chk(w, BF16, "conv3x3_skip.w", 2)
+    _chk(xs, BF16, "conv3x3_skip.xs", 2)
+    M, Cin, Cout = B * H * W, x.shape[1], w.shape[0]
+    Cs1 = xs.shape[1]
+    Cs = Cs1 + (xs2.shape[1] if xs2 is not None else 0)
+    if x.shape[0] != M or not x.is_contiguous():
+        raise ValueError(f"conv3x3_skip: x must be contiguous [B*H*W, Cin] = [{M}, Cin], got {tuple(x.shape)}")
+    if tuple(w.shape) != (Cout, 9 * Cin + Cs) or not w.is_contiguous():
+        raise ValueError(f"conv3x3_skip: packed weight must be a contiguous [Cout, {9 * Cin + Cs}] tensor, got {tuple(w.shape)}")
+    for t, nm in ((xs, "xs"), (xs2, "xs2")):
+        if t is not None:
+            _chk(t, BF16, "conv3x3_skip." + nm, 2)
+            if t.shape[0] != M or t.stride(1) != 1:
+                raise ValueError(f"conv3x3_skip: {nm} must be [{M}, C] rows with unit channel stride, got {tuple(t.shape)} strides {t.stride()}")
+    if out is None:
+        out = torch.empty(M, Cout, dtype=BF16, device=x.device)
+    nws = lib.ae_conv3x3_skip_workspace_floats(B, H, W, Cin, Cout, Cs)
+    ws = torch.empty(nws, dtype=torch.float32, device=x.device) if nws > 0 else None
+    if colstats is not None:
+        _chk(colstats, torch.float32, "conv3x3_skip.colstats", 3)
+        if tuple(colstats.shape) != ((M + 31) // 32, Cout, 2) or not colstats.is_contiguous():
+            raise ValueError(f"conv3x3_skip: colstats must be a contiguous [{(M + 31) // 32}, {Cout}, 2] fp32 buffer")
+    check(lib.ae_conv3x3_skip_bf16(_p(x), _p(w), _p(bias), _p(xs), xs.stride(0), _p(xs2), xs2.stride(0) if xs2 is not None else 0, Cs, Cs1,
+                                   _p(out), B, H, W, Cin, Cout, _p(ws), _p(colstats), _s()), "ae_conv3x3_skip_bf16")
+    return out, H, W
 
 
 _GN_COUNTERS = {}
@@ -2499,6 +2562,15 @@
     return f"gemm_kernel<{plan_label(p)},conv3x3>|M={M} Cin={Cin} Cout={Cout} s{stride}{'u' if upsample2x else ''}", 2.0 * M * Cout * 9 * Cin, float(nb), 1 + p.reduce + p.colstats
 
 
+def _conv_skip_label(_r, x, w, bias, xs, B, H, W, xs2=None, **_):
+    y = _r[0]
+    M, Cout, Cin = y.shape[0], w.shape[0], x.shape[1]
+    Cs = w.shape[1] - 9 * Cin
+    p = conv_plan(B, H, W, Cin, Cout, colstats=_.get("colstats") is not None, skip=Cs, skip_split=xs.shape[1] if xs2 is not None else 0)
+    nb = 2 * (x.numel() + M * Cs + w.numel()) + 2 * y.numel()
+    return f"gemm_kernel<{plan_label(p)},conv3x3,skip>|M={M} Cin={Cin} Cout={Cout} Cs={Cs}", 2.0 * M * Cout * (9 * Cin + Cs), float(nb), 1 + p.reduce + p.colstats
+
+
 def _attn_label(_r, q, k, v, B, H, Nq, Nk, D, *a, **kw):
     fast = D in (40, 80, 160) and kw.get("key_mask") is None and os.environ.get("AE_ATTN_FAST", "1") != "0" and \
         (D != 160 or os.environ.get("AE_ATTN_FAST160", "1") != "0") and \
@@ -2555,6 +2627,7 @@
 gemm = _wrap_profiled(gemm, _gemm_label)
 attention_fp8 = _wrap_profiled(attention_fp8, _attn8_label)
 conv3x3 = _wrap_profiled(conv3x3, _conv_label)
+conv3x3_skip = _wrap_profiled(conv3x3_skip, _conv_skip_label)
 attention = _wrap_profiled(attention, _attn_label)
 groupnorm = _wrap_profiled(groupnorm, _gn_label)
 layernorm = _wrap_profiled(layernorm, _ln_label)
diff --git a/include/anyedit_hip.h b/include/anyedit_hip.h
--- a/include/anyedit_hip.h
+++ b/include/anyedit_hip.h
@@ -53,6 +53,12 @@
 int ae_conv3x3_plan(int B, int H, int W, int Cin, int Cout, int stride, int upsample2x, int out_f32, int workspace, int colstats, int k_order,
                     int* plan);
 int ae_conv3x3_up2_plan(int B, int H, int W, int Cin, int Cout, int colstats, int* plan);
+
+long ae_conv3x3_skip_workspace_floats(int B, int H, int W, int Cin, int Cout, int Cs);
+int ae_conv3x3_skip_bf16(const void* x, const void* w, const float* bias, const void* xs, long ldxs, const void* xs2, long ldxs2, int Cs, int Cs1,
+                         void* y, int B, int H, int W, int Cin, int Cout, float* workspace, float* colstats, void* stream);
+int ae_conv3x3_skip_plan(int B, int H, int W, int Cin, int Cout, int Cs, int Cs1, int workspace, int colstats, int* plan);
+int ae_conv3x3_skip_fold(int B, int H, int W, int Cin, int Cout, int Cs, int Cs1, int colstats);
 
 int ae_groupnorm_rows_per_chunk(int HW, int C);
 long ae_groupnorm_workspace_floats(int B, int HW, int C, int groups);
```

New measurement: 6.776 edited-images/sec (median of 6 runs). No clear change (+1.0%).
